# sclaus2/CutFEMx

Hardware: AMD Instinct MI355X
Metric: assembled DOFs/sec (active dofs / full hot-path step) + cut-quadrature points/sec, Poisson P1 sphere level-set (higher is better)
Workload: dtype f64; 1 GPU; 3D Poisson P1, sphere level set on 512^3 background mesh (805306368 tets), Nitsche + ghost penalty, runtime quadrature order 4; one step = cut + rules + sparsity + assemble_matrix + assemble_vector + deactivation; cells=805306368, active_dofs=17125633, parallelism=1 gpu

## Files before the change

cutfemx_amd/_lib.py:

```python
from __future__ import annotations

import ctypes as C
from pathlib import Path

import os

import numpy as np

_HERE = Path(__file__).resolve().parent
LIB_PATH = Path(os.environ["CFX_LIB"]).resolve() if os.environ.get("CFX_LIB") else _HERE / "libcutfemx_amd.so"

OK, ERR_INVALID_ARGUMENT, ERR_RUNTIME, ERR_OUT_OF_RANGE, ERR_HIP, ERR_STEP_VOID = 0, -1, -2, -3, -4, -5


class StepVoid(RuntimeError):
    """Raised inside a cutfemx_amd.step whose capacities (taken from the previous step) did not fit: the results of
    the step are void; `cutfemx_amd.run_step` ends it and repeats the body."""

INSIDE, INTERSECTED, OUTSIDE = -1, 0, 1
CELL, EXTERIOR_FACET, INTERIOR_FACET = 0, 1, 2
K_MASS, K_STIFFNESS, K_NITSCHE, K_GHOST_GRADJUMP, K_ELASTICITY = 1, 2, 3, 4, 5
K_EXTENSION_L2 = 8
K_JUMP = 9
K_SIP = 10
K_DIV_TEST, K_DIV_TRIAL = 20, 21
L_SOURCE, L_NITSCHE_RHS = 101, 102
M_FIELD, M_L2_DIFF, M_H1_SEMI = 201, 202, 203
F_ONE, F_SINPROD, F_POISSON_RHS, F_COEFFICIENT = 0, 1, 2, 3


class CutOptions(C.Structure):
    _fields_ = [("cut_approximation_order", C.c_int32), ("max_refinement_iterations", C.c_int32),
                ("edge_max_depth", C.c_int32), ("reserved", C.c_int32)]


class RulesView(C.Structure):
    _fields_ = [("tdim", C.c_int32), ("gdim", C.c_int32), ("nq", C.c_int64), ("nr", C.c_int64),
                ("points", C.c_void_p), ("weights", C.c_void_p), ("offsets", C.c_void_p),
                ("parent_map", C.c_void_p), ("host_width", C.c_int32), ("reserved", C.c_int32),
                ("host_rows", C.c_void_p), ("host_verts", C.c_void_p)]


class Integral(C.Structure):
    _fields_ = [("type", C.c_int32), ("kernel", C.c_int32), ("qdegree", C.c_int32),
                ("point_stride", C.c_int32), ("entities", C.c_void_p), ("n_entities", C.c_int64),
                ("rules", C.c_void_p), ("point_data", C.c_void_p), ("params", C.c_double * 8),
                ("coefficient", C.c_void_p)]


class Coefficient(C.Structure):
    _fields_ = [("space", C.c_void_p), ("values", C.c_void_p)]


class AggregationView(C.Structure):
    _fields_ = [("ncells", C.c_int64), ("root_cell", C.c_void_p), ("aggregate_id", C.c_void_p),
                ("propagation_depth", C.c_void_p), ("cut_volume_fraction", C.c_void_p),
                ("active_cells", C.c_void_p), ("cut_cells", C.c_void_p), ("interior_cells", C.c_void_p),
                ("well_posed_cells", C.c_void_p), ("ill_posed_cells", C.c_void_p), ("rootless_cells", C.c_void_p),
                ("n_active", C.c_int64), ("n_cut", C.c_int64), ("n_interior", C.c_int64),
                ("n_well_posed", C.c_int64), ("n_ill_posed", C.c_int64), ("n_rootless", C.c_int64),
                ("pairs", C.c_void_p), ("n_pairs", C.c_int64)]


class DistExchange(C.Structure):
    _fields_ = [("peer", C.c_int32), ("reserved", C.c_int32), ("send_offset", C.c_int64), ("send_count", C.c_int64),
                ("send_index", C.c_void_p), ("recv_offset", C.c_int64), ("recv_count", C.c_int64),
                ("recv_index", C.c_void_p)]


class DistRowExchange(C.Structure):
    _fields_ = [("peer", C.c_int32), ("reserved", C.c_int32), ("send_row_lo", C.c_int64), ("send_row_hi", C.c_int64),
                ("recv_row_lo", C.c_int64), ("recv_row_hi", C.c_int64)]


HOST_EXCHANGE_FN = C.CFUNCTYPE(C.c_int, C.c_void_p, C.c_int, C.POINTER(C.c_int32), C.POINTER(C.c_void_p),
                               C.POINTER(C.c_int64), C.POINTER(C.c_void_p), C.POINTER(C.c_int64))


class CGOptions(C.Structure):
    _fields_ = [("rtol", C.c_double), ("atol", C.c_double), ("max_iter", C.c_int32), ("check_every", C.c_int32),
                ("precond", C.c_int32), ("lanes_per_row", C.c_int32)]


class CGInfoStruct(C.Structure):
    _fields_ = [("reason", C.c_int32), ("iterations", C.c_int32), ("residual_norm", C.c_double), ("rhs_norm", C.c_double)]


PC_NONE, PC_JACOBI = 0, 1
CG_CONVERGED, CG_MAX_ITER, CG_BREAKDOWN, CG_BAD_DIAGONAL = 1, 2, 3, 4


class PatternView(C.Structure):
    _fields_ = [("nrows", C.c_int64), ("nnz", C.c_int64), ("indptr", C.c_void_p),
                ("indices", C.c_void_p), ("ncols", C.c_int64)]


SYMBOLS = [
    "cfx_init", "cfx_last_error", "cfx_set_stream", "cfx_synchronize", "cfx_step_begin", "cfx_step_end", "cfx_step_resolve", "cfx_step_abort",
    "cfx_step_set_margin", "cfx_step_forget", "cfx_sync_count", "cfx_list_count", "cfx_integrand_register", "cfx_integrand_compile", "cfx_integrand_register_facet", "cfx_integrand_register_variant", "cfx_integrand_compile_bs", "cfx_integrand_register2", "cfx_integrand_compile2", "cfx_integrand_compile_coefficients", "cfx_form_set_coefficients", "cfx_overlap_begin", "cfx_overlap_side", "cfx_overlap_end", "cfx_copy",
    "cfx_device_alloc", "cfx_device_free", "cfx_device_memset", "cfx_device_cache_release", "cfx_device_memory_stats", "cfx_profile_enable", "cfx_profile_reset",
    "cfx_profile_count", "cfx_profile_get", "cfx_event_create", "cfx_event_record",
    "cfx_event_elapsed_ms", "cfx_event_destroy", "cfx_mesh_create", "cfx_mesh_create_box", "cfx_mesh_create_slab",
    "cfx_mesh_info", "cfx_mesh_destroy", "cfx_cut_options_default", "cfx_cut_create",
    "cfx_cut_restrict", "cfx_cut_create_facets", "cfx_exterior_facets", "cfx_full_facet_rules",
    "cfx_facet_rules_to_cells", "cfx_cut_update", "cfx_cut_info", "cfx_cut_domain", "cfx_locate_entities",
    "cfx_runtime_quadrature", "cfx_runtime_quadratures", "cfx_full_cell_rules", "cfx_rules_create", "cfx_rules_view_get",
    "cfx_rules_physical_points", "cfx_rules_destroy", "cfx_evaluate_normals",
    "cfx_evaluate_values", "cfx_ghost_penalty_facets", "cfx_interior_facets_for_cells", "cfx_cell_aggregation_create", "cfx_cell_aggregation_view_get",
    "cfx_cell_aggregation_destroy", "cfx_cut_destroy", "cfx_space_create",
    "cfx_space_static_bytes", "cfx_space_lattice_rows", "cfx_space_lattice_source_rows", "cfx_space_destroy", "cfx_form_create", "cfx_form_create2", "cfx_form_destroy", "cfx_form_prepare", "cfx_create_sparsity",
    "cfx_pattern_view_get", "cfx_pattern_reuse_stats", "cfx_pattern_destroy", "cfx_assemble_matrix", "cfx_assemble_matrix_zeroed", "cfx_assemble_vector", "cfx_assemble_scalar",
    "cfx_apply_lifting", "cfx_set_bc", "cfx_zero_rows", "cfx_csr_block_merge", "cfx_csr_permute", "cfx_tabulate_entity", "cfx_active_domain", "cfx_active_view", "cfx_deactivate_outside",
    "cfx_active_destroy", "cfx_csr_spmv", "cfx_cg_options_default", "cfx_cg_solve",
    "cfx_dist_unique_id", "cfx_dist_comm_create", "cfx_dist_comm_create_host", "cfx_dist_comm_create_device", "cfx_dist_comm_info", "cfx_dist_comm_destroy",
    "cfx_dist_scatter_forward", "cfx_dist_scatter_reverse_add", "cfx_dist_scatter_reverse_matrix", "cfx_dist_indicator_or",
    "cfx_dist_indicator_forward",
    "cfx_mesh_create_f32", "cfx_cut_create_f32", "cfx_cut_update_f32", "cfx_rules_create_f32", "cfx_rules_view_get_f32",
    "cfx_rules_physical_points_f32", "cfx_evaluate_normals_f32", "cfx_evaluate_values_f32", "cfx_widen_f32",
    "cfx_assemble_matrix_f32", "cfx_assemble_matrix_zeroed_f32", "cfx_assemble_vector_f32", "cfx_apply_lifting_f32",
    "cfx_set_bc_f32", "cfx_zero_rows_f32", "cfx_deactivate_outside_f32",
    "cfx_assemble_matrix_c128", "cfx_assemble_vector_c128", "cfx_apply_lifting_c128", "cfx_set_bc_c128",
    "cfx_deactivate_outside_c128",
    "cfx_assemble_matrix_c64", "cfx_assemble_vector_c64", "cfx_apply_lifting_c64", "cfx_set_bc_c64", "cfx_deactivate_outside_c64",
]

_lib = None
_initialised = False


def load():
    global _lib
    if _lib is None:
        if not LIB_PATH.exists():
            raise RuntimeError(
                f"{LIB_PATH} is missing: build it with `python -c 'import __graft_entry__ as g; "
                "g.build()'` (hipcc --offload-arch=gfx950). cutfemx_amd has no CPU fallback.")
        import importlib.util
        import sys
        if "torch" not in sys.modules and importlib.util.find_spec("torch") is not None:
            import torch
        _lib = C.CDLL(str(LIB_PATH))
        _lib.cfx_last_error.restype = C.c_char_p
        for name in SYMBOLS:
            getattr(_lib, name)
    return _lib


def lib():
    global _initialised
    l = load()
    if not _initialised:
        check(l.cfx_init(_default_device()))
        _initialised = True
    return l


def _default_device() -> int:
    import os
    return int(os.environ.get("LOCAL_RANK", "0")) if os.environ.get("CFX_DEVICE") is None \
        else int(os.environ["CFX_DEVICE"])


def check(code: int):
    if code == OK:
        return
    msg = (load().cfx_last_error() or b"").decode()
    if code == ERR_INVALID_ARGUMENT:
        raise ValueError(msg)
    if code == ERR_OUT_OF_RANGE:
        raise IndexError(msg)
    if code == ERR_STEP_VOID:
        raise StepVoid(msg)
    raise RuntimeError(msg)


class DeviceBuffer:

    def __init__(self, count: int, dtype, shape=None):
        self.dtype = np.dtype(dtype)
        self.size = int(count)
        self.shape = shape if shape is not None else (self.size,)
        self.ndim = len(self.shape)
        p = C.c_void_p()
        check(lib().cfx_device_alloc(C.byref(p), C.c_size_t(max(self.size, 1) * self.dtype.itemsize)))
        self.ptr = p.value

    def numpy(self) -> np.ndarray:
        return download(self.ptr, self.size, self.dtype).reshape(self.shape)

    def fill_from(self, host: np.ndarray):
        host = np.ascontiguousarray(host, dtype=self.dtype)
        check(lib().cfx_copy(C.c_void_p(self.ptr), host.ctypes.data_as(C.c_void_p), C.c_size_t(host.nbytes)))

    def __del__(self):
        try:
            if self.ptr:
                load().cfx_device_free(C.c_void_p(self.ptr))
                self.ptr = None
        except Exception:
            pass


def is_torch(a) -> bool:
    return type(a).__module__.startswith("torch")


def is_device(a) -> bool:
    return isinstance(a, DeviceBuffer) or (is_torch(a) and a.is_cuda)


def as_ptr(a, dtype, keep: list):
    if a is None:
        return None
    if isinstance(a, DeviceBuffer):
        if a.dtype != np.dtype(dtype):
            raise TypeError(f"device buffer has dtype {a.dtype}, expected {np.dtype(dtype)}")
        keep.append(a)
        return C.c_void_p(a.ptr)
    if is_torch(a):
        import torch
        want = {np.float64: torch.float64, np.float32: torch.float32, np.int32: torch.int32, np.int8: torch.int8}[dtype]
        if a.dtype != want or not a.is_contiguous():
            a = a.to(want).contiguous()
        keep.append(a)
        return C.c_void_p(a.data_ptr())
    arr = np.ascontiguousarray(a, dtype=dtype)
    keep.append(arr)
    return arr.ctypes.data_as(C.c_void_p)


def scalar_dtype(a):
    if a is None:
        return np.float64
    if getattr(a, "dtype", None) == np.dtype(np.complex128):
        return np.complex128
    if getattr(a, "dtype", None) == np.dtype(np.complex64):
        return np.complex64
    if isinstance(a, DeviceBuffer):
        return np.float32 if a.dtype == np.dtype(np.float32) else np.float64
    if is_torch(a):
        import torch
        return np.float32 if a.dtype == torch.float32 else np.float64
    return np.float32 if getattr(a, "dtype", None) == np.dtype(np.float32) else np.float64


def release_cache():
    check(lib().cfx_device_cache_release())


def memory_stats(reset_peak: bool = False) -> dict:
    a, b, c = C.c_size_t(), C.c_size_t(), C.c_size_t()
    check(lib().cfx_device_memory_stats(C.byref(a), C.byref(b), C.byref(c), 1 if reset_peak else 0))
    return dict(in_use=a.value, cached=b.value, peak=c.value)


_step_open = False


def resolve_counts():
    if _step_open:
        check(lib().cfx_step_resolve())


# ... 12 lines not shown
```

cutfemx_amd/csrc/cfx_common.h:

```cpp
#pragma once

#include <hip/hip_runtime.h>

#include <algorithm>
#include <array>
#include <cstdint>
#include <cstdio>
#include <cstring>
#include <functional>
#include <map>
#include <memory>
#include <stdexcept>
#include <string>
#include <utility>
#include <vector>

#include "../../include/cutfemx_amd.h"
#include "cfx_switches.h"

namespace cfx
{

struct Error : std::runtime_error
{
// ... 357 lines not shown
  CFX_HIP(hipStreamSynchronize(ctx().stream));
  return a;
}

template <typename T>
inline DevArray<T> to_device_aligned(const T* src, int64_t n)
{
  if (src != nullptr && n > 0 && is_device_pointer(src) && (reinterpret_cast<uintptr_t>(src) & 15) != 0)
  {
    DevArray<T> a;
    a.alloc(n);
    CFX_HIP(hipMemcpyAsync(a.p, src, sizeof(T) * (size_t)n, hipMemcpyDeviceToDevice, ctx().stream));
    return a;
  }
  return to_device(src, n);
}

struct ErrorFlag
{
  int* p;
  bool deferred;
  ErrorFlag(int code, const char* message, void (*decode)(int) = nullptr);
  void check(int code, const char* message) const;
};
int64_t count_for_buffer(const Count& c, const void* user);
void end_of_call_sync();

int64_t& sync_counter();

void* pinned_scratch();

struct StepVoidGuard
{
  int64_t* host = nullptr;
  StepVoidGuard();
  void check() const;
};

template <typename T>
inline T read_scalar(const T* dev)
{
  static_assert(sizeof(T) <= 256, "read_scalar reads small values");
  T* h = static_cast<T*>(pinned_scratch());
  CFX_HIP(hipMemcpyAsync(h, dev, sizeof(T), hipMemcpyDeviceToHost, ctx().stream));
  const StepVoidGuard guard;
  CFX_HIP(hipStreamSynchronize(ctx().stream));
  const T v = *h;
  ++sync_counter();
  if (ctx().trace_sync) fprintf(stderr, "cutfemx_amd: read-back after %s\n", ctx().last_launch);
  guard.check();
  return v;
}

template <typename T>
inline void read_two(const T* dev_a, const T* dev_b, T& a, T& b)
{
  static_assert(2 * sizeof(T) <= 256, "read_two reads small values");
  T* h = static_cast<T*>(pinned_scratch());
  CFX_HIP(hipMemcpyAsync(h, dev_a, sizeof(T), hipMemcpyDeviceToHost, ctx().stream));
  CFX_HIP(hipMemcpyAsync(h + 1, dev_b, sizeof(T), hipMemcpyDeviceToHost, ctx().stream));
  const StepVoidGuard guard;
  CFX_HIP(hipStreamSynchronize(ctx().stream));
  a = h[0]; b = h[1];
  ++sync_counter();
  if (ctx().trace_sync) fprintf(stderr, "cutfemx_amd: read-back after %s\n", ctx().last_launch);
  guard.check();
}

template <typename T>
inline std::vector<T> download(const T* dev, int64_t n)
{
  std::vector<T> v((size_t)n);
  if (n > 0)
  {
    CFX_HIP(hipMemcpyAsync(v.data(), dev, sizeof(T) * (size_t)n, hipMemcpyDeviceToHost, ctx().stream));
    const StepVoidGuard guard;
    CFX_HIP(hipStreamSynchronize(ctx().stream));
    guard.check();
  }
  return v;
}

template <typename T>
struct OutArray
{
  T* user = nullptr;
  DevArray<T> staging;
  T* dev = nullptr;
  int64_t n = 0;
  OutArray(T* dst, int64_t count, bool copy_in) : user(dst), n(count)
  {
    if (is_device_pointer(dst)) { dev = dst; return; }
    staging.alloc(count);
    dev = staging.p;
    if (copy_in && count > 0)
      CFX_HIP(hipMemcpyAsync(dev, dst, sizeof(T) * (size_t)count, hipMemcpyHostToDevice, ctx().stream));
  }
  void finish()
  {
    if (dev != user && n > 0)
    {
      CFX_HIP(hipMemcpyAsync(user, dev, sizeof(T) * (size_t)n, hipMemcpyDeviceToHost, ctx().stream));
      CFX_HIP(hipStreamSynchronize(ctx().stream));
    }
  }
};

void exclusive_scan(const int32_t* in, int64_t* out, int64_t n, CountPlan* after = nullptr);
void exclusive_scan(const int32_t* in, int32_t* out, int64_t n, CountPlan* after = nullptr);
void exclusive_scan(const int64_t* in, int64_t* out, int64_t n, CountPlan* after = nullptr);
void exclusive_scan_pair(const int32_t* inA, int64_t* outA, const int32_t* inB, int64_t* outB, int64_t n, CountPlan* after = nullptr);
void exclusive_scan_pair(const int64_t* inA, int64_t* outA, const int64_t* inB, int64_t* outB, int64_t n, CountPlan* after = nullptr);

struct Adjacency
{
  DevArray<int64_t> offsets;
  DevArray<int32_t> cells;
  bool built = false;
};

void build_adjacency(const int32_t* map, int64_t ncells, int width, int64_t nitems, Adjacency& adj);

struct Stencil
{
  DevArray<int64_t> offsets;
  DevArray<int32_t> nbr;
  DevArray<uint32_t> slot4;
  DevArray<uint8_t> diagpos;
  DevArray<uint8_t> cpos;
  bool built = false, usable = false;
  bool lists = false;
  DevArray<uint8_t> slotn;
  bool slotn_built = false, slotn_ok = false;
  int max_len = 0;
  DevArray<int64_t> tile_voff;
  DevArray<int32_t> tile_verts;
  DevArray<uint16_t> st_loc;
  bool tiles_built = false, tiles_usable = false;
  int max_tile_verts = 0, max_tile_items = 0, max_tile_st = 0;
  bool lat_built = false, lat_tmpl_built = false;
  int64_t lat_rows = 0, lat_rstar = -1;
  int64_t lat_sb0 = 0;
  int lat_rel = 0;
  int lat_len = 0;
  DevArray<double> lat_scratch;
  const double* lat_tmpl = nullptr;
  DevArray<unsigned long long> lat_written;
  static constexpr int kLatStarCells = 64, kLatSrcDegrees = 9;
  int lat_src_state = 0;
  std::vector<double> lat_star;
  double lat_src_T[kLatSrcDegrees][8] = {};
  bool lat_src_T_built[kLatSrcDegrees] = {};
  DevArray<unsigned long long> lat_src_written;
  DevArray<uint8_t> arena;
  int64_t arena_used = 0;
  template <typename T>
  void take(DevArray<T>& a, int64_t n)
  {
    const int64_t bytes = ((int64_t)sizeof(T) * (n > 0 ? n : 1) + 255) & ~255LL;
    if (arena.p && arena_used + bytes <= arena.n)
    {
      a.release();
      a.p = reinterpret_cast<T*>(arena.p + arena_used); a.n = n; a.owned = false;
      arena_used += bytes;
    }
    else
      a.alloc(n);
  }
};
constexpr int kRowTile = 16;
constexpr unsigned kLatFlag = 0x80u, kDiagPosMask = 0x7fu;
__device__ __forceinline__ bool lattice_template_row(unsigned diagpos_raw, unsigned umark, unsigned long long mask,
                                                     unsigned inline_bits, unsigned long long full)
{
  return (diagpos_raw & kLatFlag) != 0 && __popc(umark & inline_bits) == 1 && mask == full;
}
__device__ __forceinline__ bool lattice_source_row(int32_t vec_t2off_r, unsigned diagpos_raw)
{
  return vec_t2off_r != 0 && (diagpos_raw & kLatFlag) != 0;
}

struct VecBlocks
{
  bool built = false, usable = false;
  int B = 0;
  int64_t nblocks = 0, u_total = 0;
  DevArray<int64_t> u_off;
  DevArray<uint16_t> slot;
  DevArray<uint16_t> seg;
  DevArray<int64_t> p_off;
  DevArray<int64_t> p_pos;
};
constexpr int kVbEntries = 2048;

constexpr int kKuhnTet[6][4] = {{0, 1, 3, 7}, {0, 1, 5, 7}, {0, 2, 3, 7}, {0, 2, 6, 7}, {0, 4, 5, 7}, {0, 4, 6, 7}};

}

struct cfx_mesh_s
{
  int tdim = 0, gdim = 0;
  int64_t nnodes = 0, ncells = 0;
  cfx::DevArray<double> x;
  cfx::DevArray<int32_t> conn;
  cfx::Adjacency v2c;
  const cfx::Adjacency& vertex_cells()
  {
    if (!v2c.built) cfx::build_adjacency(conn.p, ncells, tdim + 1, nnodes, v2c);
    return v2c;
  }
  cfx::DevArray<int32_t> c2c;
  bool c2c_built = false;
  int box_n = 0;
  bool hex_groups = false;
  cfx::DevArray<uint8_t> hex_corners;
  const cfx::DevArray<int32_t>& cell_neighbours();
  cfx::DevArray<int32_t> class_nruns;
  cfx::DevArray<int2> class_runs;
  cfx::DevArray<int2> class_sub_runs;
  bool class_built = false;
};
constexpr int kClassBlock = 1024, kClassRuns = 32;
constexpr int kClassSub = 4, kClassSubRuns = 16;

struct cfx_rules_s
{
  const uint64_t serial = cfx::next_serial();
  cfx_rules_s() { cfx::rules_serial_live(serial, true); }
  ~cfx_rules_s() { cfx::rules_serial_live(serial, false); }
  cfx_rules_s(const cfx_rules_s&) = delete;
  cfx_rules_s& operator=(const cfx_rules_s&) = delete;
  cfx_mesh_t mesh = nullptr;
  int tdim = 0, gdim = 0;
  cfx::Count nq, nr;
  cfx::DevArray<double> points, weights;
  cfx::DevArray<float> points_f32, weights_f32;
  cfx::DevArray<int32_t> offsets, parent_map;
  bool parent_sentinel = false;
  int host_width = 0;
  cfx::DevArray<int32_t> host_rows;
  cfx::DevArray<int32_t> host_verts;
};

struct cfx_cut_s
{
  cfx_mesh_t mesh = nullptr;
  int nls = 0;
  int ls_ndofs_cell = 0;
  int64_t ls_ndofs = 0;
  cfx_cut_options options{};
  cfx::DevArray<int32_t> ls_dofmap;
  std::vector<cfx::DevArray<double>> ls_values;
  cfx::DevArray<int8_t> domain;
  cfx::DevArray<uint8_t> host_mask;
  cfx::DevArray<int32_t> tile_block;
  cfx::DevArray<int32_t> tiles_inside, tiles_cut;
  cfx::DevArray<uint8_t> block_class;
  cfx::DevArray<uint8_t> codes0;
  cfx::DevArray<uint8_t> touch0;
  bool touch_valid = false;
  uint64_t gen = 0;
  ~cfx_cut_s() { cfx::provenance_forget_cut(this); }
  std::map<std::string, cfx::DevArray<int32_t>> located;
  std::map<std::string, cfx::DevArray<int32_t>> ghost_rows;
  int host_width = 0;
  int64_t n_hosts = 0;
  cfx::DevArray<int32_t> host_ids;
  cfx::DevArray<int32_t> host_rows;
  cfx::DevArray<int32_t> host_verts;
  std::map<std::string, cfx::DevArray<int32_t>> located_ids;
  int64_t nhosts() const { return host_width ? n_hosts : mesh->ncells; }
  int host_dim() const { return host_width ? mesh->tdim - 1 : mesh->tdim; }
};

struct cfx_pattern_cache
{
  struct cfx_pattern_s* live = nullptr;
  cfx::DevArray<int64_t> indptr;
  cfx::DevArray<int32_t> indices;
  cfx::DevArray<uint8_t> sig;
  std::vector<int> form_key;
  int64_t nrows = 0;
  bool valid = false;
  void drop();
};

struct cfx_space_s
{
  cfx_mesh_t mesh = nullptr;
  int degree = 1, bs = 1, ndofs_cell = 0;
  int64_t ndofs = 0;
  cfx::DevArray<int32_t> dofmap;
  cfx::Adjacency d2c;
  std::vector<std::weak_ptr<struct cfx_row_plan>> plans;
  cfx::Stencil stencil;
  cfx::VecBlocks vblocks;
  cfx::DevArray<int32_t> dof_verts;
  bool dof_verts_built = false, dof_verts_ok = false;
  cfx_pattern_cache pcache;
  ~cfx_space_s() { cfx::step_forget_owner(this); pcache.drop(); }
  bool lists_short_overflow = false;
  bool long_rows = false;
  bool huge_rows = false;
  const cfx::Adjacency& dof_cells()
  {
    if (dofmap.p == mesh->conn.p && ndofs == mesh->nnodes) return mesh->vertex_cells();
    if (!d2c.built) cfx::build_adjacency(dofmap.p, mesh->ncells, ndofs_cell, ndofs, d2c);
    return d2c;
  }
};

struct cfx_coefficient_dev
{
  cfx_space_t space = nullptr;
  cfx::DevArray<double> values;
};

struct cfx_integral_dev
{
  int type = 0, kernel = 0, qdegree = 0, point_stride = 0;
  cfx::DevArray<int32_t> entities;
  cfx::Count n_entities;
  cfx_rules_t rules = nullptr;
  uint64_t entities_serial = 0, rules_serial = 0;
  int64_t n_std = -1;
  cfx::DevArray<double> point_data;
  cfx::DevArray<double> coefficient;
  std::vector<cfx_coefficient_dev> coefficients;
  double params[8] = {0, 0, 0, 0, 0, 0, 0, 0};
};

struct cfx_row_plan
{
  bool built = false;
  bool usable = false;
  cfx::DevArray<uint8_t> mark_block;
  cfx::DevArray<uint8_t> rowcls;
  bool bulk = false;
  int bulk_kind = 0;
  uint8_t bulk_bits = 0;
  cfx::DevArray<uint8_t> cellmark;
  cfx::DevArray<uint8_t> cellsig;
  cfx::DevArray<uint8_t> rowmark;
  cfx::DevArray<int32_t> active_rows;
  cfx::Count n_active_rows;
  cfx::DevArray<int32_t> special_rows;
  cfx::Count n_special_rows;
  cfx::DevArray<uint8_t> special_mark;
  cfx::DevArray<int32_t> special_pos;
  cfx::DevArray<int32_t> plain_rows;
  cfx::Count n_plain_rows;
  uint64_t serial = 0;
  cfx::DevArray<unsigned long long> plain_masks;
  cfx::DevArray<uint8_t> plain_uniform;
  bool plain_masks_built = false;
  cfx::DevArray<int32_t> plain_tile_first, plain_tile_id;
  cfx::Count n_plain_tiles;
  cfx::DevArray<int32_t> lat_tile_first, lat_tile_id;
  cfx::Count n_lat_tiles;
  bool lat_tiles_built = false;
  unsigned lat_bits = 0;
  cfx::DevArray<int32_t> vec_t2off;
  bool vec_t2off_used = false;
  cfx::Count n_vec_odd_rows;
  cfx::Count vec_t2_total;
  int vec_fast = -1;
  uint8_t vec_mark = 0;
  bool vec_groups = false;
  int64_t vec_group_cap = 0;
  cfx::DevArray<int32_t> vb_active;
  cfx::DevArray<int32_t> vb_cut;
  cfx::DevArray<int64_t> vb_base;
  int64_t n_vb_active = 0, n_vb_cut = 0, vb_total = 0;
  int vb_state = -1;
  uint8_t vb_mark = 0;
  bool vb_merged = false;
  bool any_cells = false;
  cfx::Count nfacets;
  cfx::DevArray<int32_t> cell_tile_counts;
  cfx::DevArray<int64_t> row_tile_counts;
  bool fold_ok = true;
  cfx::DevArray<int32_t> facet_rows;
  cfx::DevArray<uint8_t> facet_slot;
  cfx::DevArray<int64_t> d2f_offsets;
  cfx::DevArray<int32_t> d2f;
  int n_cell_slots = 0, n_facet_slots = 0;
  cfx::DevArray<int64_t> std_bits[4];
  cfx::DevArray<int32_t> std_rank[4];
  cfx::DevArray<int32_t> rule_key_block;
  cfx::DevArray<int32_t> rule_keys[4], rule_first[4];
  uint32_t rule_mask[4] = {0, 0, 0, 0};
  cfx::DevArray<int32_t> cut_cells;
  int64_t n_cut_cells = 0;
  cfx::DevArray<int64_t> cut_bits;
  cfx::DevArray<int32_t> cut_rank;
  cfx::DevArray<int32_t> cut_first[4];
  bool cut_cells_built = false;
  int cell_slot_integral[4] = {0, 0, 0, 0};
  int facet_slot_integral[2] = {0, 0};
  std::vector<std::array<int64_t, 7>> key_cells, key_facets;
};

struct cfx_form_s
{
  cfx_space_t V = nullptr;
  cfx_space_t V1 = nullptr;
  bool rectangular() const { return V1 != nullptr && V1 != V; }
  int rank = 2;
  std::vector<cfx_integral_dev> integrals;
  std::shared_ptr<cfx_row_plan> plan;
  std::map<std::vector<int>, std::unique_ptr<cfx_form_s>> sub_forms;
};

namespace cfx
{
bool assemble_rect_rows(cfx_form_s* a, cfx_pattern_s* P, const int8_t* bc0, const int8_t* bc1, double* values, int* error);
cfx_row_plan& row_plan(cfx_form_s* a);
void validate_form(const cfx_form_s* a);
const Stencil& space_stencil(cfx_space_s* V);
const Stencil& space_stencil_slotn(cfx_space_s* V);
bool plain_row_masks(cfx_form_s* a, int32_t* counts = nullptr, int* maxlen = nullptr);
void plan_cut_cells(cfx_form_s* a);
const Stencil& space_stencil_tiles(cfx_space_s* V);
const Stencil& space_lattice(cfx_space_s* V);
bool lattice_template(cfx_space_s* V);
const double* lattice_source_moments(cfx_space_s* V, int qdegree);
bool plain_lattice_tiles(cfx_form_s* a, unsigned inline_bits);
bool space_dof_verts(cfx_space_s* V);
bool plain_vec_offsets(cfx_form_s* L, uint8_t mark);
bool source_groups_ok(cfx_form_s* L, uint8_t mark);
const VecBlocks& space_vec_blocks(cfx_space_s* V);
bool vec_block_plan(cfx_form_s* L, uint8_t mark, bool merged);
void build_pattern(cfx_form_s* a, cfx_pattern_s* P);
void build_pattern_rectangular(cfx_form_s* a, cfx_pattern_s* P);
void plan_cell_signature(cfx_form_s* a);
bool pattern_reuse_ok(cfx_form_s* a);
void pattern_remember(cfx_form_s* a, cfx_pattern_s* P);
void prepare_form_tables(cfx_form_s* a);
bool assemble_matrix_rows(cfx_form_s* a, cfx_pattern_s* P, const int8_t* bc0, const int8_t* bc1, double* values,
                          bool fresh = false);
bool assemble_vector_rows(cfx_form_s* L, double* b);
bool user_integrand_known(int kernel);
int user_integrand_rank(int kernel);
int user_integrand_kind(int kernel);
bool user_integrand_two(int kernel);
void user_coefficients_check(const cfx_form_s* a, const cfx_integral_dev& I);
int64_t user_stage1_facets(const cfx_form_s* a, const cfx_integral_dev& I, double* out, int64_t only_index = -1);
int64_t user_stage1(const cfx_form_s* a, const cfx_integral_dev& I, bool runtime, double* out, int out_mode, int64_t out_stride,
                    int64_t only_index = -1);
void functional_entity(const cfx_form_s* M, const cfx_integral_dev& I, int64_t index, int use_rule, double* out_dev);
}

struct cfx_pattern_s
{
  cfx_space_s* cache_owner = nullptr;
  ~cfx_pattern_s();
  int64_t nrows = 0;
  cfx::Count nnz;
  int64_t ncols = 0;
  int max_row_len = 0;
  int64_t n_hashed_rows = 0, n_reused_rows = 0;
  uint64_t built_plan = 0;
  uint64_t stencil_plan = 0;
  uint64_t split_plan = 0;
  cfx::DevArray<int32_t> short_rows, mid_rows, long_rows;
  int64_t n_short_rows = 0, n_mid_rows = 0, n_long_rows = 0;
  uint64_t full_plan = 0;
  cfx::DevArray<int32_t> full_rows;
  int64_t n_full_rows = 0;
  int64_t n_full_short = 0;
  uint64_t odd_plan = 0;
  cfx::DevArray<int32_t> odd_rows;
  int64_t n_odd_rows = 0;
  cfx::DevArray<int32_t> rest_rows;
  int64_t n_rest_rows = 0;
  cfx::DevArray<int64_t> indptr;
  cfx::DevArray<int32_t> indices;
};

struct cfx_aggregation_s
{
  int64_t ncells = 0;
  cfx::DevArray<int32_t> root_cell, aggregate_id, depth;
  cfx::DevArray<double> fraction;
  cfx::DevArray<int32_t> active, cut, interior, well, ill, rootless, pairs;
  int64_t n_pairs = 0;
};

struct cfx_active_s
{
  cfx_space_t V = nullptr;
  std::shared_ptr<cfx_row_plan> plan;
  cfx::DevArray<uint8_t> cell_indicator;
  bool lists_built = false;
  cfx::DevArray<int32_t> active_cells, inactive_dofs;
  cfx::Count n_active, n_inactive;
};
namespace cfx
{
void active_lists(cfx_active_s* d);
}
```

cutfemx_amd/csrc/cfx_fem.hip:

```cpp
#include <cstdlib>

#include "cfx_elem.h"

using namespace cfx;

namespace
{

struct AsmArgs
{
  const double* x;
  const int32_t* conn;
  const int32_t* dofmap;
  DevN n;
  const int32_t* entities;
  const int32_t* offsets;
  const int32_t* parent_map;
  const double* points;
  const double* weights;
  const double* point_data;
  int point_stride;
  int kernel;
  int qdegree;
  double params[8];
// ... 1586 lines not shown
}
template <int TDIM>
__global__ void __launch_bounds__(kBlock) cut_moments_kernel(int64_t nr, const int32_t* __restrict__ offsets,
                                                             const double* __restrict__ points, const double* __restrict__ weights,
                                                             double* __restrict__ out)
{
  constexpr int NV = TDIM + 1, NM = 1 + NV + NV * (NV + 1) / 2;
  const int64_t e = (int64_t)blockIdx.x * kBlock + threadIdx.x;
  if (e >= nr) return;
  double m[16];
#pragma unroll
  for (int k = 0; k < 16; ++k) m[k] = 0.0;
  const int32_t q0 = offsets[e], q1 = offsets[e + 1];
  for (int32_t q = q0; q < q1; ++q)
  {
    double lam[NV];
    lam[0] = 1.0;
#pragma unroll
    for (int t = 0; t < TDIM; ++t) { lam[t + 1] = points[(int64_t)q * TDIM + t]; lam[0] -= lam[t + 1]; }
    const double w = weights[q];
    m[0] += w;
    int idx = 1 + NV;
#pragma unroll
    for (int x = 0; x < NV; ++x)
    {
      const double wx = w * lam[x];
      m[1 + x] += wx;
#pragma unroll
      for (int y = x; y < NV; ++y) m[idx++] += wx * lam[y];
    }
  }
  static_assert(NM <= 16, "record of 16 doubles");
  double2* o = reinterpret_cast<double2*>(out + 16 * e);
#pragma unroll
  for (int k = 0; k < 8; ++k) o[k] = make_double2(m[2 * k], m[2 * k + 1]);
}
}

namespace cfx
{
void dump_integral(cfx_form_s* a, int integral, int parts, double* out, bool fold_facets)
{
  cfx_space_s* V = a->V;
  ZeroFlag err;
  AsmArgs A{};
  A.x = V->mesh->x.p; A.conn = V->mesh->conn.p; A.dofmap = V->dofmap.p;
  A.dump = out; A.error = err.p;
  A.dump_fold = fold_facets ? 1 : 0;
  const cfx_integral_dev& I = a->integrals[integral];
  if (a->rectangular() && user_integrand_known(I.kernel)) launch_user_integral(a, I, A, -1, 0, parts);
  else launch_integral(a, I, A, -1, 0, parts);
}
void dump_facet_jumps_p1(cfx_form_s* a, int integral, double* out, int* error)
{
  cfx_space_s* V = a->V;
  const cfx_integral_dev& I = a->integrals[integral];
  if (I.n_entities.cap() == 0) return;
  if (V->mesh->tdim == 2)
    launch("assemble_facets", facet_jump_p1_kernel<2>, grid_for(I.n_entities.cap()), dim3(kBlock), 0, I.n_entities, I.entities.p,
           V->mesh->x.p, V->mesh->conn.p, V->dofmap.p, I.params[0], I.params[1], I.qdegree, out, error);
  else
    launch("assemble_facets", facet_jump_p1_kernel<3>, grid_for(I.n_entities.cap()), dim3(kBlock), 0, I.n_entities, I.entities.p,
           V->mesh->x.p, V->mesh->conn.p, V->dofmap.p, I.params[0], I.params[1], I.qdegree, out, error);
}
void dump_cut_moments(cfx_form_s* a, int integral, double* out)
{
  const cfx_integral_dev& I = a->integrals[integral];
  if (!I.rules || I.rules->nr.value() == 0) return;
  const int64_t nrl = I.rules->nr.value();
  if (a->V->mesh->tdim == 2)
    launch("assemble_cells_cut", cut_moments_kernel<2>, grid_for(nrl), dim3(kBlock), 0, nrl,
           I.rules->offsets.p, I.rules->points.p, I.rules->weights.p, out);
  else
    launch("assemble_cells_cut", cut_moments_kernel<3>, grid_for(nrl), dim3(kBlock), 0, nrl,
           I.rules->offsets.p, I.rules->points.p, I.rules->weights.p, out);
}

void dump_facet_jumps_p2(cfx_form_s* a, int integral, int nq, double* out)
{
  cfx_space_s* V = a->V;
  const cfx_integral_dev& I = a->integrals[integral];
  const int64_t nf = I.n_entities.value();
  if (nf == 0) return;
  if (V->mesh->tdim == 2)
    launch("assemble_facets", facet_jumps_p2_kernel<2>, grid_for(nf * nq), dim3(kBlock), 0, nf, nq,
           I.entities.p, V->mesh->x.p, V->mesh->conn.p, V->dofmap.p, I.params[0], I.params[1], I.qdegree, out);
  else
    launch("assemble_facets", facet_jumps_p2_kernel<3>, grid_for(nf * nq), dim3(kBlock), 0, nf, nq,
           I.entities.p, V->mesh->x.p, V->mesh->conn.p, V->dofmap.p, I.params[0], I.params[1], I.qdegree, out);
}
}

extern "C" {

int cfx_space_create(cfx_mesh_t mesh, int degree, int bs, int64_t ndofs, const int32_t* dofmap, int ndofs_cell,
                     cfx_space_t* out)
{
  CFX_API_BEGIN
  ctx().ensure();
  require(mesh && dofmap && out, CFX_ERR_INVALID_ARGUMENT, "cfx_space_create: null argument");
  require(degree == 1 || degree == 2, CFX_ERR_INVALID_ARGUMENT, "cfx_space_create: Lagrange degree must be 1 or 2");
  const int expect = degree == 1 ? mesh->tdim + 1 : (mesh->tdim == 2 ? 6 : 10);
  require(ndofs_cell == expect, CFX_ERR_INVALID_ARGUMENT, "cfx_space_create: dofs per cell do not match the element");
  require(bs == 1 || bs == mesh->gdim, CFX_ERR_INVALID_ARGUMENT, "cfx_space_create: block size must be 1 or gdim");
  require(ndofs > 0 && ndofs * bs < 2147483647LL, CFX_ERR_INVALID_ARGUMENT, "cfx_space_create: dof count must fit int32");
  auto V = std::make_unique<cfx_space_s>();
  V->mesh = mesh; V->degree = degree; V->bs = bs; V->ndofs = ndofs; V->ndofs_cell = ndofs_cell;
  V->dofmap = to_device_aligned(dofmap, mesh->ncells * (int64_t)ndofs_cell);
  *out = V.release();
  CFX_API_END
}

int cfx_space_static_bytes(cfx_space_t V, int64_t bytes[4])
{
  CFX_API_BEGIN
  require(V && bytes, CFX_ERR_INVALID_ARGUMENT, "cfx_space_static_bytes: null argument");
  const bool shared = V->dofmap.p == V->mesh->conn.p && V->ndofs == V->mesh->nnodes;
  const cfx::Adjacency& adj = shared ? V->mesh->v2c : V->d2c;
  bytes[0] = adj.built ? 8 * adj.offsets.n + 4 * adj.cells.n : 0;
  const cfx::Stencil& S = V->stencil;
  bytes[1] = 8 * S.offsets.n + 4 * S.nbr.n + 4 * S.slot4.n + S.diagpos.n + S.cpos.n + S.slotn.n;
  const cfx::VecBlocks& B = V->vblocks;
  bytes[2] = 8 * S.tile_voff.n + 4 * S.tile_verts.n + 2 * S.st_loc.n
             + 8 * B.u_off.n + 2 * B.slot.n + 2 * B.seg.n + 8 * B.p_off.n + 8 * B.p_pos.n;
  bytes[3] = (V->mesh->c2c_built ? 4 * V->mesh->c2c.n : 0)
             + (V->mesh->class_built ? 4 * V->mesh->class_nruns.n + 8 * (V->mesh->class_runs.n + V->mesh->class_sub_runs.n) : 0);
  CFX_API_END
}

int cfx_space_lattice_rows(cfx_space_t V, int64_t* n, int64_t* template_rows)
{
  CFX_API_BEGIN
  require(V && n, CFX_ERR_INVALID_ARGUMENT, "cfx_space_lattice_rows: null argument");
  *n = 0;
  if (template_rows) *template_rows = 0;
  if (V->degree != 1 || V->bs != 1 || !cfx::space_stencil(V).usable) return CFX_OK;
  const cfx::Stencil& S = cfx::space_lattice(V);
  *n = S.lat_rows;
  if (template_rows && S.lat_rows > 0 && S.lat_written.p) *template_rows = (int64_t)cfx::read_scalar(S.lat_written.p);
  CFX_API_END
}

int cfx_space_lattice_source_rows(cfx_space_t V, int64_t* rows)
{
  CFX_API_BEGIN
  require(V && rows, CFX_ERR_INVALID_ARGUMENT, "cfx_space_lattice_source_rows: null argument");
  *rows = 0;
  if (V->degree != 1 || V->bs != 1 || !cfx::space_stencil(V).usable) return CFX_OK;
  const cfx::Stencil& S = cfx::space_lattice(V);
  if (S.lat_rows > 0 && S.lat_src_written.p) *rows = (int64_t)cfx::read_scalar(S.lat_src_written.p);
  CFX_API_END
}

int cfx_space_destroy(cfx_space_t V)
{
  CFX_API_BEGIN
  delete V;
  CFX_API_END
}

static int form_create_impl(cfx_space_t V, cfx_space_t V1, int rank, int n_integrals, const cfx_integral* integrals,
                            cfx_form_t* out);

int cfx_form_create(cfx_space_t V, int rank, int n_integrals, const cfx_integral* integrals, cfx_form_t* out)
{
  return form_create_impl(V, V, rank, n_integrals, integrals, out);
}

int cfx_form_create2(cfx_space_t V_test, cfx_space_t V_trial, int n_integrals, const cfx_integral* integrals, cfx_form_t* out)
{
  CFX_API_BEGIN
  require(V_test && V_trial, CFX_ERR_INVALID_ARGUMENT, "cfx_form_create2: null argument");
  require(V_test->mesh == V_trial->mesh, CFX_ERR_INVALID_ARGUMENT, "cfx_form_create2: the two spaces live on different meshes");
  CFX_API_END_NO_RETURN
  return form_create_impl(V_test, V_trial, 2, n_integrals, integrals, out);
}

static int form_create_impl(cfx_space_t V, cfx_space_t V1, int rank, int n_integrals, const cfx_integral* integrals,
                            cfx_form_t* out)
{
  CFX_API_BEGIN
  ctx().ensure();
  require(V && out && (integrals || n_integrals == 0), CFX_ERR_INVALID_ARGUMENT, "cfx_form_create: null argument");
  require(rank == 0 || rank == 1 || rank == 2, CFX_ERR_INVALID_ARGUMENT, "cfx_form_create: rank must be 0, 1 or 2");
  auto a = std::make_unique<cfx_form_s>();
  a->V = V; a->V1 = V1; a->rank = rank;
  const bool rect = V1 != V;
  for (int i = 0; i < n_integrals; ++i)
  {
    const cfx_integral& in = integrals[i];
    cfx_integral_dev I;
    I.type = in.type; I.kernel = in.kernel; I.qdegree = in.qdegree; I.point_stride = in.point_stride;
    require(in.type == CFX_CELL || in.type == CFX_INTERIOR_FACET, CFX_ERR_INVALID_ARGUMENT,
            "cfx_form_create: integral type must be cell or interior_facet");
    const bool user = user_integrand_known(in.kernel);
    const int kernel_rank = user ? user_integrand_rank(in.kernel) : (in.kernel < 100 ? 2 : (in.kernel < 200 ? 1 : 0));
    const bool bilinear = kernel_rank == 2;
    require(kernel_rank == rank, CFX_ERR_INVALID_ARGUMENT, "cfx_form_create: kernel rank does not match the form");
    require(in.qdegree >= 0 && in.qdegree <= CFX_QUAD_MAX_DEGREE, CFX_ERR_INVALID_ARGUMENT,
            "cfx_form_create: quadrature degree out of range");
    if (user)
    {
      if (rect)
        require(user_integrand_two(in.kernel), CFX_ERR_INVALID_ARGUMENT,
                "cfx_form_create2: the integrand was registered for a square form (one space); a form between two spaces "
                "takes an integrand registered with cfx_integrand_register2");
      else
        require(!user_integrand_two(in.kernel), CFX_ERR_INVALID_ARGUMENT,
                "cfx_form_create: the integrand was registered with cfx_integrand_register2 for a form between two spaces; "
                "a square form takes one registered for one space");
    }
    if (in.type == CFX_INTERIOR_FACET && user)
    {
      require(user_integrand_kind(in.kernel) == 1 && V->degree <= 2 && V1->degree <= 2 && 2 * V->ndofs_cell * V->bs <= 24
                  && 2 * V1->ndofs_cell * V1->bs <= 24,
              CFX_ERR_INVALID_ARGUMENT,
              "cfx_form_create: an interior-facet integral takes an integrand registered with cfx_integrand_register_facet "
              "(or cfx_integrand_register2 with facet = 1): spaces of degree 1 or 2 with at most 24 macro dofs on each side");
      if (in.rules)
        require(in.rules->host_width == 4 && in.point_data == nullptr, CFX_ERR_INVALID_ARGUMENT,
                "cfx_form_create: runtime rules of an interior-facet integral are facet-hosted rules over interior rows "
                "(cfx_cut_create_facets with row_width 4)");
    }
    else if (in.type == CFX_INTERIOR_FACET && rank == 0)
      throw Error(CFX_ERR_INVALID_ARGUMENT,
                  "cfx_form_create: interior-facet integrals of a functional take registered facet integrands "
                  "(cfx_integrand_register_variant with rank 0, facet 1)");
    else if (in.type == CFX_INTERIOR_FACET)
    {
      require(in.kernel == CFX_K_GHOST_GRADJUMP || in.kernel == CFX_K_EXTENSION_L2 || in.kernel == CFX_K_JUMP
                  || in.kernel == CFX_K_SIP,
              CFX_ERR_INVALID_ARGUMENT,
              "cfx_form_create: interior-facet integrals support the ghost-penalty, value-jump, interior-penalty and "
              "extension-penalty kernels");
      if (in.rules)
        require(in.kernel != CFX_K_EXTENSION_L2 && in.rules->host_width == 4 && in.point_data == nullptr,
                CFX_ERR_INVALID_ARGUMENT,
                "cfx_form_create: runtime rules of an interior-facet integral are facet-hosted rules over interior rows "
                "(cfx_cut_create_facets with row_width 4)");
    }
    else if (in.rules && in.rules->host_width != 0)
      throw Error(CFX_ERR_INVALID_ARGUMENT,
                  "cfx_form_create: a cell integral takes cell-hosted rules (pass facet-hosted rules through "
                  "cfx_facet_rules_to_cells)");
    else if (user)
      require(in.type == CFX_CELL && V->degree <= 2 && V1->degree <= 2 && user_integrand_kind(in.kernel) == 0,
              CFX_ERR_INVALID_ARGUMENT,
              "cfx_form_create: a cell integral takes an integrand registered with cfx_integrand_register (spaces of degree 1 or 2)");
    else if (rank == 0)
      require((in.kernel == CFX_M_FIELD || in.kernel == CFX_M_L2_DIFF || in.kernel == CFX_M_H1_SEMI)
                  && (V->degree == 1 || V->degree == 2) && V->bs >= 1 && V->bs <= 3,
              CFX_ERR_INVALID_ARGUMENT,
              "cfx_form_create: unknown functional id (CFX_M_FIELD, CFX_M_L2_DIFF, CFX_M_H1_SEMI on Lagrange spaces of degree "
              "1 or 2, block size 1..3)");
    else
      require(in.kernel == CFX_K_MASS || in.kernel == CFX_K_STIFFNESS || in.kernel == CFX_K_NITSCHE
                  || in.kernel == CFX_K_ELASTICITY || in.kernel == CFX_L_SOURCE || in.kernel == CFX_L_NITSCHE_RHS
                  || (rect && (in.kernel == CFX_K_DIV_TEST || in.kernel == CFX_K_DIV_TRIAL)),
              CFX_ERR_INVALID_ARGUMENT,
              "cfx_form_create: unknown cell kernel id (the divergence blocks need different test and trial spaces: "
              "cfx_form_create2)");
    if (rect && user)
    {
    }
    else if (rect)
    {
      require(in.coefficient == nullptr && in.point_data == nullptr, CFX_ERR_INVALID_ARGUMENT,
              "cfx_form_create2: coefficients / per-point data are not supported on rectangular blocks");
      const int gd = V->mesh->gdim;
      if (in.type == CFX_INTERIOR_FACET)
        require((in.kernel == CFX_K_GHOST_GRADJUMP || in.kernel == CFX_K_JUMP) && V->bs == 1 && V1->bs == 1 && in.rules == nullptr,
                CFX_ERR_INVALID_ARGUMENT,
                "cfx_form_create2: cell integrals, and interior-facet integrals (gradient jump, value jump) between "
                "scalar spaces over standard facets");
      else if (in.kernel == CFX_K_DIV_TEST)
        require(V->bs == gd && V1->bs == 1, CFX_ERR_INVALID_ARGUMENT, "div(v) p: vector test space, scalar trial space");
      else if (in.kernel == CFX_K_DIV_TRIAL)
        require(V->bs == 1 && V1->bs == gd, CFX_ERR_INVALID_ARGUMENT, "q div(u): scalar test space, vector trial space");
      else
        require((in.kernel == CFX_K_MASS || in.kernel == CFX_K_STIFFNESS) && V->bs == V1->bs, CFX_ERR_INVALID_ARGUMENT,
                "cfx_form_create2: mass / stiffness blocks need equal block sizes; other kernels are square-only");
    }
    if (in.kernel == CFX_K_NITSCHE || in.kernel == CFX_L_NITSCHE_RHS)
    {
      require(V->bs == 1, CFX_ERR_INVALID_ARGUMENT, "Nitsche kernels are scalar");
      require(in.n_entities == 0 && in.rules && in.point_data && in.point_stride >= V->mesh->gdim,
              CFX_ERR_INVALID_ARGUMENT,
              "Nitsche kernels need runtime interface rules and per-point normals (point_data)");
    }
    if (in.kernel == CFX_K_ELASTICITY)
      require(V->bs == V->mesh->gdim, CFX_ERR_INVALID_ARGUMENT, "elasticity needs a vector space (bs == gdim)");
    if (in.kernel == CFX_L_SOURCE)
      require(V->bs == 1 || (int)in.params[0] == CFX_F_COEFFICIENT, CFX_ERR_INVALID_ARGUMENT,
              "the source term of a vector space takes a vector-valued Function (field id CFX_F_COEFFICIENT)");
    if (bilinear)
    {
      require(in.coefficient == nullptr || in.kernel == CFX_K_MASS || in.kernel == CFX_K_STIFFNESS
                  || in.kernel == CFX_K_ELASTICITY || (rect && user),
              CFX_ERR_INVALID_ARGUMENT, "cfx_form_create: a coefficient is accepted by the mass, stiffness and elasticity terms");
      if (in.coefficient) I.coefficient = to_device(in.coefficient, V->ndofs);
    }
    else if (rank == 0)
    {
      const int field = (int)in.params[0];
      if (user)
        require(in.type == CFX_CELL || in.coefficient == nullptr || V->bs == 1, CFX_ERR_INVALID_ARGUMENT,
// ... 730 lines not shown
```

cutfemx_amd/csrc/cfx_gather.hip:

```cpp
#include <cstdlib>
#include <type_traits>

#include "cfx_elem.h"

using namespace cfx;

namespace cfx
{
void dump_integral(cfx_form_s* a, int integral, int parts, double* out, bool fold_facets = false);
void dump_facet_jumps_p1(cfx_form_s* a, int integral, double* out, int* error);
void dump_facet_jumps_p2(cfx_form_s* a, int integral, int nq, double* out);
void dump_cut_moments(cfx_form_s* a, int integral, double* out);
int quad_npoints(int dim, int degree);
}

namespace
{

constexpr int kWave = 64;
#ifndef CFX_XCD_TILE
#define CFX_XCD_TILE 128
#endif
__device__ __forceinline__ int64_t row_block_id(int64_t b)
{
// ... 432 lines not shown
  double det;
  if constexpr (TDIM == 2) det = ed[0][0] * ed[1][1] - ed[0][1] * ed[1][0];
  else
    det = ed[0][0] * (ed[1][1] * ed[2][2] - ed[1][2] * ed[2][1]) - ed[0][1] * (ed[1][0] * ed[2][2] - ed[1][2] * ed[2][0])
          + ed[0][2] * (ed[1][0] * ed[2][1] - ed[1][1] * ed[2][0]);
  const double cscale = fscale * fabs(det);
#pragma unroll
  for (int i = 0; i < ND; ++i) be[i] = 0.0;
  const double umax = kPi * hmax;
  if (umax <= 0.03)
  {
    double S[TDIM], C[TDIM];
#pragma unroll
    for (int d = 0; d < TDIM; ++d)
    {
      if (Sa) { S[d] = Sa[d]; C[d] = Ca[d]; }
      else cfx_sincospi(x[0][d], S[d], C[d]);
#pragma unroll
      for (int t = 0; t < TDIM; ++t) ed[t][d] *= kPi;
    }
    auto series = [&](auto deg_tag)
    {
      constexpr int DEGS = decltype(deg_tag)::value;
      double co[TDIM][DEGS + 1];
#pragma unroll
      for (int d = 0; d < TDIM; ++d)
      {
        const double inv[8] = {1.0, 1.0, -1.0 / 2.0, -1.0 / 6.0, 1.0 / 24.0, 1.0 / 120.0, -1.0 / 720.0, -1.0 / 5040.0};
#pragma unroll
        for (int k = 0; k <= DEGS; ++k) co[d][k] = ((k & 1) ? C[d] : S[d]) * inv[k];
      }
      for (int q = 0; q < npts; ++q)
      {
        double X[TDIM];
#pragma unroll
        for (int t = 0; t < TDIM; ++t) X[t] = pts[q * TDIM + t];
        double f = wts[q];
#pragma unroll
        for (int d = 0; d < TDIM; ++d)
        {
          double u = X[0] * ed[0][d];
#pragma unroll
          for (int t = 1; t < TDIM; ++t) u = fma(X[t], ed[t][d], u);
          double p = co[d][DEGS];
#pragma unroll
          for (int k = DEGS - 1; k >= 0; --k) p = fma(p, u, co[d][k]);
          f *= p;
        }
        be[0] += f;
#pragma unroll
        for (int t = 0; t < TDIM; ++t) be[t + 1] = fma(f, X[t], be[t + 1]);
      }
#pragma unroll
      for (int t = 0; t < TDIM; ++t) be[0] -= be[t + 1];
#pragma unroll
      for (int i = 0; i < ND; ++i) be[i] *= cscale;
    };
    if (umax <= 0.0065) series(std::integral_constant<int, 5>{});
    else series(std::integral_constant<int, 7>{});
  }
  else
  {
    for (int q = 0; q < npts; ++q)
    {
      double X[TDIM], l0 = 1.0;
#pragma unroll
      for (int t = 0; t < TDIM; ++t) { X[t] = pts[q * TDIM + t]; l0 -= X[t]; }
      double f = wts[q] * cscale;
#pragma unroll
      for (int d = 0; d < TDIM; ++d)
      {
        double v = x[0][d];
#pragma unroll
        for (int t = 0; t < TDIM; ++t) v = fma(X[t], ed[t][d], v);
        f *= cfx_sinpi(v);
      }
      be[0] = fma(f, l0, be[0]);
#pragma unroll
      for (int t = 0; t < TDIM; ++t) be[t + 1] = fma(f, X[t], be[t + 1]);
    }
  }
}

template <int TDIM>
__device__ __forceinline__ void source_compute(const VecArgs& A, const SourceCell<TDIM>& c, bool valid, int npts,
                                               const double* __restrict__ pts, const double* __restrict__ wts, double fscale)
{
  constexpr int ND = TDIM + 1;
  double be[ND];
  source_vector<TDIM>(c.x, npts, pts, wts, fscale, be);
  if (!valid) return;
  bool record = A.t2 == nullptr;
#pragma unroll
  for (int i = 0; i < ND; ++i)
  {
    if (c.t2o[i] >= 0) A.t2[(int64_t)c.t2o[i] + ((c.cp >> (8 * i)) & 0xffu)] = be[i];
    else record = true;
  }
  if (record)
  {
#pragma unroll
    for (int i = 0; i < ND; ++i) A.out[A.out_cells > 0 ? (int64_t)i * A.out_cells + c.cell : (int64_t)i * A.n.cap + c.e] = be[i];
  }
}

#ifndef CFX_SOURCE_WAVES
#define CFX_SOURCE_WAVES 4
#endif
template <int TDIM>
__global__ void __launch_bounds__(kBlock, CFX_SOURCE_WAVES) vec_source_sin_p1_kernel(VecArgs A)
{
  const int64_t stride = (int64_t)gridDim.x * kBlock;
  const int64_t e0 = (int64_t)blockIdx.x * kBlock + threadIdx.x;
  const int64_t An = dev_n(A.n);
  if (An == 0) return;
  const int64_t last = An - 1;
  int npts;
  const double* wts;
  const double* pts = ref_rule(TDIM, A.qdegree, npts, wts);
  const double fscale = A.params[1] * ((int)A.params[0] == CFX_F_POISSON_RHS ? (double)TDIM * kPi * kPi : 1.0);
  auto ent = [&](int64_t e) { return A.entities[e < last ? e : last]; };
  SourceCell<TDIM> a, b;
  int32_t cell_c, cell_d;
  a.e = e0; b.e = e0 + stride;
  a.cell = ent(a.e); b.cell = ent(b.e); cell_c = ent(e0 + 2 * stride);
  source_load_conn<TDIM>(A, a);
  source_load_conn<TDIM>(A, b);
  source_load_vertices<TDIM>(A, a);
  for (int64_t e = e0; e < An; e += stride)
  {
    cell_d = ent(e + 3 * stride);
    SourceCell<TDIM> c;
    c.e = e + 2 * stride; c.cell = cell_c;
    source_load_conn<TDIM>(A, c);
    source_load_vertices<TDIM>(A, b);
    source_compute<TDIM>(A, a, true, npts, pts, wts, fscale);
    a = b;
    b = c;
    cell_c = cell_d;
  }
}

struct GroupHead
{
  const int32_t* ent;
  __device__ bool operator()(int64_t i) const { return i == 0 || ent[i - 1] / 6 != ent[i] / 6; }
};

struct GroupArgs
{
  const int32_t* first;
  DevN ng;
  int64_t cap;
};

template <bool LATTICE>
__global__ void __launch_bounds__(kBlock, CFX_SOURCE_WAVES) vec_source_groups_kernel(VecArgs A, GroupArgs G, const uint8_t* __restrict__ diagpos)
{
  __shared__ int32_t s_queue[LATTICE ? kBlock : 1];
  __shared__ int s_n;
  int64_t g = (int64_t)blockIdx.x * kBlock + threadIdx.x;
  int q = threadIdx.x, nq = 0;
  if constexpr (!LATTICE)
  {
    if (g >= dev_n(G.ng)) return;
  }
  else
  {
    if (threadIdx.x == 0) s_n = 0;
    __syncthreads();
    if (g < dev_n(G.ng))
    {
      const int4* c = reinterpret_cast<const int4*>(A.conn) + 6 * (int64_t)(A.entities[G.first[g]] / 6);
      const int4 r0 = c[0], r3 = c[3], r4 = c[4];
      const int32_t cv[8] = {r0.x, r0.y, r3.y, r0.z, r4.y, r4.z, r3.z, r0.w};
      bool bulk = true;
#pragma unroll
      for (int k = 0; k < 8; ++k) bulk = bulk & lattice_source_row(A.t2off[cv[k]], diagpos[cv[k]]);
      if (!bulk) s_queue[atomicAdd(&s_n, 1)] = (int32_t)threadIdx.x;
    }
    __syncthreads();
    nq = s_n;
  }
  do
  {
    if constexpr (LATTICE)
    {
      if (q >= nq) break;
      g = (int64_t)blockIdx.x * kBlock + s_queue[q];
      q += kBlock;
    }
    const int64_t n = dev_n(A.n), f = G.first[g];
    int32_t ids[6];
#pragma unroll
    for (int m = 0; m < 6; ++m) ids[m] = A.entities[f + m < n ? f + m : n - 1];
    const int32_t hex = ids[0] / 6;
    unsigned mask = 0;
#pragma unroll
    for (int m = 0; m < 6; ++m)
      if (f + m < n && ids[m] / 6 == hex) mask |= 1u << (ids[m] - 6 * hex);
    const int4* conn4 = reinterpret_cast<const int4*>(A.conn) + 6 * (int64_t)hex;
    const int4 r0 = conn4[0], r3 = conn4[3], r4 = conn4[4];
    const int32_t cv[8] = {r0.x, r0.y, r3.y, r0.z, r4.y, r4.z, r3.z, r0.w};
    double x0[3], x7[3];
    load_vertex<3>(A.x, cv[0], x0);
    load_vertex<3>(A.x, cv[7], x7);
    unsigned plain = 0;
#pragma unroll
    for (int k = 0; k < 8; ++k) plain |= A.t2off[cv[k]] != 0 ? 1u << k : 0u;
    int npts;
    const double* wts;
    const double* pts = ref_rule(3, A.qdegree, npts, wts);
    const double fscale = A.params[1] * ((int)A.params[0] == CFX_F_POISSON_RHS ? 3.0 * kPi * kPi : 1.0);
    double S[3], C[3];
#pragma unroll
    for (int d = 0; d < 3; ++d) cfx_sincospi(x0[d], S[d], C[d]);
    double acc[8];
#pragma unroll
    for (int k = 0; k < 8; ++k) acc[k] = 0.0;
    const int64_t stride = A.out_cells > 0 ? A.out_cells : A.n.cap;
    constexpr unsigned kMidA = 0x442211u, kMidB = 0x656353u;
    int j = __builtin_ctz(mask);
#pragma unroll 1
    while (true)
    {
      const unsigned rest = mask & ~((2u << j) - 1u);
      const int4 row = conn4[j];
      double x[4][3];
      load_vertex<3>(A.x, row.y, x[1]);
      load_vertex<3>(A.x, row.z, x[2]);
#pragma unroll
      for (int d = 0; d < 3; ++d) { x[0][d] = x0[d]; x[3][d] = x7[d]; }
      double be[4];
      source_vector<3>(x, npts, pts, wts, fscale, be, S, C);
      const int ka = (int)((kMidA >> (4 * j)) & 0xfu), kb = (int)((kMidB >> (4 * j)) & 0xfu);
      acc[0] += be[0];
      acc[7] += be[3];
#pragma unroll
      for (int k = 1; k < 7; ++k) acc[k] += k == ka ? be[1] : (k == kb ? be[2] : 0.0);
      if ((plain & ((1u << ka) | (1u << kb) | 0x81u)) != ((1u << ka) | (1u << kb) | 0x81u))
      {
        const int64_t at = A.out_cells > 0 ? 6 * (int64_t)hex + j : f + __popc(mask & ((1u << j) - 1u));
#pragma unroll
        for (int i = 0; i < 4; ++i) A.out[(int64_t)i * stride + at] = be[i];
      }
      if (!rest) break;
      j = __builtin_ctz(rest);
    }
    const int4 s0 = conn4[0], s3 = conn4[3], s4 = conn4[4];
    const int32_t sv[8] = {s0.x, s0.y, s3.y, s0.z, s4.y, s4.z, s3.z, s0.w};
#pragma unroll
    for (int k = 0; k < 8; ++k)
    {
      if constexpr (LATTICE)
      {
        const int32_t off = A.t2off[sv[k]];
        if (off != 0 && !lattice_source_row(off, diagpos[sv[k]])) A.t2[(int64_t)k * G.cap + off - 1] = acc[k];
      }
      else if (plain & (1u << k)) A.t2[(int64_t)k * G.cap + A.t2off[sv[k]] - 1] = acc[k];
    }
  } while (LATTICE);
}

struct VecBlockArgs
{
  int64_t n_active;
  const int32_t* active;
  const int64_t* base;
  const int64_t* u_off;
  const uint16_t* slot;
  const uint16_t* seg;
  const uint8_t* cellmark;
  uint8_t mark;
  int64_t ncells;
  double* part;
  struct Rules
  {
    const int32_t* parent_map;
    DevN nr;
    const double* tensors;
    const int32_t* keys;
    const int32_t* first;
    unsigned mask;
  } rules[4];
  int n_slots;
};

template <int ND>
__device__ __forceinline__ void add_rule_vectors(const VecBlockArgs& P, int64_t c, unsigned cm, double* be)
{
  if ((cm & 0xF0u) == 0) return;
  for (int s = 0; s < P.n_slots; ++s)
    if (cm & (16u << s))
    {
      const VecBlockArgs::Rules& R = P.rules[s];
      for (int64_t e = first_rule(R.keys, R.first, R.mask, (int32_t)c); e < dev_len(R.nr) && R.parent_map[e] == c; ++e)
#pragma unroll
        for (int j = 0; j < ND; ++j) be[j] += R.tensors[e * ND + j];
    }
}

template <int ND>
__device__ __forceinline__ void load_slots(const uint16_t* __restrict__ slot, int64_t c, uint16_t* sl)
{
  if constexpr (ND % 4 == 0)
  {
    const uint2* w = reinterpret_cast<const uint2*>(slot + c * ND);
#pragma unroll
    for (int j = 0; j < ND / 4; ++j)
    {
      const uint2 v = w[j];
      sl[4 * j] = (uint16_t)(v.x & 0xffffu); sl[4 * j + 1] = (uint16_t)(v.x >> 16);
      sl[4 * j + 2] = (uint16_t)(v.y & 0xffffu); sl[4 * j + 3] = (uint16_t)(v.y >> 16);
    }
  }
  else if constexpr (ND % 2 == 0)
  {
    const uint32_t* w = reinterpret_cast<const uint32_t*>(slot + c * ND);
#pragma unroll
    for (int j = 0; j < ND / 2; ++j)
    {
      const uint32_t v = w[j];
      sl[2 * j] = (uint16_t)(v & 0xffffu); sl[2 * j + 1] = (uint16_t)(v >> 16);
    }
  }
  else
  {
#pragma unroll
    for (int j = 0; j < ND; ++j) sl[j] = slot[c * ND + j];
  }
}

#ifndef CFX_VB_WAVES
#define CFX_VB_WAVES 5
#endif
template <int TDIM, int DEG, int B, int RULES>
__global__ void __launch_bounds__(B, DEG == 2 ? CFX_VB_WAVES : 1) vec_blocks_kernel(VecArgs A, VecBlockArgs P)
{
  constexpr int ND = Elem<TDIM, DEG>::ND;
  __shared__ double s_val[B * ND];
  const int32_t entry = P.active[blockIdx.x];
  const int64_t k = entry & 0x7fffffff;
  const int64_t c = k * B + threadIdx.x;
  const int nb = (int)min((int64_t)B, P.ncells - k * B);
  const bool inb = (int)threadIdx.x < nb;
  const int64_t ub = P.u_off[k], pb = P.base[k];
  const int nu = (int)(P.u_off[k + 1] - ub);
  constexpr int NW = (ND + 1) / 2;
  uint32_t slw[NW];
  if (inb)
  {
    if constexpr (ND % 2 == 0)
    {
      const uint32_t* w = reinterpret_cast<const uint32_t*>(P.slot + c * ND);
#pragma unroll
      for (int j = 0; j < NW; ++j) slw[j] = w[j];
    }
    else
    {
#pragma unroll
      for (int j = 0; j < NW; ++j)
        slw[j] = (uint32_t)P.slot[c * ND + 2 * j] | (2 * j + 1 < ND ? (uint32_t)P.slot[c * ND + 2 * j + 1] << 16 : 0u);
    }
  }
  const unsigned cm = inb ? P.cellmark[c] : 0u;
  int32_t vids[TDIM + 1];
  if constexpr (RULES != 1)
  {
    if constexpr (TDIM == 3)
    {
      const int4 r = *reinterpret_cast<const int4*>(A.conn + (inb ? c : k * B) * 4);
      vids[0] = r.x; vids[1] = r.y; vids[2] = r.z; vids[3] = r.w;
    }
    else
    {
#pragma unroll
      for (int i = 0; i <= TDIM; ++i) vids[i] = A.conn[(inb ? c : k * B) * (TDIM + 1) + i];
    }
  }
  const int t0 = threadIdx.x;
  const uint32_t f01 = (t0 < nu ? (uint32_t)P.seg[ub + t0] : 0u) | ((t0 + 1 < nu ? (uint32_t)P.seg[ub + t0 + 1] : (uint32_t)(nb * ND)) << 16);
  double be[ND];
#pragma unroll
  for (int j = 0; j < ND; ++j) be[j] = 0.0;
  if constexpr (RULES != 0) add_rule_vectors<ND>(P, c, cm, be);
  if constexpr (RULES != 1)
  {
    if (cm & P.mark) entity_vector<TDIM, DEG, false, 1>(A, 0, c, 0, be, vids);
  }
  if (inb)
  {
#pragma unroll
    for (int j = 0; j < ND; ++j) s_val[(slw[j / 2] >> (16 * (j & 1))) & 0xffffu] = be[j];
  }
  __syncthreads();
  const bool add = RULES == 1 && entry >= 0;
  const int f0 = (int)(f01 & 0xffffu), f1 = (int)(f01 >> 16);
  constexpr int T = 3;
  int g0[T], g1[T];
#pragma unroll
  for (int q = 0; q < T; ++q)
  {
    const int t = t0 + (q + 1) * B;
    g0[q] = t < nu ? (int)P.seg[ub + t] : 0;
    g1[q] = t + 1 < nu ? (int)P.seg[ub + t + 1] : nb * ND;
  }
  if (t0 < nu)
  {
    double sum = 0.0;
    for (int i = f0; i < f1; ++i) sum += s_val[i];
    if (add) P.part[pb + t0] += sum; else P.part[pb + t0] = sum;
  }
#pragma unroll
  for (int q = 0; q < T; ++q)
// ... 2557 lines not shown
#pragma unroll
        for (int a = 0; a < NV; ++a) N[a] = lam[a] * (2.0 * lam[a] - 1.0);
#pragma unroll
        for (int e2 = 0; e2 < NE; ++e2)
        {
          const int a = TDIM == 2 ? ea2[e2 % 3] : ea3[e2 % 6], b = TDIM == 2 ? eb2[e2 % 3] : eb3[e2 % 6];
          N[NV + e2] = 4.0 * lam[a] * lam[b];
        }
        double gam = 0.0;
        if (S.kernel == CFX_K_NITSCHE)
        {
          const double* nrm = S.point_data + (int64_t)q * S.point_stride;
          double al[NV];
          al[0] = 0.0;
#pragma unroll
          for (int t = 0; t < TDIM; ++t)
          {
            double v = 0.0;
#pragma unroll
            for (int d = 0; d < TDIM; ++d) v += g.K[t][d] * nrm[d];
            al[t + 1] = v; al[0] -= v;
          }
#pragma unroll
          for (int a = 0; a < NV; ++a) dn[a] = (4.0 * lam[a] - 1.0) * al[a];
#pragma unroll
          for (int e2 = 0; e2 < NE; ++e2)
          {
            const int a = TDIM == 2 ? ea2[e2 % 3] : ea3[e2 % 6], b = TDIM == 2 ? eb2[e2 % 3] : eb3[e2 % 6];
            dn[NV + e2] = 4.0 * (lam[b] * al[a] + lam[a] * al[b]);
          }
          gam = S.params[0] / h;
        }
        else
        {
#pragma unroll
          for (int a = 0; a < ND; ++a) dn[a] = 0.0;
          gam = 1.0;
        }
        int p = 0;
#pragma unroll
        for (int a = 0; a < ND; ++a)
        {
          const double ga = gam * N[a] - dn[a];
#pragma unroll
          for (int b = a; b < ND; ++b)
          {
            const double v = w * (ga * N[b] - N[a] * dn[b]);
            To[p / kCutLanes2] += ((p % kCutLanes2) == sub) ? v : 0.0;
            ++p;
          }
        }
      }
    }
  }
#pragma unroll
  for (int p = 0; p < NP; ++p)
    if ((p % kCutLanes2) == sub) s_T[ci][p] = To[p / kCutLanes2];
  __syncthreads();
  if (!live) return;
  double* out = A.out + k * (int64_t)(ND * ND);
  for (int i = sub; i < ND; i += kCutLanes2)
  {
    double row[ND];
#pragma unroll
    for (int j = 0; j < ND; ++j)
    {
      const int a = i < j ? i : j, b = i < j ? j : i;
      row[j] = s_T[ci][a * ND - a * (a - 1) / 2 + (b - a)];
    }
    if (mom[0] != 0.0) p2_stiffness_row_moments<TDIM>(g, i, mom, row);
    double2* o2 = reinterpret_cast<double2*>(out + i * ND);
#pragma unroll
    for (int j = 0; j < ND / 2; ++j) o2[j] = make_double2(row[2 * j], row[2 * j + 1]);
  }
}

struct Stage1
{
  std::vector<DevArray<double>> buffers;
  DevArray<double> t2;
  double* vec_t2 = nullptr;
  const uint8_t* lat_src = nullptr;
  const double* lat_src_T = nullptr;
  bool vec_blocks = false;
  DevArray<double> part;
};

inline DevN rule_bound(const cfx_rules_s* R)
{
  if (R->nr.pending() && R->parent_sentinel) return DevN(R->nr.cap() + 1);
  return R->nr.devn();
}

inline VecArgs vec_args(cfx_form_s* L, const cfx_integral_dev& I)
{
  cfx_space_s* V = L->V;
  VecArgs A{};
  A.x = V->mesh->x.p; A.conn = V->mesh->conn.p;
  A.kernel = I.kernel; A.qdegree = I.qdegree; A.point_stride = I.point_stride;
  for (int k = 0; k < 8; ++k) A.params[k] = I.params[k];
  A.dofmap = V->dofmap.p;
  A.coeff = I.coefficient.n > 0 ? I.coefficient.p : nullptr;
  return A;
}

template <int DEG>
inline bool source_series_ok(const cfx_space_s* V, const cfx_integral_dev& I)
{
  const int field = (int)I.params[0];
  return DEG == 1 && I.kernel == CFX_L_SOURCE && I.coefficient.n == 0 && (field == CFX_F_SINPROD || field == CFX_F_POISSON_RHS)
         && V->dofmap.p == V->mesh->conn.p && env_on<Sw::SOURCE_SERIES>();
}

template <int TDIM, int DEG>
void vec_block_partials(cfx_form_s* L, const cfx_integral_dev* Istd, uint8_t mark, const RowArgs& R, double* part)
{
  cfx_space_s* V = L->V;
  cfx_row_plan& plan = row_plan(L);
  const VecBlocks& S = space_vec_blocks(V);
  constexpr int ND = Elem<TDIM, DEG>::ND, B = ND <= 8 ? 256 : 128;
  if (S.B != B) throw Error(CFX_ERR_RUNTIME, "vec_block_partials: block size of the space's cell blocks");
  VecArgs A{};
  A.x = V->mesh->x.p; A.conn = V->mesh->conn.p;
  if (Istd) A = vec_args(L, *Istd);
  VecBlockArgs P{};
  P.n_active = plan.n_vb_active; P.active = plan.vb_active.p; P.base = plan.vb_base.p; P.u_off = S.u_off.p;
  P.slot = S.slot.p; P.seg = S.seg.p; P.cellmark = plan.cellmark.p; P.mark = mark; P.ncells = V->mesh->ncells; P.part = part;
  P.n_slots = R.n_cell;
  for (int s = 0; s < R.n_cell; ++s)
  {
    const RowIntegral& I = R.cell[s];
    P.rules[s] = {I.parent_map, I.rule_tensors ? I.nr : DevN(0), I.rule_tensors, I.rule_keys, I.rule_first, I.rule_mask};
  }
  if (P.n_active == 0) {}
  else if (Istd && source_series_ok<DEG>(V, *Istd))
  {
    if constexpr (DEG == 1)
    {
      const int64_t blocks = std::min<int64_t>(P.n_active, 256 * CFX_SOURCE_BLOCKS_PER_CU);
      launch("vec_blocks_std", vec_blocks_sin_p1_kernel<TDIM>, dim3((unsigned)blocks), dim3(kBlock), 0, A, P);
    }
  }
  else if (plan.vb_merged)
    launch("vec_blocks_std", vec_blocks_kernel<TDIM, DEG, B, 2>, dim3((unsigned)P.n_active), dim3(B), 0, A, P);
  else
    launch("vec_blocks_std", vec_blocks_kernel<TDIM, DEG, B, 0>, dim3((unsigned)P.n_active), dim3(B), 0, A, P);
  if (plan.n_vb_cut > 0)
  {
    P.n_active = plan.n_vb_cut; P.active = plan.vb_cut.p;
    launch("vec_blocks_cut", vec_blocks_kernel<TDIM, DEG, B, 1>, dim3((unsigned)P.n_active), dim3(B), 0, A, P);
  }
}

template <int TDIM, int DEG>
void vec_tensors(cfx_form_s* L, const cfx_integral_dev& I, bool runtime, double* out, double* t2 = nullptr, int64_t out_cells = 0,
                 const uint8_t* lat_src = nullptr)
{
  cfx_space_s* V = L->V;
  if (user_integrand_known(I.kernel))
  {
    if (runtime) user_stage1(L, I, true, out, 0, 0);
    else user_stage1(L, I, false, out, out_cells > 0 ? 2 : 1, out_cells > 0 ? out_cells : I.n_entities.cap());
    return;
  }
  VecArgs A = vec_args(L, I);
  A.out_cells = out_cells;
  if (t2 && !runtime)
  {
    A.t2 = t2; A.t2off = row_plan(L).vec_t2off.p; A.cpos = space_stencil(V).cpos.p;
  }
  A.out = out;
  if (!runtime)
  {
    A.n = I.n_entities; A.entities = I.entities.p;
    cfx_row_plan& plan = row_plan(L);
    if (TDIM == 3 && DEG == 1 && A.t2 && plan.vec_groups && source_series_ok<DEG>(V, I))
    {
      DevArray<int32_t> first;
      const Count ng = compact_count("source_groups", "vec.source_groups", A.n, GroupHead{A.entities}, first);
      GroupArgs G{first.p, ng.devn(), plan.vec_group_cap};
      if (ng.cap() > 0 && lat_src)
        launch("vec_tensors_std", vec_source_groups_kernel<true>, grid_for(ng.cap()), dim3(kBlock), 0, A, G, lat_src);
      else if (ng.cap() > 0)
        launch("vec_tensors_std", vec_source_groups_kernel<false>, grid_for(ng.cap()), dim3(kBlock), 0, A, G, lat_src);
    }
    else if (source_series_ok<DEG>(V, I))
    {
      if constexpr (DEG == 1)
      {
        const int64_t blocks = std::min<int64_t>((A.n.cap + kBlock - 1) / kBlock, 256 * CFX_SOURCE_BLOCKS_PER_CU);
        launch("vec_tensors_std", vec_source_sin_p1_kernel<TDIM>, dim3((unsigned)blocks), dim3(kBlock), 0, A);
      }
    }
    else
      launch("vec_tensors_std", vec_tensors_kernel<TDIM, DEG, false>, grid_for(A.n.cap), dim3(kBlock), 0, A);
  }
  else
  {
    const cfx_rules_s* R = I.rules;
    A.n = R->nr; A.offsets = R->offsets.p; A.parent_map = R->parent_map.p; A.points = R->points.p;
    A.weights = R->weights.p; A.point_data = I.point_data.n > 0 ? I.point_data.p : nullptr;
    const dim3 grid = grid_for(A.n.cap * CFX_VEC_CUT_LANES);
    if (I.kernel == CFX_L_SOURCE)
      launch("vec_tensors_cut", vec_tensors_kernel<TDIM, DEG, true, CFX_VEC_CUT_LANES, 1>, grid, dim3(kBlock), 0, A);
    else if (I.kernel == CFX_L_NITSCHE_RHS)
      launch("vec_tensors_cut", vec_tensors_kernel<TDIM, DEG, true, CFX_VEC_CUT_LANES, 2>, grid, dim3(kBlock), 0, A);
    else
      launch("vec_tensors_cut", vec_tensors_kernel<TDIM, DEG, true, CFX_VEC_CUT_LANES>, grid, dim3(kBlock), 0, A);
  }
}

inline bool p2_cut_tensors_ok(const cfx_form_s* a)
{
  if (!env_on<Sw::P2_CUT_TENSORS>()) return false;
  if (a->rank != 2 || a->V->degree != 2 || a->V->bs != 1) return false;
  bool any = false;
  for (const auto& I : a->integrals)
    if (I.type == CFX_CELL && I.rules && I.rules->nr.cap() > 0)
    {
      if (!(I.kernel == CFX_K_STIFFNESS || I.kernel == CFX_K_MASS || I.kernel == CFX_K_NITSCHE) || I.coefficient.n > 0) return false;
      any = true;
    }
  return any;
}

template <int TDIM, int DEG, int BS = 1>
RowArgs prepare(cfx_form_s* a, Stage1& st, bool combine_cuts = false)
{
  constexpr int ND = Elem<TDIM, DEG>::ND * BS;
  cfx_row_plan& plan = row_plan(a);
  cfx_space_s* V = a->V;
  RowArgs A{};
  A.x = V->mesh->x.p; A.conn = V->mesh->conn.p; A.dofmap = V->dofmap.p;
  A.iso_geometry = (DEG == 1 && V->dofmap.p == V->mesh->conn.p) ? 1 : 0;
  A.n_active = plan.n_active_rows; A.active_rows = plan.active_rows.p;
  if (plan.any_cells)
  {
    const Adjacency& adj = V->dof_cells();
    A.d2c_off = adj.offsets.p; A.d2c = adj.cells.p; A.cellmark = plan.cellmark.p;
  }
  const int64_t tsize = a->rank == 2 ? ND * ND : ND;
  A.n_cell = plan.n_cell_slots;
  for (int s = 0; s < plan.n_cell_slots; ++s)
  {
    const int ii = plan.cell_slot_integral[s];
    const cfx_integral_dev& I = a->integrals[ii];
    RowIntegral& R = A.cell[s];
    R.kernel = I.kernel; R.qdegree = I.qdegree; R.point_stride = I.point_stride;
    for (int k = 0; k < 8; ++k) R.params[k] = I.params[k];
    const int64_t n_ent = I.n_entities.cap();
    if (n_ent > 0)
    {
      R.std_bits = reinterpret_cast<const unsigned long long*>(plan.std_bits[s].p);
      R.std_rank = plan.std_rank[s].p;
    }
    const bool inline_ok = BS > 1 ? (I.kernel == CFX_K_ELASTICITY || I.kernel == CFX_K_MASS || I.kernel == CFX_K_STIFFNESS)
                                  : (DEG == 1 ? I.kernel == CFX_K_STIFFNESS
                                              : (I.kernel == CFX_K_STIFFNESS || I.kernel == CFX_K_MASS));
    R.std_inline = (a->rank == 2 && inline_ok && kRowsInline<DEG> && I.coefficient.n == 0) ? 1 : 0;
    if (BS > 1) R.std_inline = 0;
    if (R.std_inline && A.iso_geometry) R.std_inline = 2;
    if (R.std_inline == 1) A.iso_geometry = 0;
    {
      if (DEG == 2 && BS == 1 && a->rank == 2 && I.kernel == CFX_K_STIFFNESS && I.coefficient.n == 0 && I.qdegree >= 2
          && env_on<Sw::P2_CLOSED>())
        R.std_inline = 3;
      if (DEG == 2 && BS == TDIM && p2_elasticity_closed(a, I)) R.std_inline = 3;
    }
    if (a->rank == 1 && st.vec_blocks && n_ent > 0)
      R.std_tensors = nullptr;
    else if (!R.std_inline && n_ent > 0)
    {
      const bool by_cell = a->rank == 1 && BS == 1 && !st.vec_t2 && n_ent * 4 >= V->mesh->ncells;
      st.buffers.emplace_back((by_cell ? V->mesh->ncells : n_ent) * tsize);
      R.std_tensors = st.buffers.back().p;
      R.n_std = by_cell ? V->mesh->ncells : n_ent;
      R.std_by_cell = by_cell ? 1 : 0;
      if (a->rank == 2) dump_integral(a, ii, 1, st.buffers.back().p);
      else if constexpr (BS == 1)
        vec_tensors<TDIM, DEG>(a, I, false, st.buffers.back().p, st.vec_t2, by_cell ? V->mesh->ncells : 0, st.lat_src);
    }
    const int64_t n_rules = I.rules ? I.rules->nr.cap() : 0;
    if (n_rules > 0 && combine_cuts)
    {
      R.parent_map = I.rules->parent_map.p; R.nr = rule_bound(I.rules);
      R.rule_keys = plan.rule_keys[s].p; R.rule_first = plan.rule_first[s].p; R.rule_mask = plan.rule_mask[s];
    }
    else if (n_rules > 0)
    {
      R.parent_map = I.rules->parent_map.p; R.nr = rule_bound(I.rules);
      R.rule_keys = plan.rule_keys[s].p; R.rule_first = plan.rule_first[s].p; R.rule_mask = plan.rule_mask[s];
      const bool moments = DEG == 2 && BS == 1 && a->rank == 2 && I.kernel == CFX_K_STIFFNESS && I.coefficient.n == 0
                           && env_on<Sw::P2_MOMENTS>();
      st.buffers.emplace_back(n_rules * (moments ? 16 : tsize));
      R.rule_tensors = st.buffers.back().p;
      R.rule_moments = moments ? 1 : 0;
      if (moments) dump_cut_moments(a, ii, st.buffers.back().p);
      else if (a->rank == 2) dump_integral(a, ii, 2, st.buffers.back().p);
      else if constexpr (BS == 1) vec_tensors<TDIM, DEG>(a, I, true, st.buffers.back().p);
    }
  }
  if constexpr (DEG == 2 && BS == 1)
  {
    if (combine_cuts)
    {
      plan_cut_cells(a);
      if (plan.n_cut_cells > 0)
      {
        CutTensorArgs C{};
        C.n = plan.n_cut_cells; C.cut_cells = plan.cut_cells.p; C.cellmark = plan.cellmark.p;
        C.x = A.x; C.conn = A.conn; C.n_slots = plan.n_cell_slots;
        for (int s = 0; s < plan.n_cell_slots; ++s)
        {
          const cfx_integral_dev& I = a->integrals[plan.cell_slot_integral[s]];
          CutSlot& S = C.slot[s];
          S.kernel = I.kernel; S.point_stride = I.point_stride; S.params[0] = I.params[0]; S.params[1] = I.params[1];
          if (I.rules && I.rules->nr.value() > 0)
          {
            S.offsets = I.rules->offsets.p; S.parent_map = I.rules->parent_map.p; S.nr = I.rules->nr.value();
            S.points = I.rules->points.p; S.weights = I.rules->weights.p;
            S.point_data = I.point_data.n > 0 ? I.point_data.p : nullptr;
            S.rule_keys = plan.rule_keys[s].p; S.rule_first = plan.rule_first[s].p; S.rule_mask = plan.rule_mask[s];
            S.cut_first = plan.cut_first[s].p;
          }
        }
        st.buffers.emplace_back(plan.n_cut_cells * (int64_t)(ND * ND));
        C.out = st.buffers.back().p;
        launch("cut_tensors_p2", cut_tensors_p2_kernel<TDIM>, grid_for(C.n * kCutLanes2), dim3(kBlock), 0, C);
        A.cut_tensors = C.out;
        A.cut_bits = reinterpret_cast<const unsigned long long*>(plan.cut_bits.p);
        A.cut_rank = plan.cut_rank.p;
      }
    }
  }
  bool has_facets = false;
  A.fold_facets = plan.fold_ok ? 1 : 0;
  for (const auto& I : a->integrals)
  {
    has_facets = has_facets || I.type == CFX_INTERIOR_FACET;
    if (I.type == CFX_INTERIOR_FACET && I.kernel == CFX_K_EXTENSION_L2) A.fold_facets = 0;
  }
  if (has_facets && plan.nfacets.cap() > 0)
  {
    A.d2f_off = plan.d2f_offsets.p; A.d2f = plan.d2f.p; A.facet_rows = plan.facet_rows.p;
    A.special_mark = plan.special_mark.p; A.special_pos = plan.special_pos.p;
    const char fe = env_char<Sw::FACET_FOLD_STAGE1>();
    const bool fold1 = fe != '0', fold1_records = fold1 && fe != '2';
    bool user_facets = false;
    for (int s = 0; s < plan.n_facet_slots; ++s)
      user_facets = user_facets || user_integrand_known(a->integrals[plan.facet_slot_integral[s]].kernel);
    if (TDIM == 3 && DEG == 1 && BS == 1 && A.fold_facets && a->rank == 2 && fold1 && !user_facets) A.fold_facets = 2;
    bool rank_one = DEG == 1 && BS == 1 && A.fold_facets && a->rank == 2 && fold1_records;
    for (int s = 0; s < plan.n_facet_slots; ++s)
    {
      const cfx_integral_dev& I = a->integrals[plan.facet_slot_integral[s]];
      rank_one = rank_one && I.kernel == CFX_K_GHOST_GRADJUMP && I.rules == nullptr && I.n_std < 0;
    }
    if (rank_one) A.fold_facets = 3;
    if (DEG == 2 && A.fold_facets && a->rank == 2 && fold1)
    {
      bool low = true;
      int qd = -1;
      for (int s = 0; s < plan.n_facet_slots; ++s)
      {
        const cfx_integral_dev& I = a->integrals[plan.facet_slot_integral[s]];
        low = low && I.kernel == CFX_K_GHOST_GRADJUMP && I.rules == nullptr && I.n_std < 0
              && (qd < 0 || qd == I.qdegree);
        qd = I.qdegree;
      }
      const int nq = low ? quad_npoints(TDIM - 1, qd) : 0;
      if (low && nq >= 1 && nq <= 6) { A.fold_facets = 3; A.facet_nq = nq; }
    }
    const int64_t fsize = A.fold_facets == 3 ? (DEG == 2 ? 8 + 16 * A.facet_nq : 10)
                                             : (A.fold_facets == 2 ? (ND + 1) * (ND + 1) : 4 * ND * ND);
    st.buffers.emplace_back(plan.nfacets.cap() * fsize);
    A.facet_tensors = st.buffers.back().p;
    int64_t o = 0;
    for (int s = 0; s < plan.n_facet_slots; ++s)
    {
      const int ii = plan.facet_slot_integral[s];
      if (A.fold_facets == 3 && DEG == 2) dump_facet_jumps_p2(a, ii, A.facet_nq, st.buffers.back().p + o * fsize);
      else if (A.fold_facets == 3) dump_facet_jumps_p1(a, ii, st.buffers.back().p + o * fsize, nullptr);
      else dump_integral(a, ii, 1, st.buffers.back().p + o * fsize, A.fold_facets == 2);
      o += a->integrals[ii].n_entities.cap();
    }
  }
  return A;
}

constexpr const char* kEntryMissing = "assemble_matrix: entry not in the sparsity pattern";
inline void raise_gather_error(int err)
{
  require(err != 1, CFX_ERR_RUNTIME, kEntryMissing);
  require(err != 2, CFX_ERR_RUNTIME, "assemble_matrix: row longer than the gather kernel's capacity");
  require(err != 5, CFX_ERR_RUNTIME, "assemble_matrix: a stencil-subset row does not match its sparsity pattern");
  require(err != 4, CFX_ERR_INVALID_ARGUMENT, "assemble_matrix: a facet row does not join two cells across a shared facet");
  require(err == 0, CFX_ERR_RUNTIME, "assemble_matrix: the row gather reported an error");
}

template <int TDIM, int DEG>
int run_matrix(cfx_form_s* a, cfx_pattern_s* P, const int8_t* bc0, const int8_t* bc1, double* values, bool fresh)
{
  Stage1 st;
  bool combine_cuts = false;
  if constexpr (DEG == 2)
  {
    cfx_row_plan& plan0 = row_plan(a);
    const int mr0 = P->max_row_len;
    combine_cuts = P->split_plan == plan0.serial && mr0 > 64 && mr0 <= 256
                   && (plan0.n_special_rows.value() * 2 <= plan0.n_active_rows.value() || env_is<Sw::ROWS_SPLIT>('1'))
                   && plan0.n_special_rows.value() > 0
                   && p2_cut_tensors_ok(a);
  }
  RowArgs A = prepare<TDIM, DEG>(a, st, combine_cuts);
  A.fresh = fresh ? 1 : 0;
  A.bc0 = bc0; A.bc1 = bc1; A.indptr = P->indptr.p; A.indices = P->indices.p; A.values = values;
  ErrorFlag err(CFX_ERR_RUNTIME, kEntryMissing, raise_gather_error);
  A.error = err.p;
  bool lazy_zero = false;
  auto fill_all = [&]() { if (fresh) dev_fill(values, 0, sizeof(double) * (size_t)P->nnz.cap()); };
  if constexpr (DEG > 1)
  {
    cfx_row_plan& pl = row_plan(a);
    (void)pl.n_active_rows.value(); (void)pl.n_special_rows.value(); (void)pl.n_plain_rows.value();
    A.n_active = pl.n_active_rows;
  }
  if (A.n_active.cap == 0) fill_all();
  if (A.n_active.cap > 0)
  {
    const bool det = deterministic();
    const int mr = P->max_row_len;
    cfx_row_plan& plan = row_plan(a);
#define CFX_ROWS(GG, CAPP, NAME, ARGS)                                                                    \
// ... 336 lines not shown
    if (A.n_active.cap > 0)
    {
    if (mr <= 32) CFX_BLOCK(8, 32);
    else if (mr <= 128) CFX_BLOCK(16, 128);
    else CFX_BLOCK(32, 256);
    }
#undef CFX_BLOCK_V
#undef CFX_BLOCK
  }
  return err.deferred ? 0 : read_scalar(err.p);
}

#ifndef CFX_VEC_PLAIN_G
#define CFX_VEC_PLAIN_G 4
#endif
#ifndef CFX_VEC_BLOCK_G
#define CFX_VEC_BLOCK_G 1
#endif
template <int G>
__global__ void __launch_bounds__(kWave) assemble_vec_plain_kernel(DevN n_plain_d, const int32_t* __restrict__ rows,
                                                                   const int64_t* __restrict__ d2c_off,
                                                                   const int32_t* __restrict__ t2off,
                                                                   const double* __restrict__ t2, double* __restrict__ b)
{
  const int64_t n_plain = dev_n(n_plain_d);
  const int lane = threadIdx.x, gl = lane % G;
  const int64_t i = (int64_t)blockIdx.x * (kWave / G) + lane / G;
  const bool live = i < n_plain;
  const int64_t r = live ? rows[i] : 0;
  const int nc = live ? (int)(d2c_off[r + 1] - d2c_off[r]) : 0;
  const int64_t o = live ? (int64_t)t2off[r] - 1 : -1;
  double part = 0.0;
  if (o >= 0)
  {
    constexpr int Q = 8;
    double v[Q];
#pragma unroll
    for (int q = 0; q < Q; ++q)
    {
      const int k = gl + q * G;
      v[q] = k < nc ? t2[o + k] : 0.0;
    }
#pragma unroll
    for (int q = 0; q < Q; ++q) part += v[q];
    for (int k = gl + Q * G; k < nc; k += G) part += t2[o + k];
  }
#pragma unroll
  for (int d = G / 2; d >= 1; d >>= 1) part += __shfl_xor(part, d, G);
  if (live && gl == 0 && o >= 0) b[r] += part;
}

struct LatticeSource
{
  const uint8_t* diagpos;
  const double* x;
  double T[8];
  double field, scale;
  unsigned long long* written;
};

template <bool LATTICE>
__global__ void __launch_bounds__(kBlock) assemble_vec_plain_groups_kernel(DevN n_plain_d, const int32_t* __restrict__ rows,
                                                                           const uint8_t* __restrict__ corners,
                                                                           const int32_t* __restrict__ t2off,
                                                                           const double* __restrict__ t2, int64_t cap,
                                                                           double* __restrict__ b, LatticeSource Ls)
{
  if constexpr (!LATTICE)
  {
    const int64_t i = (int64_t)blockIdx.x * kBlock + threadIdx.x;
    if (i >= dev_n(n_plain_d) || i >= cap) return;
    const int64_t r = rows[i];
    if (t2off[r] == 0) return;
    const unsigned m = corners[r];
    double v[8];
#pragma unroll
    for (int k = 0; k < 8; ++k) v[k] = (m >> k) & 1u ? t2[k * cap + i] : 0.0;
    double sum = v[0];
#pragma unroll
    for (int k = 1; k < 8; ++k) sum += v[k];
    b[r] += sum;
  }
  else
  {
    const int64_t n = min(dev_n(n_plain_d), cap);
    int n_closed = 0;
    for (int64_t i = (int64_t)blockIdx.x * kBlock + threadIdx.x; i < n; i += (int64_t)gridDim.x * kBlock)
    {
      const int64_t r = rows[i];
      const int32_t off = t2off[r];
      if (lattice_source_row(off, Ls.diagpos[r]))
      {
        double xr[3], S[3], C[3];
        load_vertex<3>(Ls.x, r, xr);
#pragma unroll
        for (int d = 0; d < 3; ++d) cfx_sincospi(xr[d], S[d], C[d]);
        const double fscale = Ls.scale * ((int)Ls.field == CFX_F_POISSON_RHS ? 3.0 * kPi * kPi : 1.0);
        double vy[2];
#pragma unroll
        for (int sx = 0; sx < 2; ++sx)
        {
          double vz[2];
#pragma unroll
          for (int sy = 0; sy < 2; ++sy) vz[sy] = fma(Ls.T[sx + 2 * sy + 4], C[2], Ls.T[sx + 2 * sy] * S[2]);
          vy[sx] = fma(vz[1], C[1], vz[0] * S[1]);
        }
        b[r] += fscale * fma(vy[1], C[0], vy[0] * S[0]);
        ++n_closed;
      }
      else if (off != 0)
      {
        const unsigned m = corners[r];
        double v[8];
#pragma unroll
        for (int k = 0; k < 8; ++k) v[k] = (m >> k) & 1u ? t2[k * cap + i] : 0.0;
        double sum = v[0];
#pragma unroll
        for (int k = 1; k < 8; ++k) sum += v[k];
        b[r] += sum;
      }
    }
    __shared__ int s_closed;
    if (threadIdx.x == 0) s_closed = 0;
    __syncthreads();
#pragma unroll
    for (int o = 32; o > 0; o >>= 1) n_closed += __shfl_xor(n_closed, o, 64);
    if (threadIdx.x % 64 == 0 && n_closed) atomicAdd(&s_closed, n_closed);
    __syncthreads();
    if (threadIdx.x == 0 && s_closed) atomicAdd(Ls.written, (unsigned long long)s_closed);
  }
}

struct BlockChoice { bool use, merged; };
template <int DEG>
BlockChoice vec_block_choice(cfx_form_s* L, cfx_row_plan& plan, int slot, int count)
{
  const char e = env_char<Sw::VEC_BLOCKS>();
  if (e == '0' || count > 1 || L->V->bs != 1 || !plan.usable) return {false, false};
  for (const auto& I : L->integrals)
    if (user_integrand_known(I.kernel)) return {false, false};
  const bool series = count == 1 && source_series_ok<DEG>(L->V, L->integrals[plan.cell_slot_integral[slot]]);
  if (series && e != '2')
  {
    if (env_on<Sw::VEC_ROWORDER>() && plain_vec_offsets(L, (uint8_t)(1u << slot))) return {false, false};
  }
  return {true, !series};
}

template <int TDIM, int DEG>
void run_vector(cfx_form_s* L, double* b)
{
  Stage1 st;
  cfx_row_plan& plan = row_plan(L);
  int slot = -1, count = 0;
  for (int s = 0; s < plan.n_cell_slots; ++s)
    if (L->integrals[plan.cell_slot_integral[s]].n_entities.cap() > 0) { slot = s; ++count; }
  const uint8_t std_mark = count == 1 ? (uint8_t)(1u << slot) : (uint8_t)0;
  uint8_t rule_marks = 0;
  for (int s = 0; s < plan.n_cell_slots; ++s)
  {
    const cfx_integral_dev& I = L->integrals[plan.cell_slot_integral[s]];
    if (I.rules && I.rules->nr.cap() > 0) rule_marks |= (uint8_t)(16u << s);
  }
  const BlockChoice bc = vec_block_choice<DEG>(L, plan, slot, count);
  if (bc.use && (std_mark | rule_marks) != 0 && vec_block_plan(L, (uint8_t)(std_mark | rule_marks), bc.merged))
    st.vec_blocks = true;
  if constexpr (DEG == 1)
  {
    bool has_user = false;
    for (const auto& I : L->integrals) has_user = has_user || user_integrand_known(I.kernel);
    if (!st.vec_blocks && count == 1 && L->V->bs == 1 && plan.usable && env_on<Sw::VEC_ROWORDER>() && !has_user
        && plain_vec_offsets(L, (uint8_t)(1u << slot)))
    {
      st.t2.alloc(plan.vec_groups ? 8 * plan.vec_group_cap : plan.vec_t2_total.cap());
      st.vec_t2 = st.t2.p;
      if (plan.vec_groups && env_is<Sw::STAGING_NAN>('1')) dev_fill(st.t2.p, 0xff, sizeof(double) * (size_t)(8 * plan.vec_group_cap));
      if (plan.vec_groups && env_on<Sw::LATTICE_SOURCE>() && space_lattice(L->V).lat_rows > 0)
      {
        st.lat_src_T = lattice_source_moments(L->V, L->integrals[plan.cell_slot_integral[slot]].qdegree);
        if (st.lat_src_T) st.lat_src = space_stencil(L->V).diagpos.p;
      }
    }
  }
  RowArgs A = prepare<TDIM, DEG>(L, st);
  A.values = b;
  if (st.vec_blocks)
  {
    st.part.alloc(plan.vb_total);
    vec_block_partials<TDIM, DEG>(L, count == 1 ? &L->integrals[plan.cell_slot_integral[slot]] : nullptr, std_mark, A, st.part.p);
    if (plan.n_active_rows.cap() > 0 && plan.vb_total > 0)
    {
      const VecBlocks& S = space_vec_blocks(L->V);
      constexpr int G = CFX_VEC_BLOCK_G;
      launch("vec_blocks_rows", vec_blocks_rows_kernel<G>, row_grid((plan.n_active_rows.cap() + (kWave / G) - 1) / (kWave / G)), dim3(kWave),
             0, plan.n_active_rows, plan.active_rows.p, S.p_off.p, S.p_pos.p, plan.vb_base.p, st.part.p, b);
    }
    return;
  }
  if constexpr (DEG == 1)
  {
    const Stencil& stn = space_stencil(L->V);
    if (stn.usable) { A.slot4 = stn.slot4.p; A.diagpos = stn.diagpos.p; }
  }
  else
  {
    const Stencil& stn = space_stencil_slotn(L->V);
    if (stn.slotn_ok && L->V->bs == 1) A.slotn = stn.slotn.p;
  }
  if (st.vec_t2)
  {
    constexpr int G = CFX_VEC_PLAIN_G;
    LatticeSource Ls{};
    if (st.lat_src)
    {
      const cfx_integral_dev& I = L->integrals[plan.cell_slot_integral[slot]];
      Ls.diagpos = st.lat_src; Ls.x = L->V->mesh->x.p; Ls.field = I.params[0]; Ls.scale = I.params[1];
      for (int s = 0; s < 8; ++s) Ls.T[s] = st.lat_src_T[s];
      Ls.written = space_stencil(L->V).lat_src_written.p;
    }
    if (plan.vec_groups && st.lat_src)
      launch("assemble_vec_plain", assemble_vec_plain_groups_kernel<true>,
             dim3(std::min(grid_for(plan.n_plain_rows.cap()).x, 2048u)), dim3(kBlock), 0,
             plan.n_plain_rows, plan.plain_rows.p, L->V->mesh->hex_corners.p, plan.vec_t2off.p, st.vec_t2, plan.vec_group_cap, b, Ls);
    else if (plan.vec_groups)
      launch("assemble_vec_plain", assemble_vec_plain_groups_kernel<false>, grid_for(plan.n_plain_rows.cap()), dim3(kBlock), 0,
             plan.n_plain_rows, plan.plain_rows.p, L->V->mesh->hex_corners.p, plan.vec_t2off.p, st.vec_t2, plan.vec_group_cap, b, Ls);
    else
      launch("assemble_vec_plain", assemble_vec_plain_kernel<G>,
             dim3((unsigned)((plan.n_plain_rows.cap() + (kWave / G) - 1) / (kWave / G))), dim3(kWave), 0, plan.n_plain_rows,
             plan.plain_rows.p, A.d2c_off, plan.vec_t2off.p, st.vec_t2, b);
    A.n_active = plan.n_special_rows; A.active_rows = plan.special_rows.p;
    if (plan.n_vec_odd_rows.cap() > 0)
    {
      RowArgs O = A;
      O.n_active = plan.n_plain_rows; O.active_rows = plan.plain_rows.p;
      O.vec_skip = plan.vec_t2off.p; O.vec_n_odd = plan.n_vec_odd_rows;
      launch("assemble_vec_rows", assemble_vec_rows_kernel<TDIM, DEG, CFX_VEC_G>,
             row_grid((O.n_active.cap + (kWave / CFX_VEC_G) - 1) / (kWave / CFX_VEC_G)), dim3(kWave), 0, O);
    }
  }
  if (A.n_active.cap > 0)
    launch("assemble_vec_rows", assemble_vec_rows_kernel<TDIM, DEG, CFX_VEC_G>,
           row_grid((A.n_active.cap + (kWave / CFX_VEC_G) - 1) / (kWave / CFX_VEC_G)), dim3(kWave), 0,
           A);
}

}

namespace
{
__global__ void __launch_bounds__(kWave) lattice_tile_rows_kernel(int64_t t, int64_t ndofs, const int64_t* __restrict__ st_off,
                                                                  int32_t* __restrict__ rows, unsigned long long* __restrict__ masks,
                                                                  uint8_t* __restrict__ uniform, int32_t* __restrict__ first_id)
{
  const int lane = threadIdx.x;
  const int64_t r = t * kRowTile + lane;
  if (lane < kRowTile && r < ndofs)
  {
    const int len = (int)(st_off[r + 1] - st_off[r]);
    rows[lane] = (int32_t)r;
    masks[lane] = len >= 64 ? ~0ull : (1ull << len) - 1ull;
    uniform[lane] = 1;
  }
  if (lane == 0) { first_id[0] = 0; first_id[1] = (int32_t)t; }
}
}

namespace cfx
{

bool lattice_template(cfx_space_s* V)
{
  Stencil& S = const_cast<Stencil&>(space_lattice(V));
  if (S.lat_rows <= 0) return false;
  if (S.lat_tmpl_built) return S.lat_tmpl != nullptr;
  const int tcls = tile_class(S);
  const int tdim = V->mesh->tdim;
  if (tcls < 0 || (tdim != 2 && tdim != 3)) { S.lat_tmpl_built = true; return false; }
  const Adjacency& adj = V->dof_cells();
  const int64_t t = S.lat_rstar / kRowTile;
  const int64_t nrows = std::min<int64_t>(kRowTile, V->ndofs - t * kRowTile);
  DevArray<int32_t> rows(kRowTile), first_id(2);
  DevArray<unsigned long long> masks(kRowTile);
  DevArray<uint8_t> uniform(kRowTile);
  ZeroFlag err;
  S.lat_scratch.alloc(std::max(S.max_tile_st, 1));
  S.lat_scratch.zero();
  launch("lattice_template", lattice_tile_rows_kernel, dim3(1), dim3(kWave), 0, t, V->ndofs, S.offsets.p, rows.p, masks.p,
         uniform.p, first_id.p);
  TileArgs T{};
  T.x = V->mesh->x.p; T.n_tiles = DevN(1); T.tile_first = first_id.p; T.tile_id = first_id.p + 1;
  T.n_plain = DevN(nrows); T.rows = rows.p; T.masks = masks.p; T.uniform = uniform.p;
  T.d2c_off = adj.offsets.p; T.d2c = adj.cells.p; T.slot4 = S.slot4.p; T.cellmark = nullptr;
  T.st_off = S.offsets.p; T.st_nbr = S.nbr.p; T.st_loc = S.st_loc.p; T.diagpos = S.diagpos.p;
  T.tile_voff = S.tile_voff.p; T.tile_verts = S.tile_verts.p;
  T.indptr = S.offsets.p;
  T.values = reinterpret_cast<double*>(reinterpret_cast<uintptr_t>(S.lat_scratch.p) - sizeof(double) * (uintptr_t)S.lat_sb0);
  T.bc0 = nullptr; T.bc1 = nullptr; T.inline_bits = 1u; T.fresh = 1; T.error = err.p; T.ndofs = V->ndofs;
  T.lat_len = 0; T.stream_blocks = 0; T.lat_tmpl = nullptr; T.lat_written = nullptr;
  const dim3 gt = row_grid(1);
  if (tdim == 3 && tcls == 0) launch("lattice_template", assemble_tiles_plain_kernel<3, true, 0>, gt, dim3(kWave), 0, T);
  else if (tdim == 3) launch("lattice_template", assemble_tiles_plain_kernel<3, true, 1>, gt, dim3(kWave), 0, T);
  else if (tcls == 0) launch("lattice_template", assemble_tiles_plain_kernel<2, true, 0>, gt, dim3(kWave), 0, T);
  else launch("lattice_template", assemble_tiles_plain_kernel<2, true, 1>, gt, dim3(kWave), 0, T);
  S.lat_tmpl = S.lat_scratch.p + S.lat_rel;
  S.lat_tmpl_built = true;
  publish_across_lanes();
  return true;
}

bool source_groups_ok(cfx_form_s* L, uint8_t mark)
{
  if (!env_on<Sw::SOURCE_GROUPS>()) return false;
  cfx_space_s* V = L->V;
  if (!V->mesh->hex_groups || V->mesh->tdim != 3 || V->degree != 1 || V->bs != 1 || mark == 0 || (mark & 0x0Fu) != mark)
    return false;
  cfx_row_plan& plan = row_plan(L);
  const int slot = __builtin_ctz(mark);
  if ((mark & (mark - 1)) != 0 || slot >= plan.n_cell_slots) return false;
  const cfx_integral_dev& I = L->integrals[plan.cell_slot_integral[slot]];
  if (user_integrand_known(I.kernel) || !source_series_ok<1>(V, I) || I.n_entities.cap() == 0) return false;
  const ListProvenance* pv = provenance_lookup(I.entities.p);
  return pv && pv->n == I.n_entities.key() && pv->cut->gen == pv->gen && pv->cut->mesh == V->mesh;
}

struct Rect2Slot
{
  int kernel, qdegree;
  double scale;
  uint8_t std_bit, rule_bit;
  DevN nr;
  const int32_t* offsets;
  const int32_t* parent_map;
  const double* points;
  const double* weights;
  const int32_t* rule_keys;
  const int32_t* rule_first;
  unsigned rule_mask;
// ... 335 lines not shown
```

cutfemx_amd/csrc/cfx_rowasm.hip:

```cpp
#include <cmath>
#include <cstdlib>


#include "cfx_elem.h"

using namespace cfx;

namespace
{

constexpr int kWave = 64;

__global__ void plan_mark_cells_kernel(DevN n_d, const int32_t* __restrict__ cells, int stride, uint8_t bit,
                                       uint8_t* mark)
{
  const int64_t n = dev_n(n_d);
  const int64_t i = (int64_t)blockIdx.x * blockDim.x + threadIdx.x;
  if (i >= n) return;
  const int64_t c = cells[i * stride];
  mark[c] = mark[c] | bit;
}

__global__ void __launch_bounds__(kBlock) plan_pack_bits_kernel(int64_t ncells, const uint8_t* __restrict__ mark, uint8_t bit,
                                                                unsigned long long* __restrict__ words,
// ... 2408 lines not shown
           adj.offsets.p, counts.p, (const int64_t*)nullptr, staged.p, S.st_loc.p, maxima.p);
  }
  else
    launch("stencil_tiles", stencil_tiles_kernel<0>, grid, dim3(kWave), 0, V->ndofs, ntiles, S.offsets.p, S.nbr.p,
           adj.offsets.p, counts.p, (const int64_t*)nullptr, (int32_t*)nullptr, (uint16_t*)nullptr, maxima.p);
  const std::vector<int> mx = download(maxima.p, 3);
  S.max_tile_verts = mx[0]; S.max_tile_st = mx[1]; S.max_tile_items = mx[2];
  if (S.max_tile_st > kTileMaxSt) { staged.release(); return S; }
  S.tile_voff.alloc(ntiles + 1);
  exclusive_scan(counts.p, S.tile_voff.p, ntiles);
  const int64_t n_verts = read_scalar(S.tile_voff.p + ntiles);
  if (tail && S.arena.p + S.arena_used + (((int64_t)sizeof(int32_t) * n_verts + 255) & ~255LL) > tail) S.tile_verts.alloc(n_verts);
  else S.take(S.tile_verts, n_verts);
  if (staged.p && S.max_tile_verts <= kTileStage)
  {
    launch("stencil_tiles_write", stencil_tiles_pack_kernel, grid_for(ntiles * kWave), dim3(kBlock), 0, ntiles, counts.p,
           S.tile_voff.p, staged.p, S.tile_verts.p);
    staged.release();
  }
  else
  {
    staged.release();
    if (!S.st_loc.p) S.take(S.st_loc, S.nbr.n);
    launch("stencil_tiles_write", stencil_tiles_kernel<1>, grid, dim3(kWave), 0, V->ndofs, ntiles, S.offsets.p, S.nbr.p,
           adj.offsets.p, (int32_t*)nullptr, S.tile_voff.p, S.tile_verts.p, S.st_loc.p, maxima.p);
  }
  S.tiles_usable = true;
  publish_across_lanes();
  return S;
}

__global__ void __launch_bounds__(kBlock) lattice_maxc_kernel(int64_t ndofs, const int64_t* __restrict__ d2c_off,
                                                              unsigned long long* __restrict__ info)
{
  const int64_t r = (int64_t)blockIdx.x * kBlock + threadIdx.x;
  int c = r < ndofs ? (int)(d2c_off[r + 1] - d2c_off[r]) : 0;
#pragma unroll
  for (int o = 32; o > 0; o >>= 1) c = max(c, __shfl_xor(c, o, 64));
  if (threadIdx.x % kWave == 0 && (unsigned long long)c > *reinterpret_cast<volatile unsigned long long*>(&info[0]))
    atomicMax(&info[0], (unsigned long long)c);
}

__global__ void __launch_bounds__(kBlock) lattice_pick_kernel(int64_t ndofs, const int64_t* __restrict__ d2c_off,
                                                              const int64_t* __restrict__ st_off,
                                                              unsigned long long* __restrict__ info)
{
  __shared__ int s_hit;
  const int64_t maxc = (int64_t)info[0];
  const int64_t start = ndofs / 2;
  for (int64_t base = 0; base < ndofs; base += kBlock)
  {
    if (threadIdx.x == 0) s_hit = kBlock;
    __syncthreads();
    const int64_t k = base + threadIdx.x;
    const int64_t r = k < ndofs ? (start + k) % ndofs : -1;
    if (r >= 0 && d2c_off[r + 1] - d2c_off[r] == maxc) atomicMin(&s_hit, (int)threadIdx.x);
    __syncthreads();
    const int hit = s_hit;
    if (hit < kBlock)
    {
      if ((int)threadIdx.x == hit)
      {
        const int64_t r0 = r / kRowTile * kRowTile;
        info[1] = (unsigned long long)r;
        info[4] = (unsigned long long)st_off[r0];
        info[5] = (unsigned long long)st_off[r];
        info[6] = (unsigned long long)(st_off[r + 1] - st_off[r]);
      }
      return;
    }
    __syncthreads();
  }
}

__global__ void __launch_bounds__(kBlock) lattice_flag_kernel(int64_t ndofs, const int64_t* __restrict__ d2c_off,
                                                              const uint32_t* __restrict__ slot4,
                                                              const int64_t* __restrict__ st_off, const int32_t* __restrict__ nbr,
                                                              const double* __restrict__ x, uint8_t* __restrict__ diagpos,
                                                              unsigned long long* __restrict__ info)
{
  const int64_t r = (int64_t)blockIdx.x * kBlock + threadIdx.x;
  const int64_t maxc = (int64_t)info[0], rs = (int64_t)info[1];
  bool ok = false, top = false;
  if (r < ndofs)
  {
    const int64_t cb = d2c_off[r], cs = d2c_off[rs];
    const int nc = (int)(d2c_off[r + 1] - cb), ncs = (int)(d2c_off[rs + 1] - cs);
    const int64_t sb = st_off[r], ss = st_off[rs];
    const int len = (int)(st_off[r + 1] - sb), lens = (int)(st_off[rs + 1] - ss);
    const unsigned d = diagpos[r];
    top = nc == maxc;
    ok = nc == ncs && len == lens && (d & kDiagPosMask) == (diagpos[rs] & kDiagPosMask);
    for (int t = 0; ok && t < nc; ++t) ok = slot4[cb + t] == slot4[cs + t];
    for (int k = 0; ok && k < len; ++k)
    {
      const int64_t v = nbr[sb + k], vs = nbr[ss + k];
      for (int c = 0; c < 3; ++c)
        ok = ok && __double_as_longlong(x[3 * v + c] - x[3 * r + c]) == __double_as_longlong(x[3 * vs + c] - x[3 * rs + c]);
    }
    diagpos[r] = (uint8_t)((d & kDiagPosMask) | (ok ? kLatFlag : 0u));
  }
  const int n_ok = __popcll(__ballot(ok)), n_top = __popcll(__ballot(top));
  if (threadIdx.x % kWave == 0)
  {
    if (n_ok) atomicAdd(&info[2], (unsigned long long)n_ok);
    if (n_top) atomicAdd(&info[3], (unsigned long long)n_top);
  }
}

__global__ void __launch_bounds__(kBlock) lattice_clear_kernel(int64_t ndofs, uint8_t* __restrict__ diagpos)
{
  const int64_t r = (int64_t)blockIdx.x * kBlock + threadIdx.x;
  if (r < ndofs) diagpos[r] &= (uint8_t)kDiagPosMask;
}

bool lattice_rows_on()
{
  return env_on<Sw::LATTICE_ROWS>();
}

const Stencil& space_lattice(cfx_space_s* V)
{
  Stencil& S = const_cast<Stencil&>(space_stencil_tiles(V));
  if (S.lat_built || !S.tiles_usable) return S;
  if (!lattice_rows_on() || V->ndofs < 1 || V->mesh->x.n < 3 * V->ndofs) { S.lat_built = true; return S; }
  const Adjacency& adj = V->dof_cells();
  DevArray<unsigned long long> info(8);
  info.zero();
  const dim3 grid = grid_for(V->ndofs, kBlock);
  launch("lattice_rows", lattice_maxc_kernel, grid, dim3(kBlock), 0, V->ndofs, adj.offsets.p, info.p);
  launch("lattice_rows", lattice_pick_kernel, dim3(1), dim3(kBlock), 0, V->ndofs, adj.offsets.p, S.offsets.p, info.p);
  launch("lattice_rows", lattice_flag_kernel, grid, dim3(kBlock), 0, V->ndofs, adj.offsets.p, S.slot4.p, S.offsets.p,
         S.nbr.p, V->mesh->x.p, S.diagpos.p, info.p);
  unsigned long long h[8];
  {
    unsigned long long* pin = static_cast<unsigned long long*>(pinned_scratch());
    CFX_HIP(hipMemcpyAsync(pin, info.p, sizeof(h), hipMemcpyDeviceToHost, ctx().stream));
    CFX_HIP(hipStreamSynchronize(ctx().stream));
    for (int k = 0; k < 8; ++k) h[k] = pin[k];
    ++sync_counter();
  }
  const int64_t flagged = (int64_t)h[2], top = (int64_t)h[3];
  if (2 * flagged < top || flagged == 0 || h[6] == 0 || h[6] > 63)
  {
    launch("lattice_rows", lattice_clear_kernel, grid, dim3(kBlock), 0, V->ndofs, S.diagpos.p);
    S.lat_rows = 0;
  }
  else
  {
    S.lat_written.alloc(1);
    S.lat_written.zero();
    S.lat_src_written.alloc(1);
    S.lat_src_written.zero();
    S.lat_rstar = (int64_t)h[1];
    S.lat_sb0 = (int64_t)h[4];
    S.lat_rel = (int)((int64_t)h[5] - (int64_t)h[4]);
    S.lat_len = (int)h[6];
    S.lat_rows = flagged;
  }
  S.lat_built = true;
  publish_across_lanes();
  return S;
}

__global__ void __launch_bounds__(kWave) lattice_star_kernel(int64_t rs, const int64_t* __restrict__ d2c_off,
                                                             const int32_t* __restrict__ d2c, const int32_t* __restrict__ conn,
                                                             const double* __restrict__ x, int max_cells, double* __restrict__ out)
{
  const int64_t cb = d2c_off[rs];
  const int nc = (int)(d2c_off[rs + 1] - cb), t = threadIdx.x;
  if (t == 0) out[0] = nc <= max_cells ? (double)nc : -1.0;
  if (t >= nc || nc > max_cells) return;
  const int64_t c = d2c[cb + t];
  double* o = out + 1 + 13 * t;
  int loc = -1;
  for (int i = 0; i < 4; ++i)
  {
    const int64_t v = conn[4 * c + i];
    if (v == rs) loc = i;
    for (int d = 0; d < 3; ++d) o[3 * i + d] = x[3 * v + d] - x[3 * rs + d];
  }
  o[12] = (double)loc;
}

const double* quad_points_host(int dim, int degree);
const double* quad_weights_host(int dim, int degree);
int quad_npoints(int dim, int degree);

const double* lattice_source_moments(cfx_space_s* V, int qdegree)
{
  Stencil& S = const_cast<Stencil&>(space_lattice(V));
  if (S.lat_rows <= 0 || S.lat_src_state < 0 || qdegree < 0 || qdegree > CFX_QUAD_MAX_DEGREE || qdegree >= Stencil::kLatSrcDegrees)
    return nullptr;
  if (S.lat_src_state == 0)
  {
    if (V->mesh->tdim != 3 || V->dofmap.p != V->mesh->conn.p) { S.lat_src_state = -1; return nullptr; }
    const Adjacency& adj = V->dof_cells();
    constexpr int kN = 1 + 13 * Stencil::kLatStarCells;
    DevArray<double> star(kN);
    launch("lattice_rows", lattice_star_kernel, dim3(1), dim3(kWave), 0, S.lat_rstar, adj.offsets.p, adj.cells.p,
           V->mesh->conn.p, V->mesh->x.p, (int)Stencil::kLatStarCells, star.p);
    static_assert(Stencil::kLatSrcDegrees == CFX_QUAD_MAX_DEGREE + 1, "one set of moments per degree of the tables");
    std::vector<double> h((size_t)kN);
    CFX_HIP(hipMemcpyAsync(h.data(), star.p, sizeof(double) * (size_t)kN, hipMemcpyDeviceToHost, ctx().stream));
    CFX_HIP(hipStreamSynchronize(ctx().stream));
    ++sync_counter();
    const int nc = (int)h[0];
    bool ok = nc > 0 && nc <= Stencil::kLatStarCells;
    for (int t = 0; ok && t < nc; ++t) ok = h[1 + 13 * t + 12] >= 0.0;
    if (!ok) { S.lat_src_state = -1; return nullptr; }
    S.lat_star.assign(h.begin() + 1, h.begin() + 1 + 13 * nc);
    S.lat_src_state = 1;
    publish_across_lanes();
  }
  if (!S.lat_src_T_built[qdegree])
  {
    const int npts = quad_npoints(3, qdegree);
    const double* pts = quad_points_host(3, qdegree);
    const double* wts = quad_weights_host(3, qdegree);
    const long double pi = 3.14159265358979323846264338327950288L;
    long double T[8] = {0, 0, 0, 0, 0, 0, 0, 0};
    const int nc = (int)(S.lat_star.size() / 13);
    for (int t = 0; t < nc; ++t)
    {
      const double* o = S.lat_star.data() + 13 * t;
      const int loc = (int)o[12];
      long double e[3][3];
      for (int k = 0; k < 3; ++k)
        for (int d = 0; d < 3; ++d) e[k][d] = (long double)o[3 * (k + 1) + d] - (long double)o[d];
      const long double det = e[0][0] * (e[1][1] * e[2][2] - e[1][2] * e[2][1]) - e[0][1] * (e[1][0] * e[2][2] - e[1][2] * e[2][0])
                              + e[0][2] * (e[1][0] * e[2][1] - e[1][1] * e[2][0]);
      const long double adet = det < 0 ? -det : det;
      for (int q = 0; q < npts; ++q)
      {
        const long double X[3] = {pts[3 * q], pts[3 * q + 1], pts[3 * q + 2]};
        const long double N = loc == 0 ? 1.0L - X[0] - X[1] - X[2] : X[loc - 1];
        long double sn[3], cs[3];
        for (int d = 0; d < 3; ++d)
        {
          const long double delta = (long double)o[d] + X[0] * e[0][d] + X[1] * e[1][d] + X[2] * e[2][d];
          sn[d] = sinl(pi * delta);
          cs[d] = cosl(pi * delta);
        }
        const long double wn = adet * (long double)wts[q] * N;
        for (int s = 0; s < 8; ++s)
          T[s] += wn * ((s & 1) ? sn[0] : cs[0]) * ((s & 2) ? sn[1] : cs[1]) * ((s & 4) ? sn[2] : cs[2]);
      }
    }
    for (int s = 0; s < 8; ++s) S.lat_src_T[qdegree][s] = (double)T[s];
    S.lat_src_T_built[qdegree] = true;
  }
  return S.lat_src_T[qdegree];
}

struct LatTileStart
{
  const int32_t* rows;
  const unsigned long long* masks;
  const uint8_t* uniform;
  const uint8_t* diagpos;
  unsigned long long full;
  unsigned bits;
  __device__ bool templ(int64_t i) const
  {
    return lattice_template_row(diagpos[rows[i]], uniform[i], masks[i], bits, full);
  }
  __device__ bool operator()(int64_t i) const
  {
    if (templ(i)) return false;
    const int32_t t = rows[i] / kRowTile;
    for (int64_t j = i - 1; j >= 0 && rows[j] / kRowTile == t; --j)
      if (!templ(j)) return false;
    return true;
  }
};

bool plain_lattice_tiles(cfx_form_s* a, unsigned inline_bits)
{
  cfx_row_plan& plan = row_plan(a);
  if (plan.lat_tiles_built) return plan.lat_bits == inline_bits && plan.lat_bits != 0;
  const Stencil& S = space_lattice(a->V);
  if (S.lat_rows <= 0 || !plan.plain_masks_built || plan.plain_masks.n == 0 || plan.n_plain_tiles.cap() == 0) return false;
  DevArray<int32_t> first;
  TileIdEmit emit{plan.plain_rows.p, nullptr};
  bool emitted = false;
  auto pre = [&](int64_t cap) { plan.lat_tile_id.alloc(cap); emit.ids = plan.lat_tile_id.p; emitted = true; };
  const LatTileStart pred{plan.plain_rows.p, plan.plain_masks.p, plan.plain_uniform.p, S.diagpos.p,
                          (1ull << S.lat_len) - 1ull, inline_bits};
  plan.n_lat_tiles = compact_count("plan_plain_tiles", "plan.lattice_tiles", plan.n_plain_rows.devn(), pred, first, &emit, pre);
  plan.lat_tile_first = std::move(first);
  if (!emitted && plan.n_lat_tiles.cap() > 0)
  {
    plan.lat_tile_id.alloc(plan.n_lat_tiles.cap());
    launch("plan_plain_tiles", tile_ids_kernel, grid_for(plan.n_lat_tiles.cap()), dim3(kBlock), 0, plan.n_lat_tiles,
           plan.lat_tile_first.p, plan.plain_rows.p, plan.lat_tile_id.p);
  }
  plan.lat_bits = inline_bits;
  plan.lat_tiles_built = true;
  publish_across_lanes();
  return inline_bits != 0;
}

bool space_dof_verts(cfx_space_s* V)
{
  if (V->dof_verts_built) return V->dof_verts_ok;
  V->dof_verts_built = true;
  const int tdim = V->mesh->tdim, nd = tdim == 3 ? 10 : 6;
  if (V->degree != 2 || V->ndofs_cell != nd || (tdim != 2 && tdim != 3)) return false;
  V->dof_verts.alloc(2 * V->ndofs);
  dev_fill(V->dof_verts.p, 0xff, sizeof(int32_t) * 2 * (size_t)V->ndofs);
  launch("space_dof_verts", dof_verts_kernel, grid_for(V->mesh->ncells * nd), dim3(kBlock), 0, V->mesh->ncells, tdim,
         V->mesh->conn.p, V->dofmap.p, V->dof_verts.p);
  V->dof_verts_ok = true;
  publish_across_lanes();
  return true;
}

const Stencil& space_stencil_slotn(cfx_space_s* V)
{
  Stencil& S = const_cast<Stencil&>(space_stencil(V));
  if (S.slotn_built) return S;
  S.slotn_built = true;
  if (!env_on<Sw::P2_PLAIN>() || !S.lists || S.usable || V->degree != 2 || V->ndofs_cell > 10 || S.max_len > 255)
    return S;
  const Adjacency& adj = V->dof_cells();
  S.slotn.alloc(adj.cells.n * 12);
  S.slotn.zero();
  launch("stencil_slotn", stencil_slotn_kernel, wave_grid((V->ndofs + 3) / 4), dim3(kWave), 0, V->ndofs, adj.offsets.p,
         adj.cells.p, V->dofmap.p, V->ndofs_cell, S.offsets.p, S.nbr.p, S.slotn.p);
  S.slotn_ok = true;
  publish_across_lanes();
  return S;
}

bool plain_row_masks(cfx_form_s* a, int32_t* counts, int* maxlen)
{
  cfx_row_plan& plan = row_plan(a);
  if (plan.plain_masks_built) return false;
  plan.plain_masks_built = true;
  cfx_space_s* V = a->V;
  const Stencil& st = space_stencil(V);
  const int64_t np = plan.n_plain_rows.key();
  if (!st.usable || np == 0 || !plan.any_cells) return false;
  const Adjacency& adj = V->dof_cells();
  plan.plain_masks.alloc(np);
  plan.plain_uniform.alloc(np);
  launch("plan_plain_masks", plain_masks_kernel,
         dim3((unsigned)((np + kWave - 1) / kWave)), dim3(kWave), 0,
         plan.n_plain_rows, plan.plain_rows.p, adj.offsets.p, adj.cells.p, st.slot4.p, plan.cellmark.p, V->ndofs_cell,
         st.offsets.p, plan.plain_masks.p, plan.plain_uniform.p, counts, maxlen, plan.bulk ? plan.rowcls.p : (const uint8_t*)nullptr,
         plan.bulk_bits);
  if (space_stencil_tiles(V).tiles_usable)
  {
    DevArray<int32_t> first;
    TileIdEmit emit{plan.plain_rows.p, nullptr};
    bool emitted = false;
    auto pre = [&](int64_t cap) { plan.plain_tile_id.alloc(cap); emit.ids = plan.plain_tile_id.p; emitted = true; };
    unsigned lat_bits = 0;
    if (a->rank == 2 && lattice_rows_on())
    {
      for (int sl = 0; sl < plan.n_cell_slots && sl < 4; ++sl)
      {
        const cfx_integral_dev& I = a->integrals[plan.cell_slot_integral[sl]];
        if (I.kernel == CFX_K_STIFFNESS && I.coefficient.n == 0 && I.coefficients.empty()) lat_bits |= 1u << sl;
      }
    }
    const Stencil* lat = lat_bits ? &space_lattice(V) : nullptr;
    if (lat && lat->lat_rows > 0)
    {
      DevArray<int32_t> lfirst;
      TileIdEmit lemit{plan.plain_rows.p, nullptr};
      const LatTileStart lpred{plan.plain_rows.p, plan.plain_masks.p, plan.plain_uniform.p, lat->diagpos.p,
                               (1ull << lat->lat_len) - 1ull, lat_bits};
      const char* const sites[2] = {"plan.plain_tiles", "plan.lattice_tiles"};
      Count totals[2];
      compact_count_pair("plan_plain_tiles", sites, plan.n_plain_rows.devn(), TileStart{plan.plain_rows.p}, lpred, emit, lemit,
                         first, lfirst, totals, [&](int64_t ca, int64_t cb)
                         {
                           plan.plain_tile_id.alloc(ca); emit.ids = plan.plain_tile_id.p;
                           plan.lat_tile_id.alloc(cb); lemit.ids = plan.lat_tile_id.p;
                         });
      plan.n_plain_tiles = totals[0]; plan.n_lat_tiles = totals[1];
      plan.plain_tile_first = std::move(first);
      plan.lat_tile_first = std::move(lfirst);
      plan.lat_tiles_built = true; plan.lat_bits = lat_bits;
      publish_across_lanes();
      return counts != nullptr;
    }
    plan.n_plain_tiles = compact_count("plan_plain_tiles", "plan.plain_tiles", plan.n_plain_rows.devn(),
                                       TileStart{plan.plain_rows.p}, first, &emit, pre);
    plan.plain_tile_first = std::move(first);
    if (!emitted)
    {
      plan.plain_tile_id.alloc(plan.n_plain_tiles.cap());
      launch("plan_plain_tiles", tile_ids_kernel, grid_for(plan.n_plain_tiles.cap()), dim3(kBlock), 0, plan.n_plain_tiles,
             plan.plain_tile_first.p, plan.plain_rows.p, plan.plain_tile_id.p);
    }
  }
  publish_across_lanes();
  return counts != nullptr;
}

__global__ void __launch_bounds__(kBlock) plan_cut_first_kernel(int64_t nr, const int32_t* __restrict__ parent,
                                                                const unsigned long long* __restrict__ bits,
                                                                const int32_t* __restrict__ rank, int32_t* __restrict__ first)
{
  const int64_t e = (int64_t)blockIdx.x * kBlock + threadIdx.x;
  if (e >= nr) return;
  const int32_t c = parent[e];
  if (e > 0 && parent[e - 1] == c) return;
  const int64_t w = c >> 6;
  first[(int64_t)rank[w] + __popcll(bits[w] & ((1ull << (c & 63)) - 1ull))] = (int32_t)e;
}

struct ByteRuleMark
{
  __device__ bool operator()(uint8_t v) const { return (v & 0xF0u) != 0; }
};

void plan_cut_cells(cfx_form_s* a)
{
  cfx_row_plan& plan = row_plan(a);
  if (plan.cut_cells_built) return;
  plan.cut_cells_built = true;
  const int64_t nc = a->V->mesh->ncells;
  plan.n_cut_cells = compact_bytes("plan_cut_cells", nc, plan.cellmark.p, ByteRuleMark{}, plan.cut_cells);
  const int64_t n_cut_cells = plan.n_cut_cells;
  const int64_t nwords = (nc + 63) / 64;
  plan.cut_bits.alloc(nwords);
  plan.cut_rank.alloc(nwords + 1);
  DevArray<int32_t> pop(nwords);
  launch("plan_pack_bits", plan_pack_bits_kernel, grid_for(nwords), dim3(kBlock), 0, nc, plan.cellmark.p, (uint8_t)0xF0u,
         reinterpret_cast<unsigned long long*>(plan.cut_bits.p), pop.p, (int32_t*)nullptr);
  exclusive_scan(pop.p, plan.cut_rank.p, nwords);
  for (int slot = 0; slot < plan.n_cell_slots; ++slot)
  {
    const cfx_integral_dev& I = a->integrals[plan.cell_slot_integral[slot]];
    const int64_t nrl = I.rules ? I.rules->nr.value() : 0;
    if (nrl == 0 || n_cut_cells == 0) continue;
    plan.cut_first[slot].alloc(n_cut_cells);
    dev_fill(plan.cut_first[slot].p, 0xff, sizeof(int32_t) * (size_t)n_cut_cells);
    launch("plan_cut_cells", plan_cut_first_kernel, grid_for(nrl), dim3(kBlock), 0, nrl, I.rules->parent_map.p,
           reinterpret_cast<const unsigned long long*>(plan.cut_bits.p), plan.cut_rank.p, plan.cut_first[slot].p);
  }
  publish_across_lanes();
}

__global__ void vec_plain_len_kernel(DevN n_plain_d, int64_t n_scan, const int32_t* __restrict__ rows,
                                     const int64_t* __restrict__ d2c_off, const uint8_t* __restrict__ uniform, uint8_t mark,
                                     int64_t* __restrict__ len)
{
  const int64_t n_plain = dev_n(n_plain_d);
  const int64_t i = (int64_t)blockIdx.x * blockDim.x + threadIdx.x;
  if (i >= n_plain)
  {
    if (i < n_scan) len[i] = 0;
    return;
  }
  const int64_t r = rows[i];
  const int64_t l = uniform[i] == mark ? d2c_off[r + 1] - d2c_off[r] : 0;
  len[i] = l > 0 ? l : (1ll << 32);
}

__global__ void vec_plain_scatter_kernel(DevN n_plain_d, const int32_t* __restrict__ rows, const int64_t* __restrict__ off,
                                         int32_t* __restrict__ t2off, bool by_row)
{
  const int64_t n_plain = dev_n(n_plain_d);
  const int64_t i = (int64_t)blockIdx.x * blockDim.x + threadIdx.x;
  if (i < n_plain && (off[i + 1] & 0xffffffffll) > (off[i] & 0xffffffffll))
    t2off[rows[i]] = (by_row ? (int32_t)i : (int32_t)(off[i] & 0xffffffffll)) + 1;
}


__global__ void __launch_bounds__(kBlock) vec_plain_offsets_chained_kernel(DevN n_plain_d, const int32_t* __restrict__ rows,
                                                                           const int64_t* __restrict__ d2c_off,
                                                                           const uint8_t* __restrict__ uniform, uint8_t mark,
                                                                           int32_t* __restrict__ t2off, bool by_row,
                                                                           ChainState chain, int64_t* __restrict__ total_out,
                                                                           CountJobs after)
{
  const int64_t n_plain = dev_n(n_plain_d);
  const unsigned int tile = chain_take_tile(chain.ticket);
  const int64_t base = (int64_t)tile * kTile + (int64_t)threadIdx.x * kScanItems;
  int32_t r[kScanItems];
  int64_t l[kScanItems], s = 0;
#pragma unroll
  for (int k = 0; k < kScanItems; ++k)
  {
    const int64_t i = base + k;
    r[k] = 0; l[k] = 0;
    if (i < n_plain)
    {
      r[k] = rows[i];
      const int64_t len = uniform[i] == mark ? d2c_off[(int64_t)r[k] + 1] - d2c_off[r[k]] : 0;
      l[k] = len > 0 ? len : (1ll << 32);
    }
    s += l[k];
  }
  int64_t total;
  const int64_t local = block_exclusive_scan<int64_t>(s, total);
  const int64_t prefix = (int64_t)chain_exclusive_prefix(chain.state, tile, (unsigned long long)total);
  int64_t off = prefix + local;
#pragma unroll
  for (int k = 0; k < kScanItems; ++k)
  {
    if ((l[k] & 0xffffffffll) > 0) t2off[r[k]] = (by_row ? (int32_t)(base + k) : (int32_t)(off & 0xffffffffll)) + 1;
    off += l[k];
  }
  if (tile == gridDim.x - 1 && threadIdx.x == kBlock - 1)
  {
    *total_out = prefix + total;
    if (after.n > 0) count_publish(after);
  }
}

__global__ void gather_i32_kernel(DevN n_d, const int32_t* __restrict__ idx, const int32_t* __restrict__ src,
                                  int32_t* __restrict__ dst)
{
  const int64_t n = dev_n(n_d);
  const int64_t i = (int64_t)blockIdx.x * blockDim.x + threadIdx.x;
  if (i < n) dst[i] = src[idx[i]];
}

bool plain_vec_offsets(cfx_form_s* L, uint8_t mark)
{
  cfx_row_plan& plan = row_plan(L);
  const bool groups = source_groups_ok(L, mark);
  if (plan.vec_fast >= 0 && plan.vec_mark == mark && plan.vec_groups == groups) return plan.vec_fast == 1;
  plan.vec_mark = mark;
// ... 818 lines not shown
```

cutfemx_amd/csrc/cfx_switches.h:

```cpp
#pragma once

#include <cstdlib>
#include <cstring>

#define CFX_SWITCHES(CFX_SWITCH)                                                                                                   \
  CFX_SWITCH(DETERMINISTIC,      first_char, call,  "1: lane-ordered LDS accumulation instead of LDS atomics: bitwise reproducible matrices") \
  CFX_SWITCH(ASSEMBLY,           string,     call,  "atomic: the entity-parallel FP64-atomic kernels instead of the row gather") \
  CFX_SWITCH(STENCIL,            first_char, build, "0: no mesh-static row stencil (P1): hashed sparsity, searching gather") \
  CFX_SWITCH(STENCIL_LISTS,      first_char, build, "0: no neighbour lists for the other spaces (degree 2, vector-valued, DG)") \
  CFX_SWITCH(STENCIL_STAGED,     first_char, build, "0: two-pass stencil rows and tiles, the build a card short of memory takes (so does a tile whose union outgrows its staging row; tests reach both through this switch alone)") \
  CFX_SWITCH(TILES,              first_char, build, "0: no row tiles") \
  CFX_SWITCH(LATTICE_ROWS,       first_char, build, "0: no lattice flags and no template: every plain row is computed by the tile kernel") \
  CFX_SWITCH(LATTICE_SOURCE,     first_char, call,  "0: the P1 series source term of the lattice rows hex by hex instead of its closed form per row") \
  CFX_SWITCH(P2_PLAIN,           first_char, build, "0: degree 2 without the slot-record kernel") \
  CFX_SWITCH(P2_CLOSED,          first_char, call,  "0: degree 2 stages uncut tensors instead of closed-form rows") \
  CFX_SWITCH(P2_MOMENTS,         first_char, call,  "0: degree 2 stages cut-cell stiffness tensors instead of moments") \
  CFX_SWITCH(P2_CUT_TENSORS,     first_char, call,  "0: per-integral rule tensors and moments instead of one tensor per cut cell") \
  CFX_SWITCH(P2_INTERFACE,       first_char, call,  "0: the general gather kernel for the degree-2 interface rows") \
  CFX_SWITCH(FACET_FOLD_STAGE1,  first_char, call,  "0: full facet tensors staged, folded in the gather; 2: folded tensors but no rank-one records") \
  CFX_SWITCH(BLOCK_PLAIN,        first_char, call,  "0: vector spaces without the dof-at-a-time kernel") \
  CFX_SWITCH(BLOCK_GATHER,       first_char, call,  "0: block spaces by the entity-parallel kernels instead of the block gather") \
  CFX_SWITCH(ROWS_SPLIT,         first_char, call,  "1: split plain / interface rows whatever their share (small meshes of the kernel-path tests)") \
  CFX_SWITCH(VEC_BLOCKS,         first_char, call,  "0 / 2: linear forms never / always by cell block (also read when a space builds its cell blocks)") \
  CFX_SWITCH(VEC_ROWORDER,       first_char, call,  "0: the P1 series source term without the row-ordered staging") \
  CFX_SWITCH(SOURCE_SERIES,      first_char, call,  "0: the P1 source term by quadrature instead of its series") \
  CFX_SWITCH(SOURCE_GROUPS,      first_char, call,  "0: the P1 series source term cell by cell instead of one hex per lane") \
  CFX_SWITCH(STAGING_NAN,        first_char, call,  "1 (tests): the hex-corner planes of the staging start as NaN") \
  CFX_SWITCH(PLAIN_STAGE,        first_char, call,  "0: plain rows without LDS staging, the form that meshes with stencils longer than 32 take by themselves") \
  CFX_SWITCH(MFMA,               first_char, call,  "0: generic rows instead of the MFMA kernel for staged elasticity tensors") \
  CFX_SWITCH(CUT_TENSORS_P1,     first_char, call,  "0: the generic tensors of cut P1 cells") \
  CFX_SWITCH(RECT_GATHER,        first_char, call,  "0: rectangular blocks by the entity-parallel atomic kernel") \
  CFX_SWITCH(BULK_ROWS,          first_char, call,  "0: row plans take their marks from the entity lists, not from the classification") \
  CFX_SWITCH(PATTERN_REUSE,      first_char, call,  "0: never copy rows from the space's previous pattern") \
  CFX_SWITCH(IMPLICIT_BOX,       first_char, call,  "1: classification of generated box meshes from the cube index") \
  CFX_SWITCH(CLASSIFY_CULL,      first_char, call,  "0: classification cell by cell instead of block culling") \
  CFX_SWITCH(STEP_SPECULATE,     first_char, call,  "0: steps publish nothing, every size is read back where it is produced") \
  CFX_SWITCH(FUSED_TILES,        integer,    once,  "n: count + offsets + write of a sync-free step as one chained launch up to n tiles (default 512; 0: three launches)") \
  CFX_SWITCH(SCAN_CHAINED_TILES, integer,    once,  "n: scans up to n tiles in one chained launch (default 8192), longer ones in three") \
  CFX_SWITCH(COUNT_SYNC,         first_char, once,  "1: count the size read-backs; 2: also name each by the launch before it") \
  CFX_SWITCH(STEP_DEBUG,         present,    once,  "trace the sites of a step, their capacities and what voided it") \
  CFX_SWITCH(PLAN_DEBUG,         present,    call,  "print row-class counts of plans and patterns") \
  CFX_SWITCH(LAUNCH_TRACE,       present,    once,  "every kernel launch (name, grid) on stderr") \
  CFX_SWITCH(LAUNCH_SYNC,        present,    once,  "a stream synchronisation behind every launch: a fault surfaces at its own kernel") \
  CFX_SWITCH(ALLOC_TRACE,        present,    once,  "every hipMalloc of the block cache with its duration")

namespace cfx
{

enum class Sw : int
{
#define CFX_SWITCH(NAME, kind, when, effect) NAME,
  CFX_SWITCHES(CFX_SWITCH)
#undef CFX_SWITCH
};

namespace sw
{
enum Kind { first_char, present, integer, string };
enum When { call, build, once };
struct Entry { const char* name; Kind kind; When when; };
constexpr Entry kTable[] = {
#define CFX_SWITCH(NAME, kind, when, effect) {"CFX_" #NAME, kind, when},
  CFX_SWITCHES(CFX_SWITCH)
#undef CFX_SWITCH
};
template <Sw S, Kind K, bool Cached>
inline const char* raw()
{
  constexpr Entry e = kTable[(int)S];
  static_assert(e.kind == K, "switch read as another kind than the table gives it");
  static_assert((e.when == once) == Cached, "switch read at another time than the table gives it");
  return getenv(e.name);
}
}

template <Sw S> inline char env_char() { const char* e = sw::raw<S, sw::first_char, false>(); return e ? e[0] : '\0'; }
template <Sw S> inline bool env_is(char c) { return env_char<S>() == c; }
template <Sw S> inline bool env_on() { return !env_is<S>('0'); }
template <Sw S> inline bool env_present() { return sw::raw<S, sw::present, false>() != nullptr; }
template <Sw S> inline bool env_equals(const char* v) { const char* e = sw::raw<S, sw::string, false>(); return e && strcmp(e, v) == 0; }

template <Sw S> inline char env_char_once() { static const char c = []() { const char* e = sw::raw<S, sw::first_char, true>(); return e ? e[0] : '\0'; }(); return c; }
template <Sw S> inline bool env_present_once() { static const bool on = sw::raw<S, sw::present, true>() != nullptr; return on; }
template <Sw S> inline long long env_int_once(long long dflt) { static const long long v = [&]() { const char* e = sw::raw<S, sw::integer, true>(); return e ? atoll(e) : dflt; }(); return v; }

}
```

cutfemx_amd/fem.py:

```python
from __future__ import annotations

import ctypes as C
from dataclasses import dataclass, field

import numpy as np

from . import _lib

_C128, _C64 = np.dtype(np.complex128), np.dtype(np.complex64)


def _is_complex(dt) -> bool:
    return dt is not None and np.dtype(dt) in (_C128, _C64)


def _cfn(name: str, dt):
    return getattr(_lib.lib(), f"cfx_{name}_{'c64' if np.dtype(dt) == _C64 else 'c128'}")

from .cut import FacetRows, RuntimeQuadratureRules
from .mesh import FunctionSpace

MASS, STIFFNESS, NITSCHE, GHOST_GRADJUMP, ELASTICITY = (_lib.K_MASS, _lib.K_STIFFNESS, _lib.K_NITSCHE,
                                                        _lib.K_GHOST_GRADJUMP, _lib.K_ELASTICITY)
EXTENSION_L2 = _lib.K_EXTENSION_L2
# ... 42 lines not shown
        if part == "re":
            self._keep = keep
        else:
            self._keep_im = keep
        itype = _lib.CELL
        ent_ptr, n_ent = None, 0
        if self.facets is None and self.rules is not None and self.rules.host_width == 4 and (
                self.kernel in (_lib.K_GHOST_GRADJUMP, _lib.K_JUMP, _lib.K_SIP) or self.kernel in _user_integrand_facet):
            itype = _lib.INTERIOR_FACET
        if self.facets is not None:
            itype = _lib.INTERIOR_FACET
            if isinstance(self.facets, FacetRows):
                ent_ptr, n_ent = C.c_void_p(self.facets.ptr), self.facets.size
                keep.append(self.facets)
            elif _lib.is_torch(self.facets):
                ent_ptr, n_ent = _lib.as_ptr(self.facets, np.int32, keep), int(self.facets.numel() // 4)
            else:
                rows = np.ascontiguousarray(self.facets, dtype=np.int32).reshape(-1, 4)
                ent_ptr, n_ent = _lib.as_ptr(rows, np.int32, keep), rows.shape[0]
        elif self.cells is not None:
            if isinstance(self.cells, tuple):
                ent_ptr, n_ent = C.c_void_p(self.cells[0]), int(self.cells[1])
                keep.append(self.cells)
            else:
                ent_ptr = _lib.as_ptr(self.cells, np.int32, keep)
                n_ent = int(keep[-1].numel() if _lib.is_torch(keep[-1]) else keep[-1].size)
        pd, stride = None, 0
        if self.point_data is not None:
            pdata = self.point_data
            stride = 1 if pdata.ndim == 1 else int(pdata.shape[1])
            pd = _f64_ptr(pdata, keep)
        params = (C.c_double * 8)(*([float(v) for v in self.params] + [0.0] * (8 - len(self.params))))
        coeff = None
        if self.coefficient is not None:
            values = self._coefficient_values()
            if self._complex_coefficient():
                values = np.ascontiguousarray(np.real(values) if part == "re" else np.imag(values), dtype=np.float64)
            coeff = _f64_ptr(values, keep)
        return _lib.Integral(itype, self.kernel, int(self.qdegree), stride, ent_ptr, n_ent,
                             self.rules._h if self.rules is not None else None, pd, params, coeff)


class _Widened:

    def __init__(self, ptr, n):
        p = C.c_void_p()
        _lib.check(_lib.lib().cfx_widen_f32(C.c_void_p(ptr), C.c_int64(n), C.byref(p)))
        self.ptr = p.value

    def __del__(self):
        try:
            if self.ptr:
                _lib.load().cfx_device_free(C.c_void_p(self.ptr))
                self.ptr = None
        except Exception:
            pass


def _f64_ptr(a, keep: list):
    if _lib.scalar_dtype(a) == np.float32 and _lib.is_device(a):
        n = a.size if isinstance(a, _lib.DeviceBuffer) else int(a.numel())
        w = _Widened(a.ptr if isinstance(a, _lib.DeviceBuffer) else a.contiguous().data_ptr(), n)
        keep.append(w)
        return C.c_void_p(w.ptr)
    return _lib.as_ptr(a, np.float64, keep)


def _coefficient_list(functions, keep: list):
    functions = tuple(functions)
    for f in functions:
        if not hasattr(f, "function_space") or not hasattr(f, "values"):
            raise TypeError("coefficients: a list of Functions (each with its function_space and values)")
        v = f.values
        if v.is_complex() if _lib.is_torch(v) else _is_complex(v.dtype) if isinstance(v, _lib.DeviceBuffer) else np.iscomplexobj(v):
            raise ValueError("coefficients: complex Functions in a coefficient list are not supported (the Functions of a "
                             "list are real; a complex constant goes into Integral.scale)")
    arr = (_lib.Coefficient * max(len(functions), 1))()
    for k, f in enumerate(functions):
        W = f.function_space
        v = f.values
        n = v.size if isinstance(v, _lib.DeviceBuffer) else int(v.numel()) if _lib.is_torch(v) else np.asarray(v).size
        if n != W.ndofs * W.bs:
            raise ValueError(f"coefficients[{k}]: {n} values for a space of {W.ndofs} dofs x block size {W.bs}")
        arr[k].space = W._h.value
        arr[k].values = _f64_ptr(f.values, keep).value
        keep.append(W)
    return len(functions), arr


class CutForm:

    def __init__(self, V: FunctionSpace, integrals, rank: int, trial_space: FunctionSpace | None = None, dtype=None):
        self.function_space, self.rank = V, rank
        self.trial_space = V if trial_space is None else trial_space
        self.integrals = list(integrals)
        cplx = any(isinstance(i.scale, complex) and i.scale.imag != 0.0 for i in self.integrals) \
            or any(i._complex_coefficient() for i in self.integrals)
        if dtype is not None and np.dtype(dtype) not in (np.dtype(np.float64), np.dtype(np.float32), _C128, _C64):
            raise TypeError("forms are float64 (float32 containers), complex128 or complex64")
        if cplx and dtype is not None and not _is_complex(dtype):
            raise TypeError("a complex constant or coefficient needs dtype=complex128 (or complex64)")
        self.dtype = np.dtype(dtype) if _is_complex(dtype) else (_C128 if cplx else np.dtype(np.float64))
        self._scaled = any(complex(i.scale) != 1.0 for i in self.integrals)
        if self._scaled and not _is_complex(self.dtype):
            raise TypeError("Integral.scale belongs to complex forms (fold a real constant into `params`)")
        self._h_im = None

        if self.trial_space is not V:
            for i in self.integrals:
                cs = getattr(i.coefficient, "function_space", None)
                if i.kernel in _user_integrand_two and cs is not None and cs is not V:
                    raise ValueError("cfx_form_create2: the coefficient of a registered two-space integrand must be a "
                                     "Function of the test space (it is packed with the test space's dofmap)")

        def create(part):
            arr = (_lib.Integral * len(self.integrals))(*[i._cstruct(part) for i in self.integrals])
            h = C.c_void_p()
            if self.trial_space is not V:
                if rank != 2:
                    raise ValueError("a trial space goes with a bilinear form")
                _lib.check(_lib.lib().cfx_form_create2(V._h, self.trial_space._h, len(self.integrals), arr, C.byref(h)))
            else:
                _lib.check(_lib.lib().cfx_form_create(V._h, rank, len(self.integrals), arr, C.byref(h)))
            return h
        self._h = None
        self._h = create("re")
        if any(i._complex_coefficient() for i in self.integrals):
            self._h_im = create("im")
        self._coefficient_keep: dict = {}
        for k, i in enumerate(self.integrals):
            if len(tuple(i.coefficients)) > 0:
                self.set_coefficients(k, i.coefficients)

    def set_coefficients(self, integral_index: int, functions) -> None:
        keep: list = []
        n, arr = _coefficient_list(functions, keep)
        handles = [self._h] + ([self._h_im] if self._h_im is not None else [])
        for h in handles:
            _lib.check(_lib.lib().cfx_form_set_coefficients(h, int(integral_index), n, arr))
        self._coefficient_keep[int(integral_index)] = keep

    def _parts(self):
        n = len(self.integrals)
        s = np.array([complex(i.scale) for i in self.integrals])
        out = [(self._h, (C.c_double * (2 * n))(*np.column_stack([s.real, s.imag]).ravel()))]
        if self._h_im is not None:
            t = np.array([1j * complex(i.scale) if i._complex_coefficient() else 0.0 for i in self.integrals])
            out.append((self._h_im, (C.c_double * (2 * n))(*np.column_stack([t.real, t.imag]).ravel())))
        return out

    def prepare(self):
        _lib.check(_lib.lib().cfx_form_prepare(self._h))
        return self

    def __del__(self):
        try:
            if self._h:
                _lib.load().cfx_form_destroy(self._h)
                self._h = None
            if getattr(self, "_h_im", None):
                _lib.load().cfx_form_destroy(self._h_im)
                self._h_im = None
        except Exception:
            pass


class overlap:

    def __enter__(self):
        _lib.check(_lib.lib().cfx_overlap_begin())
        return self

    def side(self, fn):
        _lib.check(_lib.lib().cfx_overlap_side(1))
        try:
            return fn()
        finally:
            _lib.check(_lib.lib().cfx_overlap_side(0))

    def __exit__(self, *exc):
        _lib.check(_lib.lib().cfx_overlap_end())
        return False


_user_integrand_rank: dict[int, int] = {}
_user_integrand_two: set[int] = set()
_user_integrand_facet: set[int] = set()


def _coefficient_signature(coefficients):
    sig = [(int(c[0]), int(c[1]) if len(c) > 1 else 1) for c in coefficients]
    nd = (C.c_int * max(len(sig), 1))(*[c[0] for c in sig])
    bs = (C.c_int * max(len(sig), 1))(*[c[1] for c in sig])
    return sig, nd, bs


def _coefficient_defaults(sig) -> str:
    lines, off = ["#ifndef CFX_NCOEF", f"#define CFX_NCOEF {len(sig)}",
                  f"#define CFX_CSTRIDE {sum(n * b for n, b in sig)}"], 0
    for k, (n, b) in enumerate(sig):
        lines += [f"#define CFX_W_ND{k} {n}", f"#define CFX_W_BS{k} {b}", f"#define CFX_W_OFF{k} {off}"]
        off += n * b
    return "\n".join(lines + ["#endif", ""])


def register_integrand(name: str, source: str, rank: int = 2, facet: bool = False, variant=None, trial=None,
                       coefficients=None) -> int:
    if coefficients is not None and len(coefficients) > 0:
        sig, _, _ = _coefficient_signature(coefficients)
        if variant is None:
            variant = (3, 4, 1)
        kid = register_integrand(name, _coefficient_defaults(sig) + source, rank, facet, variant, trial)
        if kid in _user_integrand_two:
            v = list(variant) + ([1] if len(variant) < 3 else [])
            t = v[3:5] if len(v) >= 5 else (list(trial) + [1])[:2]
            compile_integrand2(kid, v[0], v[1], v[2], t[0], t[1], coefficients=sig)
        else:
            tdim, nd, bs = (list(variant) + [1])[:3]
            compile_integrand(kid, tdim, nd, bs, coefficients=sig)
        return kid
    kid = C.c_int()
    two = trial is not None or (variant is not None and len(variant) == 5)
    if two:
        if rank != 2:
            raise ValueError("register_integrand: an integrand between two spaces is bilinear")
        if variant is None:
            raise ValueError("register_integrand: `trial` goes with `variant=(tdim, nd0[, bs0])`")
        if trial is not None:
            if len(variant) > 3:
                raise ValueError("register_integrand: give the trial space either in `variant` or in `trial`")
            tdim, nd0, bs0 = (list(variant) + [1])[:3]
            nd1, bs1 = (list(trial) + [1])[:2]
        else:
            tdim, nd0, bs0, nd1, bs1 = variant
        _lib.check(_lib.load().cfx_integrand_register2(name.encode(), source.encode(), int(bool(facet)), int(tdim), int(nd0),
                                                       int(bs0), int(nd1), int(bs1), C.byref(kid)))
        _user_integrand_rank[kid.value] = 2
        _user_integrand_two.add(kid.value)
        return kid.value
    if rank not in (0, 1, 2):
        raise ValueError("register_integrand: rank must be 0, 1 or 2")
    if variant is None and facet and rank == 0:
        variant = (3, 4, 1)
    if variant is None and not facet:
        _lib.check(_lib.load().cfx_integrand_register(name.encode(), source.encode(), int(rank), C.byref(kid)))
    elif variant is None:
        _lib.check(_lib.load().cfx_integrand_register_facet(name.encode(), source.encode(), C.byref(kid)))
    else:
        tdim, nd, bs = (list(variant) + [1])[:3]
        _lib.check(_lib.load().cfx_integrand_register_variant(name.encode(), source.encode(), int(rank), int(bool(facet)),
                                                              int(tdim), int(nd), int(bs), C.byref(kid)))
    _user_integrand_rank[kid.value] = int(rank)
    if facet and rank == 0:
        _user_integrand_facet.add(kid.value)
    return kid.value


def compile_integrand(kernel_id: int, tdim: int, ndofs_cell: int, bs: int = 1, coefficients=None) -> None:
    if coefficients is not None and len(coefficients) > 0:
        sig, nd, cbs = _coefficient_signature(coefficients)
        _lib.check(_lib.load().cfx_integrand_compile_coefficients(int(kernel_id), int(tdim), int(ndofs_cell), int(bs), 0, 0,
                                                                  len(sig), nd, cbs))
        return
    _lib.check(_lib.load().cfx_integrand_compile_bs(int(kernel_id), int(tdim), int(ndofs_cell), int(bs)))


def compile_integrand2(kernel_id: int, tdim: int, nd0: int, bs0: int, nd1: int, bs1: int, coefficients=None) -> None:
    if coefficients is not None and len(coefficients) > 0:
        sig, nd, cbs = _coefficient_signature(coefficients)
        _lib.check(_lib.load().cfx_integrand_compile_coefficients(int(kernel_id), int(tdim), int(nd0), int(bs0), int(nd1),
                                                                  int(bs1), len(sig), nd, cbs))
        return
    _lib.check(_lib.load().cfx_integrand_compile2(int(kernel_id), int(tdim), int(nd0), int(bs0), int(nd1), int(bs1)))


def form(integrals, V: FunctionSpace, rank: int | None = None, trial_space: FunctionSpace | None = None, dtype=None) -> CutForm:
    integrals = list(integrals)
    if rank is None:
        ranks = {_user_integrand_rank[i.kernel] if i.kernel in _user_integrand_rank
                 else (2 if i.kernel < 100 else 1 if i.kernel < 200 else 0) for i in integrals}
        if len(ranks) != 1:
            raise ValueError("all integrals of a form must have the same rank")
        rank = ranks.pop()
    return CutForm(V, integrals, rank, trial_space, dtype)


class MatrixCSR:

    def __init__(self, pattern_handle, V: FunctionSpace, values=None, dtype=None):
        self._p = pattern_handle
        self.function_space = V
        self.dtype = np.dtype(_lib.scalar_dtype(values) if dtype is None else dtype)
        if self.dtype not in (np.dtype(np.float32), np.dtype(np.float64), _C128, _C64):
            raise TypeError("MatrixCSR holds float64, float32, complex128 or complex64 values")
        v = _lib.PatternView()
        _lib.check(_lib.lib().cfx_pattern_view_get(self._p, C.byref(v)))
        self._view = v
        self.nrows, self.ncols = int(v.nrows), int(v.ncols)
        self._nnz_pending = _lib._step_open
        self._nnz = int(v.nnz)
        self._owns_values = values is None
        self._zero_pending = False
        if values is None:
            p = C.c_void_p()
            _lib.check(_lib.lib().cfx_device_alloc(C.byref(p), C.c_size_t(self.dtype.itemsize * max(self.nnz, 1))))
            self._vptr = p.value
# ... 736 lines not shown
```

cutfemx_amd/mesh.py:

```python
from __future__ import annotations

import ctypes as C

import numpy as np

from . import _lib

KUHN_TET = np.array([[0, 1, 3, 7], [0, 1, 5, 7], [0, 2, 3, 7], [0, 2, 6, 7], [0, 4, 5, 7], [0, 4, 6, 7]])
KUHN_TRI = np.array([[0, 1, 3], [0, 3, 2]])


def box_mesh_arrays(tdim: int, n: int, lower=None, upper=None):
    n1 = n + 1
    lo = np.zeros(tdim) if lower is None else np.asarray(lower, dtype=np.float64)
    hi = np.ones(tdim) if upper is None else np.asarray(upper, dtype=np.float64)
    axes = [np.arange(n1, dtype=np.float64) / n * (hi[d] - lo[d]) + lo[d] for d in range(tdim)]
    x = np.zeros((n1 ** tdim, 3))
    if tdim == 2:
        yy, xx = np.meshgrid(axes[1], axes[0], indexing="ij")
        x[:, 0], x[:, 1] = xx.ravel(), yy.ravel()
        iy, ix = np.meshgrid(np.arange(n), np.arange(n), indexing="ij")
        ix, iy = ix.ravel(), iy.ravel()
        corner = np.stack([(ix + (i & 1)) + n1 * (iy + ((i >> 1) & 1)) for i in range(4)], axis=1)
        conn = corner[:, KUHN_TRI].reshape(-1, 3)
# ... 12 lines not shown

    def __init__(self, handle, tdim, gdim, nnodes, ncells, keep=()):
        self._h = handle
        self.tdim, self.gdim = tdim, gdim
        self.num_nodes, self.num_cells = int(nnodes), int(ncells)
        self._keep = list(keep)
        self.dtype = np.dtype(np.float64)

    @classmethod
    def from_arrays(cls, tdim: int, x, conn) -> "Mesh":
        keep: list = []
        nnodes = x.shape[0]
        ncells = conn.shape[0]
        stride = conn.shape[1]
        h = C.c_void_p()
        if _lib.scalar_dtype(x) == np.float32:
            _lib.check(_lib.lib().cfx_mesh_create_f32(tdim, tdim, C.c_int64(nnodes), _lib.as_ptr(x, np.float32, keep),
                                                      C.c_int64(ncells), _lib.as_ptr(conn, np.int32, keep), stride,
                                                      C.byref(h)))
            m = cls(h, tdim, tdim, nnodes, ncells, [k for k in keep[1:] if _lib.is_device(k)])
            m.dtype = np.dtype(np.float32)
            return m
        _lib.check(_lib.lib().cfx_mesh_create(tdim, tdim, C.c_int64(nnodes), _lib.as_ptr(x, np.float64, keep),
                                              C.c_int64(ncells), _lib.as_ptr(conn, np.int32, keep), stride,
                                              C.byref(h)))
        return cls(h, tdim, tdim, nnodes, ncells, [k for k in keep if _lib.is_device(k)])

    @classmethod
    def create_box(cls, tdim: int, n: int) -> "Mesh":
        h = C.c_void_p()
        _lib.check(_lib.lib().cfx_mesh_create_box(tdim, n, C.byref(h)))
        nn, nc = C.c_int64(), C.c_int64()
        _lib.check(_lib.lib().cfx_mesh_info(h, None, None, C.byref(nn), C.byref(nc), None, None))
        return cls(h, tdim, tdim, nn.value, nc.value)

    @classmethod
    def create_slab(cls, n: int, z0: int, nz: int) -> "Mesh":
        h = C.c_void_p()
        _lib.check(_lib.lib().cfx_mesh_create_slab(n, z0, nz, C.byref(h)))
        nn, nc = C.c_int64(), C.c_int64()
        _lib.check(_lib.lib().cfx_mesh_info(h, None, None, C.byref(nn), C.byref(nc), None, None))
        return cls(h, 3, 3, nn.value, nc.value)

    def _info(self):
        x, conn = C.c_void_p(), C.c_void_p()
        _lib.check(_lib.lib().cfx_mesh_info(self._h, None, None, None, None, C.byref(x), C.byref(conn)))
        return x.value, conn.value

    @property
    def x_ptr(self) -> int:
        return self._info()[0]

    @property
    def conn_ptr(self) -> int:
        return self._info()[1]

    @property
    def x(self) -> np.ndarray:
        return _lib.download(self.x_ptr, self.num_nodes * 3, np.float64).reshape(-1, 3)

    @property
    def conn(self) -> np.ndarray:
        return _lib.download(self.conn_ptr, self.num_cells * (self.tdim + 1), np.int32).reshape(-1, self.tdim + 1)

    def __del__(self):
        try:
            if self._h:
                _lib.load().cfx_mesh_destroy(self._h)
                self._h = None
        except Exception:
            pass


_EDGES = {2: [(1, 2), (0, 2), (0, 1)], 3: [(2, 3), (1, 3), (1, 2), (0, 3), (0, 2), (0, 1)]}


def lagrange_dofmap(tdim: int, conn: np.ndarray, num_nodes: int, degree: int):
    conn = np.asarray(conn)
    if degree == 1:
        return np.ascontiguousarray(conn, dtype=np.int32), int(num_nodes)
    edges = np.stack([np.sort(conn[:, list(e)], axis=1) for e in _EDGES[tdim]], axis=1)
    key = edges[..., 0].astype(np.int64) * num_nodes + edges[..., 1]
    uniq, inv = np.unique(key.ravel(), return_inverse=True)
    edge_dofs = inv.reshape(key.shape) + num_nodes
    dofmap = np.concatenate([conn, edge_dofs], axis=1)
    return np.ascontiguousarray(dofmap, dtype=np.int32), int(num_nodes + uniq.size)


def box_lagrange2_dofmap(mesh: "Mesh", n: int, device=None, chunk: int = 1 << 24):
    import torch

    from .dist import as_torch
    device = torch.device("cuda", torch.cuda.current_device()) if device is None else device
    s = n + 1
    nn, nc = mesh.num_nodes, mesh.num_cells
    conn = as_torch(mesh.conn_ptr, nc * 4, "int32", device).view(nc, 4)
    table = torch.tensor([1, s, s * s, 1 + s, 1 + s * s, s + s * s, 1 + s + s * s], device=device, dtype=torch.int32)
    out = torch.empty((nc, 10), device=device, dtype=torch.int32)
    out[:, :4] = conn
    for lo in range(0, nc, chunk):
        c = conn[lo:lo + chunk]
        for k, (p, q) in enumerate(_EDGES[3]):
            a = torch.minimum(c[:, p], c[:, q])
            d = (c[:, p] - c[:, q]).abs()
            direction = (d[:, None] == table[None, :]).to(torch.int32).argmax(dim=1).to(torch.int32)
            out[lo:lo + chunk, 4 + k] = nn + 7 * a + direction
    return out, 8 * nn


class FunctionSpace:

    def __init__(self, mesh: Mesh, degree: int = 1, dofmap=None, ndofs: int | None = None, bs: int = 1):
        self.mesh, self.degree, self.bs = mesh, degree, bs
        keep: list = []
        if dofmap is None:
            if degree == 1:
                self.ndofs, self.ndofs_cell = mesh.num_nodes, mesh.tdim + 1
                ptr = C.c_void_p(mesh.conn_ptr)
            else:
                dm, nd = lagrange_dofmap(mesh.tdim, mesh.conn, mesh.num_nodes, degree)
                self.ndofs, self.ndofs_cell = nd, dm.shape[1]
                ptr = _lib.as_ptr(dm, np.int32, keep)
                self._host_dofmap = dm
        else:
            self.ndofs, self.ndofs_cell = int(ndofs), dofmap.shape[1]
            ptr = _lib.as_ptr(dofmap, np.int32, keep)
        self._keep = [k for k in keep if _lib.is_device(k)] + [mesh]
        self._h = C.c_void_p()
        _lib.check(_lib.lib().cfx_space_create(mesh._h, degree, bs, C.c_int64(self.ndofs), ptr, self.ndofs_cell,
                                               C.byref(self._h)))
        self._dofmap_ptr = ptr

    def static_table_bytes(self) -> dict:
        b = (C.c_int64 * 4)()
        _lib.check(_lib.lib().cfx_space_static_bytes(self._h, b))
        return dict(dof_cells=int(b[0]), row_stencil=int(b[1]), row_tiles=int(b[2]), cell_neighbours=int(b[3]))

    def _lattice(self):
        n, w = C.c_int64(0), C.c_int64(0)
        _lib.check(_lib.lib().cfx_space_lattice_rows(self._h, C.byref(n), C.byref(w)))
        return int(n.value), int(w.value)

    def lattice_rows(self) -> int:
        return self._lattice()[0]

    def lattice_template_rows(self) -> int:
        return self._lattice()[1]

    def lattice_source_rows(self) -> int:
        n = C.c_int64(0)
        _lib.check(_lib.lib().cfx_space_lattice_source_rows(self._h, C.byref(n)))
        return int(n.value)

    @property
    def dofmap(self) -> np.ndarray:
        if hasattr(self, "_host_dofmap"):
            return self._host_dofmap
        if self.degree == 1:
            return self.mesh.conn
        raise RuntimeError("dofmap was supplied by the caller")

    def __del__(self):
        try:
            if self._h:
                _lib.load().cfx_space_destroy(self._h)
                self._h = None
        except Exception:
            pass


class Function:

    def __init__(self, V: FunctionSpace, values=None, name: str = "f"):
        self.function_space = V
        self.name = name
        self.values = np.zeros(V.ndofs * V.bs) if values is None else values

    def interpolate(self, f):
        if self.function_space.degree != 1:
            raise NotImplementedError("interpolate is provided for P1 spaces")
        x = self.function_space.mesh.x
        self.values = np.ascontiguousarray(f(x.T), dtype=np.float64)
```

include/cutfemx_amd.h:

```cpp
#ifndef CUTFEMX_AMD_H
#define CUTFEMX_AMD_H

#include <stddef.h>
#include <stdint.h>

#ifdef __cplusplus
extern "C" {
#endif

#define CFX_OK 0
#define CFX_ERR_INVALID_ARGUMENT (-1)
#define CFX_ERR_RUNTIME (-2)
#define CFX_ERR_OUT_OF_RANGE (-3)
#define CFX_ERR_HIP (-4)
#define CFX_ERR_STEP_VOID (-5)

#define CFX_INSIDE (-1)
#define CFX_INTERSECTED 0
#define CFX_OUTSIDE 1

#define CFX_CELL 0
#define CFX_EXTERIOR_FACET 1
#define CFX_INTERIOR_FACET 2

// ... 26 lines not shown
typedef struct cfx_form_s* cfx_form_t;
typedef struct cfx_pattern_s* cfx_pattern_t;
typedef struct cfx_active_s* cfx_active_t;
typedef struct cfx_aggregation_s* cfx_aggregation_t;

typedef struct
{
  int32_t cut_approximation_order;
  int32_t max_refinement_iterations;
  int32_t edge_max_depth;
  int32_t reserved;
} cfx_cut_options;

typedef struct
{
  int32_t tdim;
  int32_t gdim;
  int64_t nq;
  int64_t nr;
  const double* points;
  const double* weights;
  const int32_t* offsets;
  const int32_t* parent_map;
  int32_t host_width;
  int32_t reserved;
  const int32_t* host_rows;
  const int32_t* host_verts;
} cfx_rules_view;

typedef struct
{
  int32_t type;
  int32_t kernel;
  int32_t qdegree;
  int32_t point_stride;
  const int32_t* entities;
  int64_t n_entities;
  cfx_rules_t rules;
  const double* point_data;
  double params[8];
  const double* coefficient;
} cfx_integral;

typedef struct
{
  int64_t nrows;
  int64_t nnz;
  const int64_t* indptr;
  const int32_t* indices;
  int64_t ncols;
} cfx_pattern_view;

int cfx_init(int device);
const char* cfx_last_error(void);
int cfx_set_stream(void* hip_stream);
int cfx_synchronize(void);
int cfx_overlap_begin(void);
int cfx_overlap_side(int side);
int cfx_overlap_end(void);
int cfx_step_begin(const char* key);
int cfx_step_end(int* redo, int64_t* published, int64_t* read_back);
int cfx_step_resolve(void);
int cfx_step_abort(void);
int cfx_step_set_margin(double factor, int64_t slack);
int cfx_step_forget(const char* key);
int cfx_list_count(const void* list, int64_t n_given, int64_t* n);
int cfx_sync_count(int64_t* n);
int cfx_copy(void* dst, const void* src, size_t bytes);
int cfx_device_alloc(void** ptr, size_t bytes);
int cfx_device_free(void* ptr);
int cfx_device_cache_release(void);
int cfx_device_memory_stats(size_t* in_use, size_t* cached, size_t* peak, int reset_peak);
int cfx_device_memset(void* ptr, int byte, size_t bytes);
int cfx_profile_enable(int on);
int cfx_profile_reset(void);
int cfx_profile_count(void);
int cfx_profile_get(int i, const char** name, double* total_ms, int64_t* launches);
int cfx_event_create(void** ev);
int cfx_event_record(void* ev);
int cfx_event_elapsed_ms(void* start, void* stop, double* ms);
int cfx_event_destroy(void* ev);

int cfx_mesh_create(int tdim, int gdim, int64_t nnodes, const double* x,
                    int64_t ncells, const int32_t* conn, int cell_stride,
                    cfx_mesh_t* out);
int cfx_mesh_create_box(int tdim, int n, cfx_mesh_t* out);
int cfx_mesh_create_slab(int n, int z0, int nz, cfx_mesh_t* out);
int cfx_mesh_info(cfx_mesh_t m, int* tdim, int* gdim, int64_t* nnodes, int64_t* ncells,
                  const double** x, const int32_t** conn);
int cfx_mesh_destroy(cfx_mesh_t m);

int cfx_cut_options_default(cfx_cut_options* opt);
int cfx_cut_create(cfx_mesh_t mesh, int n_level_sets, const int32_t* ls_dofmap,
                   int ls_ndofs_cell, int64_t ls_ndofs, const double* const* ls_values,
                   const cfx_cut_options* opt, cfx_cut_t* out);
#define CFX_NOT_CANDIDATE 2
int cfx_cut_restrict(cfx_cut_t cut, const int32_t* cells, int64_t n);
int cfx_cut_update(cfx_cut_t cut, const double* const* ls_values);
int cfx_cut_info(cfx_cut_t cut, int* tdim, int* gdim, int64_t* num_local_cells,
                 int* n_level_sets);
int cfx_cut_domain(cfx_cut_t cut, int level_set, const int8_t** domain);
int cfx_locate_entities(cfx_cut_t cut, const char* selector,
                        const int32_t** entities, int64_t* n);
int cfx_runtime_quadrature(cfx_cut_t cut, const char* selector, int order,
                           const char* backend, cfx_rules_t* out);
int cfx_runtime_quadratures(cfx_cut_t cut, int n, const char* const* selectors, int order,
                            const char* backend, cfx_rules_t* out);
int cfx_full_cell_rules(cfx_mesh_t mesh, const int32_t* cells, int64_t n, int order,
                        cfx_rules_t* out);
int cfx_rules_create(cfx_mesh_t mesh, int tdim, int64_t nq, int64_t nr, const double* points,
                     const double* weights, const int32_t* offsets,
                     const int32_t* parent_map, cfx_rules_t* out);
int cfx_rules_view_get(cfx_rules_t r, cfx_rules_view* view);
int cfx_rules_physical_points(cfx_rules_t r, double* out);
int cfx_rules_destroy(cfx_rules_t r);
int cfx_evaluate_normals(cfx_cut_t cut, int level_set, cfx_rules_t rules, double sign,
                         double* out );
int cfx_evaluate_values(cfx_cut_t cut, int level_set, cfx_rules_t rules,
                        double* out );
int cfx_ghost_penalty_facets(cfx_cut_t cut, const char* selector,
                             const int32_t** rows, int64_t* n);
int cfx_interior_facets_for_cells(cfx_mesh_t mesh, const int32_t* cells, int64_t n, int32_t** rows, int64_t* n_rows);

int cfx_cut_create_facets(cfx_mesh_t mesh, int64_t n, const int32_t* facet_ids, const int32_t* rows, int row_width,
                          const int32_t* entity_geometry, int n_level_sets, const int32_t* ls_dofmap, int ls_ndofs_cell,
                          int64_t ls_ndofs, const double* const* ls_values, const cfx_cut_options* opt, cfx_cut_t* out);
int cfx_exterior_facets(cfx_mesh_t mesh, int32_t** rows, int64_t* n_rows);
int cfx_full_facet_rules(cfx_cut_t facet_cut, const char* selector, int order, cfx_rules_t* out);
int cfx_facet_rules_to_cells(cfx_rules_t facet_rules, int side, cfx_rules_t* out);

typedef struct
{
  int64_t ncells;
  const int32_t* root_cell;
  const int32_t* aggregate_id;
  const int32_t* propagation_depth;
  const double* cut_volume_fraction;
  const int32_t *active_cells, *cut_cells, *interior_cells, *well_posed_cells, *ill_posed_cells, *rootless_cells;
  int64_t n_active, n_cut, n_interior, n_well_posed, n_ill_posed, n_rootless;
  const int32_t* pairs;
  int64_t n_pairs;
} cfx_aggregation_view;
int cfx_cell_aggregation_create(cfx_cut_t cut, const char* selector, double volume_fraction_threshold,
                                int root_policy, int max_iterations, int allow_rootless, cfx_aggregation_t* out);
int cfx_cell_aggregation_view_get(cfx_aggregation_t agg, cfx_aggregation_view* view);
int cfx_cell_aggregation_destroy(cfx_aggregation_t agg);
int cfx_cut_destroy(cfx_cut_t cut);

int cfx_space_create(cfx_mesh_t mesh, int degree, int bs, int64_t ndofs,
                     const int32_t* dofmap, int ndofs_cell, cfx_space_t* out);
int cfx_space_static_bytes(cfx_space_t V, int64_t bytes[4]);
int cfx_space_lattice_rows(cfx_space_t V, int64_t* n, int64_t* template_rows);
int cfx_space_lattice_source_rows(cfx_space_t V, int64_t* rows);
int cfx_space_destroy(cfx_space_t V);

int cfx_form_create(cfx_space_t V, int rank, int n_integrals,
                    const cfx_integral* integrals, cfx_form_t* out);
int cfx_form_create2(cfx_space_t V_test, cfx_space_t V_trial, int n_integrals, const cfx_integral* integrals,
                     cfx_form_t* out);
int cfx_form_destroy(cfx_form_t a);
int cfx_form_prepare(cfx_form_t a);
int cfx_create_sparsity(cfx_form_t a, cfx_pattern_t* out);
int cfx_pattern_view_get(cfx_pattern_t p, cfx_pattern_view* view);
int cfx_pattern_reuse_stats(cfx_pattern_t p, int64_t* hashed_rows, int64_t* reused_rows);
int cfx_pattern_destroy(cfx_pattern_t p);
int cfx_assemble_matrix(cfx_form_t a, cfx_pattern_t pattern, const int8_t* bc0,
                        const int8_t* bc1, double* values);
int cfx_assemble_matrix_zeroed(cfx_form_t a, cfx_pattern_t pattern, const int8_t* bc0,
                               const int8_t* bc1, double* values);
int cfx_assemble_vector(cfx_form_t L, double* b);
int cfx_assemble_scalar(cfx_form_t M, double* value);

int cfx_apply_lifting(cfx_form_t a, const int8_t* bc_markers, const double* bc_values, const double* x0,
                      double alpha, double* b);
int cfx_set_bc(int64_t n, const int8_t* bc_markers, const double* bc_values, const double* x0, double alpha,
               double* b);
int cfx_zero_rows(cfx_pattern_t P, const double* values, double tol, int32_t** rows, int64_t* n_rows);
int cfx_csr_block_merge(int nbr, int nbc, const int64_t* const* indptr, const int32_t* const* indices,
                        const double* const* values, const int64_t* nrows, const int64_t* ncols, int64_t** out_indptr,
                        int32_t** out_indices, double** out_values, int64_t* out_nnz);
int cfx_csr_permute(int64_t nrows, int64_t ncols, const int64_t* indptr, const int32_t* indices, const double* values,
                    const int32_t* row_perm, const int32_t* col_perm, int64_t** out_indptr, int32_t** out_indices,
                    double** out_values);
int cfx_tabulate_entity(cfx_form_t a, int integral, int64_t index, int use_rule, double* Ae);

int cfx_integrand_register(const char* name, const char* source, int rank, int* kernel_id);
int cfx_integrand_compile(int kernel_id, int tdim, int ndofs_cell);
int cfx_integrand_register_facet(const char* name, const char* source, int* kernel_id);
int cfx_integrand_register_variant(const char* name, const char* source, int rank, int facet, int tdim, int ndofs_cell, int bs,
                                   int* kernel_id);
int cfx_integrand_compile_bs(int kernel_id, int tdim, int ndofs_cell, int bs);
int cfx_integrand_register2(const char* name, const char* source, int facet, int tdim, int nd0, int bs0, int nd1, int bs1,
                            int* kernel_id);
int cfx_integrand_compile2(int kernel_id, int tdim, int nd0, int bs0, int nd1, int bs1);
typedef struct { cfx_space_t space; const double* values; } cfx_coefficient;
int cfx_form_set_coefficients(cfx_form_t a, int integral, int n, const cfx_coefficient* coeffs);
int cfx_integrand_compile_coefficients(int kernel_id, int tdim, int nd0, int bs0, int nd1, int bs1,
                                       int n, const int* nd, const int* bs);

int cfx_active_domain(cfx_form_t a, cfx_active_t* out);
int cfx_active_view(cfx_active_t d, const int32_t** active_cells, int64_t* n_active,
                    const int32_t** inactive_dofs, int64_t* n_inactive);
int cfx_deactivate_outside(cfx_active_t d, cfx_pattern_t pattern, double* values,
                           double* b , double diagonal, double rhs_value);
int cfx_active_destroy(cfx_active_t d);

#define CFX_PC_NONE 0
#define CFX_PC_JACOBI 1
#define CFX_CG_CONVERGED 1
#define CFX_CG_MAX_ITER 2
#define CFX_CG_BREAKDOWN 3
#define CFX_CG_BAD_DIAGONAL 4
typedef struct
{
  double rtol, atol;
  int32_t max_iter, check_every, precond, lanes_per_row;
} cfx_cg_options;
typedef struct
{
  int32_t reason, iterations;
  double residual_norm, rhs_norm;
} cfx_cg_info;
int cfx_csr_spmv(int64_t nrows, const int64_t* indptr, const int32_t* indices, const double* values,
                 const int32_t* rows , int64_t n_rows, int lanes_per_row ,
                 const double* x, double* y);
int cfx_cg_options_default(cfx_cg_options* opt);
int cfx_cg_solve(int64_t nrows, const int64_t* indptr, const int32_t* indices, const double* values,
                 const int32_t* rows, int64_t n_rows, const double* b, double* x ,
                 const cfx_cg_options* opt , cfx_cg_info* info );

typedef struct
{
  int32_t tdim, gdim;
  int64_t nq, nr;
  const float* points;
  const float* weights;
  const int32_t* offsets;
  const int32_t* parent_map;
  int32_t host_width;
  int32_t reserved;
  const int32_t* host_rows;
  const int32_t* host_verts;
} cfx_rules_view_f32;
int cfx_mesh_create_f32(int tdim, int gdim, int64_t nnodes, const float* x, int64_t ncells, const int32_t* conn,
                        int cell_stride, cfx_mesh_t* out);
int cfx_cut_create_f32(cfx_mesh_t mesh, int n_level_sets, const int32_t* ls_dofmap, int ls_ndofs_cell,
                       int64_t ls_ndofs, const float* const* ls_values, const cfx_cut_options* opt, cfx_cut_t* out);
int cfx_cut_update_f32(cfx_cut_t cut, const float* const* ls_values);
int cfx_rules_create_f32(cfx_mesh_t mesh, int tdim, int64_t nq, int64_t nr, const float* points, const float* weights,
                         const int32_t* offsets, const int32_t* parent_map, cfx_rules_t* out);
int cfx_rules_view_get_f32(cfx_rules_t r, cfx_rules_view_f32* view);
int cfx_rules_physical_points_f32(cfx_rules_t r, float* out);
int cfx_evaluate_normals_f32(cfx_cut_t cut, int level_set, cfx_rules_t rules, float sign, float* out);
int cfx_evaluate_values_f32(cfx_cut_t cut, int level_set, cfx_rules_t rules, float* out);
int cfx_widen_f32(const float* src, int64_t n, double** out);
int cfx_assemble_matrix_f32(cfx_form_t a, cfx_pattern_t pattern, const int8_t* bc0, const int8_t* bc1, float* values);
int cfx_assemble_matrix_zeroed_f32(cfx_form_t a, cfx_pattern_t pattern, const int8_t* bc0, const int8_t* bc1,
                                   float* values);
int cfx_assemble_vector_f32(cfx_form_t L, float* b);
int cfx_apply_lifting_f32(cfx_form_t a, const int8_t* bc_markers, const float* bc_values, const float* x0, float alpha,
                          float* b);
int cfx_set_bc_f32(int64_t n, const int8_t* bc_markers, const float* bc_values, const float* x0, float alpha, float* b);
int cfx_zero_rows_f32(cfx_pattern_t P, const float* values, float tol, int32_t** rows, int64_t* n_rows);
int cfx_deactivate_outside_f32(cfx_active_t d, cfx_pattern_t pattern, float* values, float* b ,
                               float diagonal, float rhs_value);
int cfx_assemble_matrix_c128(cfx_form_t a, cfx_pattern_t pattern, const int8_t* bc0, const int8_t* bc1, const double* scales,
                             int zero_first, double* values );
int cfx_assemble_vector_c128(cfx_form_t L, const double* scales, double* b );
int cfx_apply_lifting_c128(cfx_form_t a, const int8_t* bc_markers, const double* bc_values ,
                           const double* x0 , double alpha_re, double alpha_im, const double* scales,
                           double* b );
int cfx_set_bc_c128(int64_t n, const int8_t* bc_markers, const double* bc_values, const double* x0, double alpha_re,
                    double alpha_im, double* b);
int cfx_deactivate_outside_c128(cfx_active_t domain, cfx_pattern_t pattern, double* values, double* b, double diag_re,
                                double diag_im, double rhs_re, double rhs_im);
int cfx_assemble_matrix_c64(cfx_form_t a, cfx_pattern_t pattern, const int8_t* bc0, const int8_t* bc1, const double* scales,
                            int zero_first, float* values );
int cfx_assemble_vector_c64(cfx_form_t L, const double* scales, float* b );
int cfx_apply_lifting_c64(cfx_form_t a, const int8_t* bc_markers, const float* bc_values ,
                          const float* x0 , double alpha_re, double alpha_im, const double* scales,
                          float* b );
int cfx_set_bc_c64(int64_t n, const int8_t* bc_markers, const float* bc_values, const float* x0, double alpha_re,
                   double alpha_im, float* b);
int cfx_deactivate_outside_c64(cfx_active_t domain, cfx_pattern_t pattern, float* values, float* b, double diag_re,
                               double diag_im, double rhs_re, double rhs_im);


typedef struct cfx_comm_s* cfx_comm_t;
#define CFX_DIST_ID_BYTES 128
typedef int (*cfx_host_exchange_fn)(void* user, int n, const int32_t* peers, const void* const* send,
                                    const int64_t* send_bytes, void* const* recv, const int64_t* recv_bytes);
int cfx_dist_unique_id(char id[CFX_DIST_ID_BYTES]);
int cfx_dist_comm_create(int world, int rank, const char id[CFX_DIST_ID_BYTES], cfx_comm_t* out);
int cfx_dist_comm_create_host(int world, int rank, cfx_host_exchange_fn fn, void* user, cfx_comm_t* out);
typedef int (*cfx_device_exchange_fn)(void* user, int n, const int32_t* peers, const void* const* send,
                                      const int64_t* send_bytes, void* const* recv, const int64_t* recv_bytes);
int cfx_dist_comm_create_device(int world, int rank, cfx_device_exchange_fn fn, void* user, cfx_comm_t* out);
int cfx_dist_comm_info(cfx_comm_t comm, int* world, int* rank, int* is_rccl);
int cfx_dist_comm_destroy(cfx_comm_t comm);
typedef struct
{
  int32_t peer;
  int32_t reserved;
  int64_t send_offset, send_count;
  const int32_t* send_index;
  int64_t recv_offset, recv_count;
  const int32_t* recv_index;
} cfx_dist_exchange;
int cfx_dist_scatter_forward(cfx_comm_t comm, double* x, int n, const cfx_dist_exchange* ex);
int cfx_dist_scatter_reverse_add(cfx_comm_t comm, double* x, int n, const cfx_dist_exchange* ex);
typedef struct
{
  int32_t peer;
  int32_t reserved;
// ... 13 lines not shown
```

Before: 1.164 billion DOF/s.

## Restrict closed-form P1 source hex kernel to shell hexes read by non-lattice rows

For the P1 series source term on large entity lists, the change first marks in a bitset the hexes touched by rows that do not use the lattice closed form, then compacts those bits into a hex list. The hex kernel then runs only over that shell instead of scanning every hex group of the full entity list, and it recovers entity offsets through bit ranks. The aim is to skip source work for interior hexes whose rows are already covered by the lattice template. In exchange it adds a mark kernel with atomics, a compaction pass and a persistent bitset that has to be cleared each step. Debug APIs for tile lists and shell counts, plus a rewritten tile-list compaction, are also included.

```diff
diff --git a/cutfemx_amd/_lib.py b/cutfemx_amd/_lib.py
--- a/cutfemx_amd/_lib.py
+++ b/cutfemx_amd/_lib.py
@@ -108,7 +108,7 @@
     "cfx_rules_physical_points", "cfx_rules_destroy", "cfx_evaluate_normals",
     "cfx_evaluate_values", "cfx_ghost_penalty_facets", "cfx_interior_facets_for_cells", "cfx_cell_aggregation_create", "cfx_cell_aggregation_view_get",
     "cfx_cell_aggregation_destroy", "cfx_cut_destroy", "cfx_space_create",
-    "cfx_space_static_bytes", "cfx_space_lattice_rows", "cfx_space_lattice_source_rows", "cfx_space_destroy", "cfx_form_create", "cfx_form_create2", "cfx_form_destroy", "cfx_form_prepare", "cfx_create_sparsity",
+    "cfx_space_static_bytes", "cfx_space_lattice_rows", "cfx_space_lattice_source_rows", "cfx_space_source_shell_hexes", "cfx_space_destroy", "cfx_form_create", "cfx_form_create2", "cfx_form_destroy", "cfx_form_prepare", "cfx_form_lattice_tile_lists", "cfx_create_sparsity",
     "cfx_pattern_view_get", "cfx_pattern_reuse_stats", "cfx_pattern_destroy", "cfx_assemble_matrix", "cfx_assemble_matrix_zeroed", "cfx_assemble_vector", "cfx_assemble_scalar",
     "cfx_apply_lifting", "cfx_set_bc", "cfx_zero_rows", "cfx_csr_block_merge", "cfx_csr_permute", "cfx_tabulate_entity", "cfx_active_domain", "cfx_active_view", "cfx_deactivate_outside",
     "cfx_active_destroy", "cfx_csr_spmv", "cfx_cg_options_default", "cfx_cg_solve",
diff --git a/cutfemx_amd/csrc/cfx_common.h b/cutfemx_amd/csrc/cfx_common.h
--- a/cutfemx_amd/csrc/cfx_common.h
+++ b/cutfemx_amd/csrc/cfx_common.h
@@ -533,6 +533,10 @@
   double lat_src_T[kLatSrcDegrees][8] = {};
   bool lat_src_T_built[kLatSrcDegrees] = {};
   DevArray<unsigned long long> lat_src_written;
+  DevArray<unsigned long long> lat_shell_ran;
+  mutable bool lat_shell_counted = false;
+  mutable DevArray<unsigned long long> shell_bits;
+  mutable bool shell_dirty = false;
   DevArray<uint8_t> arena;
   int64_t arena_used = 0;
   template <typename T>
@@ -807,6 +811,8 @@
 bool lattice_template(cfx_space_s* V);
 const double* lattice_source_moments(cfx_space_s* V, int qdegree);
 bool plain_lattice_tiles(cfx_form_s* a, unsigned inline_bits);
+void lattice_tile_lists(cfx_form_s* a, int64_t* n_plain, int64_t* n_tiles, int32_t* plain_rows, uint8_t* templ,
+                        int32_t* tile_first, int32_t* tile_id);
 bool space_dof_verts(cfx_space_s* V);
 bool plain_vec_offsets(cfx_form_s* L, uint8_t mark);
 bool source_groups_ok(cfx_form_s* L, uint8_t mark);
diff --git a/cutfemx_amd/csrc/cfx_fem.hip b/cutfemx_amd/csrc/cfx_fem.hip
--- a/cutfemx_amd/csrc/cfx_fem.hip
+++ b/cutfemx_amd/csrc/cfx_fem.hip
@@ -1762,6 +1762,27 @@
   CFX_API_END
 }
 
+int cfx_space_source_shell_hexes(cfx_space_t V, int64_t* hexes)
+{
+  CFX_API_BEGIN
+  require(V && hexes, CFX_ERR_INVALID_ARGUMENT, "cfx_space_source_shell_hexes: null argument");
+  *hexes = 0;
+  const cfx::Stencil& S = V->stencil;
+  if (S.lat_built && S.lat_rows > 0 && S.lat_shell_ran.p) *hexes = (int64_t)cfx::read_scalar(S.lat_shell_ran.p);
+  CFX_API_END
+}
+
+int cfx_form_lattice_tile_lists(cfx_form_t a, int64_t* n_plain, int64_t* n_tiles, int32_t* plain_rows, uint8_t* templ,
+                                int32_t* tile_first, int32_t* tile_id)
+{
+  CFX_API_BEGIN
+  require(a && n_plain && n_tiles, CFX_ERR_INVALID_ARGUMENT, "cfx_form_lattice_tile_lists: null argument");
+  *n_plain = 0; *n_tiles = -1;
+  if (a->rank == 0 || !a->plan) return CFX_OK;
+  cfx::lattice_tile_lists(a, n_plain, n_tiles, plain_rows, templ, tile_first, tile_id);
+  CFX_API_END
+}
+
 int cfx_space_destroy(cfx_space_t V)
 {
   CFX_API_BEGIN
diff --git a/cutfemx_amd/csrc/cfx_gather.hip b/cutfemx_amd/csrc/cfx_gather.hip
--- a/cutfemx_amd/csrc/cfx_gather.hip
+++ b/cutfemx_amd/csrc/cfx_gather.hip
@@ -608,18 +608,173 @@
   const int32_t* first;
   DevN ng;
   int64_t cap;
+  const unsigned long long* bits = nullptr;
+  const int32_t* rank = nullptr;
+  unsigned long long* ran = nullptr;
 };
 
-template <bool LATTICE>
-__global__ void __launch_bounds__(kBlock, CFX_SOURCE_WAVES) vec_source_groups_kernel(VecArgs A, GroupArgs G, const uint8_t* __restrict__ diagpos)
-{
-  __shared__ int32_t s_queue[LATTICE ? kBlock : 1];
+constexpr int kShellMarkRows = 4;
+__global__ void __launch_bounds__(kBlock) source_shell_mark_kernel(DevN n_special_d, const int32_t* __restrict__ special,
+                                                                   DevN n_plain_d, const int32_t* __restrict__ plain,
+                                                                   const int32_t* __restrict__ t2off,
+                                                                   const uint8_t* __restrict__ diagpos,
+                                                                   const int64_t* __restrict__ d2c_off,
+                                                                   const int32_t* __restrict__ d2c,
+                                                                   const uint8_t* __restrict__ cellmark, uint8_t mark,
+                                                                   unsigned int* __restrict__ bits32, int64_t nhex,
+                                                                   unsigned long long* __restrict__ ran)
+{
+  __shared__ int32_t s_rows[kBlock];
+  __shared__ int s_n;
+  const int64_t i = (int64_t)blockIdx.x * kBlock + threadIdx.x;
+  if (i == 0) *ran = 0ull;
+  if (threadIdx.x == 0) s_n = 0;
+  __syncthreads();
+  int32_t r = -1;
+  if (i < n_special_d.cap)
+  {
+    if (i < dev_n(n_special_d)) r = special[i];
+  }
+  else if (i - n_special_d.cap < dev_n(n_plain_d))
+  {
+    r = plain[i - n_special_d.cap];
+    if (lattice_source_row(t2off[r], diagpos[r])) r = -1;
+  }
+  if (r >= 0) s_rows[atomicAdd(&s_n, 1)] = r;
+  __syncthreads();
+  constexpr int U = kShellMarkRows, NG = kBlock / 32;
+  const int nq = s_n, k = threadIdx.x & 31;
+  auto hex_of = [&](int32_t c) -> int64_t { return c >= 0 && (cellmark[c] & mark) && c / 6 < nhex ? (int64_t)(c / 6) : -1; };
+  for (int q0 = threadIdx.x >> 5; q0 < nq; q0 += NG * U)
+  {
+    int64_t e0[U], e1[U], h[U];
+    int32_t c[U];
+    bool todo[U];
+    unsigned w[U];
+#pragma unroll
+    for (int u = 0; u < U; ++u)
+    {
+      const int q = q0 + u * NG;
+      e0[u] = 0; e1[u] = 0;
+      if (q < nq) { const int64_t row = s_rows[q]; e0[u] = d2c_off[row]; e1[u] = d2c_off[row + 1]; }
+    }
+#pragma unroll
+    for (int u = 0; u < U; ++u) c[u] = e0[u] + k < e1[u] ? d2c[e0[u] + k] : -1;
+#pragma unroll
+    for (int u = 0; u < U; ++u) h[u] = hex_of(c[u]);
+#pragma unroll
+    for (int u = 0; u < U; ++u)
+    {
+      const int64_t left = __shfl_up(h[u], 1, 32);
+      todo[u] = h[u] >= 0 && !(k > 0 && left == h[u]);
+      w[u] = todo[u] ? bits32[h[u] >> 5] : ~0u;
+    }
+#pragma unroll
+    for (int u = 0; u < U; ++u)
+      if (todo[u] && !(w[u] & (1u << (h[u] & 31)))) atomicOr(&bits32[h[u] >> 5], 1u << (h[u] & 31));
+#pragma unroll
+    for (int u = 0; u < U; ++u)
+      for (int64_t e = e0[u] + 32 + k; e < e1[u]; e += 32)
+      {
+        const int64_t hh = hex_of(d2c[e]);
+        if (hh >= 0 && !(bits32[hh >> 5] & (1u << (hh & 31)))) atomicOr(&bits32[hh >> 5], 1u << (hh & 31));
+      }
+  }
+}
+
+struct ShellWords
+{
+  unsigned long long* words;
+  int64_t nwords;
+  int per;
+};
+
+__global__ void __launch_bounds__(kBlock) source_shell_count_kernel(ShellWords S, int32_t* __restrict__ tile_counts)
+{
+  const int64_t base = (int64_t)blockIdx.x * kBlock * S.per;
+  int c = 0;
+  for (int k = 0; k < S.per; ++k)
+  {
+    const int64_t i = base + (int64_t)k * kBlock + threadIdx.x;
+    if (i < S.nwords) c += __popcll(S.words[i]);
+  }
+  int total;
+  (void)block_exclusive_scan<int>(c, total);
+  if (threadIdx.x == 0) tile_counts[blockIdx.x] = total;
+}
+
+__global__ void __launch_bounds__(kBlock) source_shell_write_kernel(ShellWords S, const int64_t* __restrict__ tile_offsets,
+                                                                    int32_t* __restrict__ out, int64_t cap, ChainState chain,
+                                                                    int64_t* __restrict__ total_out, CountJobs after)
+{
+  const unsigned int tile = chain.state ? chain_take_tile(chain.ticket) : blockIdx.x;
+  const int64_t base = ((int64_t)tile * kBlock + threadIdx.x) * S.per;
+  int c = 0;
+  for (int k = 0; k < S.per; ++k)
+    if (base + k < S.nwords) c += __popcll(S.words[base + k]);
+  int total;
+  const int off = block_exclusive_scan<int>(c, total);
+  int64_t prefix;
+  if (chain.state) prefix = (int64_t)chain_exclusive_prefix(chain.state, tile, (unsigned long long)total);
+  else prefix = tile_offsets[tile];
+  int64_t o = prefix + off;
+  if (c > 0)
+    for (int k = 0; k < S.per; ++k)
+    {
+      const int64_t i = base + k;
+      unsigned long long w = i < S.nwords ? S.words[i] : 0ull;
+      if (w == 0ull) continue;
+      S.words[i] = 0ull;
+      while (w)
+      {
+        if (o < cap) out[o] = (int32_t)(i * 64 + __builtin_ctzll(w));
+        ++o;
+        w &= w - 1ull;
+      }
+    }
+  if (chain.state && tile == gridDim.x - 1 && threadIdx.x == kBlock - 1)
+  {
+    *total_out = prefix + total;
+    if (after.n > 0) count_publish(after);
+  }
+}
+
+#ifndef CFX_SOURCE_SHELL_WAVES
+#define CFX_SOURCE_SHELL_WAVES 3
+#endif
+template <bool LATTICE, bool SHELL = false>
+__global__ void __launch_bounds__(kBlock, SHELL ? CFX_SOURCE_SHELL_WAVES : CFX_SOURCE_WAVES)
+vec_source_groups_kernel(VecArgs A, GroupArgs G, const uint8_t* __restrict__ diagpos)
+{
+  static_assert(LATTICE || !SHELL, "the shell list serves the closed-form path");
+  __shared__ int32_t s_queue[LATTICE && !SHELL ? kBlock : 1];
   __shared__ int s_n;
   int64_t g = (int64_t)blockIdx.x * kBlock + threadIdx.x;
   int q = threadIdx.x, nq = 0;
+  int32_t shell_hex = 0;
+  unsigned shell_mask = 0;
   if constexpr (!LATTICE)
   {
     if (g >= dev_n(G.ng)) return;
+  }
+  else if constexpr (SHELL)
+  {
+    if (threadIdx.x == 0) s_n = 0;
+    __syncthreads();
+    if (g < dev_n(G.ng))
+    {
+      shell_hex = G.first[g];
+      const int64_t c0 = 6 * (int64_t)shell_hex;
+      const int sh = (int)(c0 & 63);
+      unsigned long long m = G.bits[c0 >> 6] >> sh;
+      if (sh > 58) m |= G.bits[(c0 >> 6) + 1] << (64 - sh);
+      shell_mask = (unsigned)m & 63u;
+    }
+    const int ran = __popcll(__ballot(shell_mask != 0));
+    if ((threadIdx.x & 63) == 0 && ran) atomicAdd(&s_n, ran);
+    __syncthreads();
+    if (threadIdx.x == 0 && s_n) atomicAdd(G.ran, (unsigned long long)s_n);
+    if (shell_mask == 0) return;
   }
   else
   {
@@ -640,21 +795,33 @@
   }
   do
   {
-    if constexpr (LATTICE)
+    if constexpr (LATTICE && !SHELL)
     {
       if (q >= nq) break;
       g = (int64_t)blockIdx.x * kBlock + s_queue[q];
       q += kBlock;
     }
-    const int64_t n = dev_n(A.n), f = G.first[g];
-    int32_t ids[6];
-#pragma unroll
-    for (int m = 0; m < 6; ++m) ids[m] = A.entities[f + m < n ? f + m : n - 1];
-    const int32_t hex = ids[0] / 6;
+    int64_t f;
+    int32_t hex;
     unsigned mask = 0;
-#pragma unroll
-    for (int m = 0; m < 6; ++m)
-      if (f + m < n && ids[m] / 6 == hex) mask |= 1u << (ids[m] - 6 * hex);
+    if constexpr (SHELL)
+    {
+      hex = shell_hex;
+      mask = shell_mask;
+      f = entity_index(G.bits, G.rank, 6 * (int64_t)hex + __builtin_ctz(mask));
+    }
+    else
+    {
+      const int64_t n = dev_n(A.n);
+      f = G.first[g];
+      int32_t ids[6];
+#pragma unroll
+      for (int m = 0; m < 6; ++m) ids[m] = A.entities[f + m < n ? f + m : n - 1];
+      hex = ids[0] / 6;
+#pragma unroll
+      for (int m = 0; m < 6; ++m)
+        if (f + m < n && ids[m] / 6 == hex) mask |= 1u << (ids[m] - 6 * hex);
+    }
     const int4* conn4 = reinterpret_cast<const int4*>(A.conn) + 6 * (int64_t)hex;
     const int4 r0 = conn4[0], r3 = conn4[3], r4 = conn4[4];
     const int32_t cv[8] = {r0.x, r0.y, r3.y, r0.z, r4.y, r4.z, r3.z, r0.w};
@@ -715,7 +882,7 @@
       }
       else if (plain & (1u << k)) A.t2[(int64_t)k * G.cap + A.t2off[sv[k]] - 1] = acc[k];
     }
-  } while (LATTICE);
+  } while (LATTICE && !SHELL);
 }
 
 struct VecBlockArgs
@@ -3579,9 +3746,60 @@
   }
 }
 
+constexpr int64_t kSourceShellMinEntities = 4000000;
+inline Count source_shell_hexes(cfx_form_s* L, int slot, const uint8_t* diagpos, DevArray<int32_t>& hexes)
+{
+  cfx_space_s* V = L->V;
+  cfx_row_plan& plan = row_plan(L);
+  const char* site = "vec.shell_hexes";
+  const int64_t nhex = V->mesh->ncells / 6, nwords = (nhex + 63) / 64;
+  const int64_t nrows = plan.n_special_rows.cap() + plan.n_plain_rows.cap();
+  const Stencil& stn = space_stencil(V);
+  if (nwords == 0 || nrows == 0)
+  {
+    hexes.alloc(0);
+    step_record(site, 0);
+    dev_fill(stn.lat_shell_ran.p, 0, sizeof(unsigned long long));
+    return Count(0);
+  }
+  if (stn.shell_bits.n != nwords) { stn.shell_bits.alloc(nwords); stn.shell_dirty = true; }
+  if (stn.shell_dirty) stn.shell_bits.zero();
+  stn.shell_dirty = true;
+  const Adjacency& adj = V->dof_cells();
+  const DevN n_special = plan.n_special_rows, n_plain = plan.n_plain_rows;
+  launch("source_shell", source_shell_mark_kernel, grid_for(nrows), dim3(kBlock), 0, n_special, plan.special_rows.p, n_plain,
+         plan.plain_rows.p, plan.vec_t2off.p, diagpos, adj.offsets.p, adj.cells.p, plan.cellmark.p, (uint8_t)(1u << slot),
+         reinterpret_cast<unsigned int*>(stn.shell_bits.p), nhex, stn.lat_shell_ran.p);
+  const int per = (int)std::min<int64_t>(64, std::max<int64_t>(1, (nwords + 512 * kBlock - 1) / (512 * kBlock)));
+  const int64_t ntiles = (nwords + (int64_t)kBlock * per - 1) / ((int64_t)kBlock * per);
+  const ShellWords W{stn.shell_bits.p, nwords, per};
+  DevArray<int32_t> counts;
+  DevArray<int64_t> offsets(ntiles + 1);
+  Count total;
+  const CountSource src{offsets.p + ntiles, kCountI64, kCountUpTo};
+  CountPlan cp(1, &site, &src);
+  const ChainState chain = fused_chain(cp.publish, ntiles);
+  CountJobs after{};
+  if (chain.state) after = cp.take_jobs();
+  else
+  {
+    counts.alloc(ntiles);
+    launch("source_groups", source_shell_count_kernel, dim3((unsigned)ntiles), dim3(kBlock), 0, W, counts.p);
+    exclusive_scan(counts.p, offsets.p, ntiles, &cp);
+  }
+  cp.finish(&total);
+  hexes.alloc(total.cap());
+  if (total.cell) hexes.count = total;
+  launch("source_groups", source_shell_write_kernel, dim3((unsigned)ntiles), dim3(kBlock), 0, W, offsets.p, hexes.p, total.cap(),
+         chain, offsets.p + ntiles, after);
+  stn.shell_dirty = false;
+  stn.lat_shell_counted = true;
+  return total;
+}
+
 template <int TDIM, int DEG>
 void vec_tensors(cfx_form_s* L, const cfx_integral_dev& I, bool runtime, double* out, double* t2 = nullptr, int64_t out_cells = 0,
-                 const uint8_t* lat_src = nullptr)
+                 const uint8_t* lat_src = nullptr, int slot = -1)
 {
   cfx_space_s* V = L->V;
   if (user_integrand_known(I.kernel))
@@ -3604,6 +3822,19 @@
     if (TDIM == 3 && DEG == 1 && A.t2 && plan.vec_groups && source_series_ok<DEG>(V, I))
     {
       DevArray<int32_t> first;
+      const char shell_sw = env_char<Sw::SOURCE_SHELL>();
+      const bool shell_on = shell_sw == '2' || (shell_sw != '0' && I.n_entities.hint() >= kSourceShellMinEntities);
+      if (lat_src && slot >= 0 && plan.std_bits[slot].p && plan.std_rank[slot].p && space_stencil(V).lat_shell_ran.p && shell_on)
+      {
+        const Count ns = source_shell_hexes(L, slot, lat_src, first);
+        GroupArgs G{first.p, ns.devn(), plan.vec_group_cap};
+        G.bits = reinterpret_cast<const unsigned long long*>(plan.std_bits[slot].p);
+        G.rank = plan.std_rank[slot].p;
+        G.ran = space_stencil(V).lat_shell_ran.p;
+        if (ns.cap() > 0)
+          launch("vec_tensors_std", vec_source_groups_kernel<true, true>, grid_for(ns.cap()), dim3(kBlock), 0, A, G, lat_src);
+        return;
+      }
       const Count ng = compact_count("source_groups", "vec.source_groups", A.n, GroupHead{A.entities}, first);
       GroupArgs G{first.p, ng.devn(), plan.vec_group_cap};
       if (ng.cap() > 0 && lat_src)
@@ -3705,7 +3936,7 @@
       R.std_by_cell = by_cell ? 1 : 0;
       if (a->rank == 2) dump_integral(a, ii, 1, st.buffers.back().p);
       else if constexpr (BS == 1)
-        vec_tensors<TDIM, DEG>(a, I, false, st.buffers.back().p, st.vec_t2, by_cell ? V->mesh->ncells : 0, st.lat_src);
+        vec_tensors<TDIM, DEG>(a, I, false, st.buffers.back().p, st.vec_t2, by_cell ? V->mesh->ncells : 0, st.lat_src, s);
     }
     const int64_t n_rules = I.rules ? I.rules->nr.cap() : 0;
     if (n_rules > 0 && combine_cuts)
@@ -4348,6 +4579,9 @@
 {
   Stage1 st;
   cfx_row_plan& plan = row_plan(L);
+  const Stencil& shell_stn = L->V->stencil;
+  const bool shell_counted = shell_stn.lat_shell_counted;
+  shell_stn.lat_shell_counted = false;
   int slot = -1, count = 0;
   for (int s = 0; s < plan.n_cell_slots; ++s)
     if (L->integrals[plan.cell_slot_integral[s]].n_entities.cap() > 0) { slot = s; ++count; }
@@ -4380,6 +4614,7 @@
   }
   RowArgs A = prepare<TDIM, DEG>(L, st);
   A.values = b;
+  if (shell_counted && !shell_stn.lat_shell_counted) dev_fill(shell_stn.lat_shell_ran.p, 0, sizeof(unsigned long long));
   if (st.vec_blocks)
   {
     st.part.alloc(plan.vb_total);
diff --git a/cutfemx_amd/csrc/cfx_rowasm.hip b/cutfemx_amd/csrc/cfx_rowasm.hip
--- a/cutfemx_amd/csrc/cfx_rowasm.hip
+++ b/cutfemx_amd/csrc/cfx_rowasm.hip
@@ -2584,6 +2584,8 @@
     S.lat_written.zero();
     S.lat_src_written.alloc(1);
     S.lat_src_written.zero();
+    S.lat_shell_ran.alloc(1);
+    S.lat_shell_ran.zero();
     S.lat_rstar = (int64_t)h[1];
     S.lat_sb0 = (int64_t)h[4];
     S.lat_rel = (int)((int64_t)h[5] - (int64_t)h[4]);
@@ -2707,6 +2709,161 @@
   }
 };
 
+static_assert(kRowTile == 16, "the 16-entry halo and windows of tile_lists_write_kernel");
+__global__ void __launch_bounds__(kBlock) tile_lists_write_kernel(DevN n_d, LatTileStart lat, TileIdEmit ea, TileIdEmit eb,
+                                                                  const int64_t* __restrict__ tile_offsets,
+                                                                  int32_t* __restrict__ outA, int64_t capA,
+                                                                  int32_t* __restrict__ outB, int64_t capB, ChainState chain,
+                                                                  int64_t* __restrict__ total_out, CountJobs after)
+{
+  __shared__ unsigned long long s_ts[kTile / 64 + 2], s_nt[kTile / 64 + 2];
+  const int64_t n = dev_n(n_d);
+  const unsigned int tile = chain.state ? chain_take_tile(chain.ticket) : blockIdx.x;
+  const int64_t tbase = (int64_t)tile * kTile;
+  const int lane = threadIdx.x & 63, wave = threadIdx.x >> 6;
+  auto flags = [&](int64_t i, bool& ts, bool& nt)
+  {
+    ts = false; nt = false;
+    if (i >= 0 && i < n)
+    {
+      ts = i == 0 || (lat.rows[i] / kRowTile) != (lat.rows[i - 1] / kRowTile);
+      nt = !lat.templ(i);
+    }
+  };
+#pragma unroll
+  for (int k = 0; k < kScanItems; ++k)
+  {
+    const int chunk = k * (kBlock / 64) + wave;
+    bool ts, nt;
+    flags(tbase + (int64_t)chunk * 64 + lane, ts, nt);
+    const unsigned long long bt = __ballot(ts), bn = __ballot(nt);
+    if (lane == 0) { s_ts[1 + chunk] = bt; s_nt[1 + chunk] = bn; }
+  }
+  if (wave == 0)
+  {
+    bool ts, nt;
+    flags(lane >= 48 ? tbase - 64 + lane : -1, ts, nt);
+    const unsigned long long bt = __ballot(ts), bn = __ballot(nt);
+    if (lane == 0) { s_ts[0] = bt; s_nt[0] = bn; s_ts[kTile / 64 + 1] = 0ull; s_nt[kTile / 64 + 1] = 0ull; }
+  }
+  __syncthreads();
+  const int lo = 64 + (int)threadIdx.x * kScanItems - 15, wd = lo >> 6, sh = lo & 63;
+  auto window = [&](const unsigned long long* a) -> unsigned
+  {
+    unsigned long long v = a[wd] >> sh;
+    if (sh) v |= a[wd + 1] << (64 - sh);
+    return (unsigned)v & 0x7fffffu;
+  };
+  const unsigned wts = window(s_ts), wnt = window(s_nt);
+  const int64_t base = tbase + (int64_t)threadIdx.x * kScanItems;
+  bool fa[kScanItems], fb[kScanItems];
+  int64_t c = 0;
+#pragma unroll
+  for (int k = 0; k < kScanItems; ++k)
+  {
+    fa[k] = (wts >> (15 + k)) & 1u;
+    const unsigned t16 = (wts >> k) & 0xffffu;
+    const int q = t16 ? 31 - __clz((int)t16) : 0;
+    const unsigned before = ((wnt >> k) & 0x7fffu) >> q;
+    fb[k] = ((wnt >> (15 + k)) & 1u) && before == 0u;
+    c += (fa[k] ? 1ll : 0ll) + (fb[k] ? (1ll << 32) : 0ll);
+  }
+  int64_t total;
+  const int64_t off = block_exclusive_scan<int64_t>(c, total);
+  int64_t prefix;
+  if (chain.state) prefix = (int64_t)chain_exclusive_prefix(chain.state, tile, (unsigned long long)total);
+  else prefix = tile_offsets[tile];
+  int64_t oa = ((prefix + off) & 0xffffffffll), ob = ((prefix + off) >> 32);
+#pragma unroll
+  for (int k = 0; k < kScanItems; ++k)
+  {
+    if (fa[k]) { if (oa < capA) { outA[oa] = (int32_t)(base + k); ea(oa, base + k); } ++oa; }
+    if (fb[k]) { if (ob < capB) { outB[ob] = (int32_t)(base + k); eb(ob, base + k); } ++ob; }
+  }
+  if (chain.state && tile == gridDim.x - 1 && threadIdx.x == kBlock - 1)
+  {
+    *total_out = prefix + total;
+    if (after.n > 0) count_publish(after);
+  }
+}
+
+static void compact_tile_lists(const char* name, const char* const sites[2], DevN n, const LatTileStart& lat, TileIdEmit& ea,
+                               TileIdEmit& eb, DevArray<int32_t>& outA, DevArray<int32_t>& outB, Count totals[2],
+                               const std::function<void(int64_t, int64_t)>& pre)
+{
+  const int64_t ntiles = (n.cap + kTile - 1) / kTile;
+  if (ntiles == 0)
+  {
+    outA.alloc(0); outB.alloc(0);
+    step_record(sites[0], 0); step_record(sites[1], 0);
+    totals[0] = Count(0); totals[1] = Count(0);
+    pre(0, 0);
+    return;
+  }
+  DevArray<int64_t> counts;
+  DevArray<int64_t> offsets(ntiles + 1);
+  const CountSource src[2] = {{offsets.p + ntiles, kCountLo32, kCountUpTo}, {offsets.p + ntiles, kCountHi32, kCountUpTo}};
+  CountPlan cp(2, sites, src);
+  const ChainState chain = fused_chain(cp.publish, ntiles);
+  CountJobs after{};
+  if (chain.state) after = cp.take_jobs();
+  else
+  {
+    counts.alloc(ntiles);
+    launch(name, compact_count2_n_kernel<TileStart, LatTileStart>, dim3((unsigned)ntiles), dim3(kBlock), 0, n, TileStart{lat.rows}, lat,
+           counts.p);
+    exclusive_scan(counts.p, offsets.p, ntiles, &cp);
+  }
+  cp.finish(totals);
+  outA.alloc(totals[0].cap()); outB.alloc(totals[1].cap());
+  if (totals[0].cell) outA.count = totals[0];
+  if (totals[1].cell) outB.count = totals[1];
+  pre(totals[0].cap(), totals[1].cap());
+  launch(name, tile_lists_write_kernel, dim3((unsigned)ntiles), dim3(kBlock), 0, n, lat, ea, eb, offsets.p, outA.p, totals[0].cap(),
+         outB.p, totals[1].cap(), chain, offsets.p + ntiles, after);
+}
+
+__global__ void __launch_bounds__(kBlock) lattice_templ_flags_kernel(DevN n_d, LatTileStart lat, uint8_t* __restrict__ out)
+{
+  const int64_t i = (int64_t)blockIdx.x * kBlock + threadIdx.x;
+  if (i < dev_n(n_d)) out[i] = lat.templ(i) ? 1 : 0;
+}
+
+void lattice_tile_lists(cfx_form_s* a, int64_t* n_plain, int64_t* n_tiles, int32_t* plain_rows, uint8_t* templ,
+                        int32_t* tile_first, int32_t* tile_id)
+{
+  cfx_row_plan& plan = row_plan(a);
+  *n_plain = 0; *n_tiles = -1;
+  if (!plan.plain_masks_built || !plan.lat_tiles_built || plan.lat_bits == 0) return;
+  const int64_t np = plan.n_plain_rows.value(), nt = plan.n_lat_tiles.value();
+  *n_plain = np; *n_tiles = nt;
+  if (plain_rows && np > 0)
+  {
+    const std::vector<int32_t> r = download(plan.plain_rows.p, np);
+    std::copy(r.begin(), r.end(), plain_rows);
+  }
+  if (templ && np > 0)
+  {
+    const Stencil& S = space_lattice(a->V);
+    const LatTileStart lat{plan.plain_rows.p, plan.plain_masks.p, plan.plain_uniform.p, S.diagpos.p, (1ull << S.lat_len) - 1ull,
+                           plan.lat_bits};
+    DevArray<uint8_t> flags(np);
+    launch("lattice_templ_flags", lattice_templ_flags_kernel, grid_for(np), dim3(kBlock), 0, DevN(np), lat, flags.p);
+    const std::vector<uint8_t> f = download(flags.p, np);
+    std::copy(f.begin(), f.end(), templ);
+  }
+  if (tile_first && nt > 0)
+  {
+    const std::vector<int32_t> f = download(plan.lat_tile_first.p, nt);
+    std::copy(f.begin(), f.end(), tile_first);
+  }
+  if (tile_id && nt > 0)
+  {
+    const std::vector<int32_t> f = download(plan.lat_tile_id.p, nt);
+    std::copy(f.begin(), f.end(), tile_id);
+  }
+}
+
 bool plain_lattice_tiles(cfx_form_s* a, unsigned inline_bits)
 {
   cfx_row_plan& plan = row_plan(a);
@@ -2806,7 +2963,7 @@
                                (1ull << lat->lat_len) - 1ull, lat_bits};
       const char* const sites[2] = {"plan.plain_tiles", "plan.lattice_tiles"};
       Count totals[2];
-      compact_count_pair("plan_plain_tiles", sites, plan.n_plain_rows.devn(), TileStart{plan.plain_rows.p}, lpred, emit, lemit,
+      compact_tile_lists("plan_plain_tiles", sites, plan.n_plain_rows.devn(), lpred, emit, lemit,
                          first, lfirst, totals, [&](int64_t ca, int64_t cb)
                          {
                            plan.plain_tile_id.alloc(ca); emit.ids = plan.plain_tile_id.p;
diff --git a/cutfemx_amd/csrc/cfx_switches.h b/cutfemx_amd/csrc/cfx_switches.h
--- a/cutfemx_amd/csrc/cfx_switches.h
+++ b/cutfemx_amd/csrc/cfx_switches.h
@@ -25,6 +25,7 @@
   CFX_SWITCH(VEC_ROWORDER,       first_char, call,  "0: the P1 series source term without the row-ordered staging") \
   CFX_SWITCH(SOURCE_SERIES,      first_char, call,  "0: the P1 source term by quadrature instead of its series") \
   CFX_SWITCH(SOURCE_GROUPS,      first_char, call,  "0: the P1 series source term cell by cell instead of one hex per lane") \
+  CFX_SWITCH(SOURCE_SHELL,       first_char, call,  "0: the hex kernel of the closed-form source term sifts every hex of the entity list instead of taking the shell hexes from the rows that read them; 2: shell hexes whatever the length of the list (default: from 4 M entities)") \
   CFX_SWITCH(STAGING_NAN,        first_char, call,  "1 (tests): the hex-corner planes of the staging start as NaN") \
   CFX_SWITCH(PLAIN_STAGE,        first_char, call,  "0: plain rows without LDS staging, the form that meshes with stencils longer than 32 take by themselves") \
   CFX_SWITCH(MFMA,               first_char, call,  "0: generic rows instead of the MFMA kernel for staged elasticity tensors") \
diff --git a/cutfemx_amd/fem.py b/cutfemx_amd/fem.py
--- a/cutfemx_amd/fem.py
+++ b/cutfemx_amd/fem.py
@@ -218,6 +218,18 @@
     def prepare(self):
         _lib.check(_lib.lib().cfx_form_prepare(self._h))
         return self
+
+    def lattice_tile_lists(self):
+        n, t = C.c_int64(0), C.c_int64(-1)
+        f = _lib.lib().cfx_form_lattice_tile_lists
+        _lib.check(f(self._h, C.byref(n), C.byref(t), None, None, None, None))
+        if t.value < 0:
+            return None
+        rows, templ = np.zeros(max(n.value, 1), dtype=np.int32), np.zeros(max(n.value, 1), dtype=np.uint8)
+        first, ids = np.zeros(max(t.value, 1), dtype=np.int32), np.zeros(max(t.value, 1), dtype=np.int32)
+        ptr = lambda a: a.ctypes.data_as(C.c_void_p)
+        _lib.check(f(self._h, C.byref(n), C.byref(t), ptr(rows), ptr(templ), ptr(first), ptr(ids)))
+        return dict(plain_rows=rows[:n.value], templ=templ[:n.value], tile_first=first[:t.value], tile_id=ids[:t.value])
 
     def __del__(self):
         try:
diff --git a/cutfemx_amd/mesh.py b/cutfemx_amd/mesh.py
--- a/cutfemx_amd/mesh.py
+++ b/cutfemx_amd/mesh.py
@@ -188,6 +188,11 @@
         _lib.check(_lib.lib().cfx_space_lattice_source_rows(self._h, C.byref(n)))
         return int(n.value)
 
+    def source_shell_hexes(self) -> int:
+        n = C.c_int64(0)
+        _lib.check(_lib.lib().cfx_space_source_shell_hexes(self._h, C.byref(n)))
+        return int(n.value)
+
     @property
     def dofmap(self) -> np.ndarray:
         if hasattr(self, "_host_dofmap"):
diff --git a/include/cutfemx_amd.h b/include/cutfemx_amd.h
--- a/include/cutfemx_amd.h
+++ b/include/cutfemx_amd.h
@@ -202,6 +202,7 @@
 int cfx_space_static_bytes(cfx_space_t V, int64_t bytes[4]);
 int cfx_space_lattice_rows(cfx_space_t V, int64_t* n, int64_t* template_rows);
 int cfx_space_lattice_source_rows(cfx_space_t V, int64_t* rows);
+int cfx_space_source_shell_hexes(cfx_space_t V, int64_t* hexes);
 int cfx_space_destroy(cfx_space_t V);
 
 int cfx_form_create(cfx_space_t V, int rank, int n_integrals,
@@ -210,6 +211,8 @@
                      cfx_form_t* out);
 int cfx_form_destroy(cfx_form_t a);
 int cfx_form_prepare(cfx_form_t a);
+int cfx_form_lattice_tile_lists(cfx_form_t a, int64_t* n_plain, int64_t* n_tiles, int32_t* plain_rows, uint8_t* templ,
+                                int32_t* tile_first, int32_t* tile_id);
 int cfx_create_sparsity(cfx_form_t a, cfx_pattern_t* out);
 int cfx_pattern_view_get(cfx_pattern_t p, cfx_pattern_view* view);
 int cfx_pattern_reuse_stats(cfx_pattern_t p, int64_t* hashed_rows, int64_t* reused_rows);
```

Measured after the change: 1.226 billion DOF/s, median of 6. +5.3%, better.
